# SabaPivot/ProjectionTrainer

Measured on AMD Instinct MI355X. Metric: Stage-1 images/sec/node (SigLIP-L-384 + Gemma3-1B, 576+128 tok), higher is better.
Workload: dtype bf16; 1 GPU; cfg2: SigLIP-ViT-L/16-384 frozen fwd + MLP projector fwd/bwd + Gemma3-1B frozen fwd/bwd, 575 vis + 128 text tokens; global_batch=32, per_gpu_batch=32, seq_len=703, parallelism=dp1

## Files before the change

include/ptk.h:

```cpp
#ifndef PTK_H
#define PTK_H

#include <stddef.h>
#include <stdint.h>

#ifdef __cplusplus
extern "C" {
#endif

#define PTK_ABI_VERSION 8

int ptk_abi_version(void);
const char* ptk_last_error(void);


typedef struct {
  int g;
  int skip;
  int64_t gs;
  int64_t off;
} ptk_rowmap;

enum { PTK_ACT_NONE = 0, PTK_ACT_GELU_TANH = 1, PTK_ACT_GELU_ERF = 2, PTK_ACT_GEGLU = 3,
       PTK_ACT_GELU_ERF_BWD = 4, PTK_ACT_GEGLU_BWD = 5 };
enum { PTK_OUT_BF16 = 0, PTK_OUT_F32 = 1, PTK_OUT_F32_BF16ROUND = 2 };

typedef struct {
  const void* A;
  const void* B;
  void* C;
  int M, N, K;
  int64_t lda, ldb, ldc;
  int batch;
  int batch_inner;
  int64_t sA0, sA1, sB0, sB1, sC0, sC1;
  float alpha;
  int act;
  int out;
  const float* bias;
  const float* rowadd;
  int rowadd_period;
  int64_t ld_rowadd;
  const float* resid;
  int64_t ld_resid;
  void* aux;
  void* aux2;
  int64_t ld_aux;
  const void* aux_in;
  const void* aux_in2;
  int64_t ld_aux_in;
  ptk_rowmap amap;
  ptk_rowmap cmap;
  const void* resid16;
  int64_t ld_resid16;
  int bf16_linear;
  void* tail_ws;
  const void* B_kt;
  int A_kt, C_kt, aux_kt, aux_in_kt;
} ptk_gemm_desc;
int ptk_gemm_ktiled_counts(int64_t* out2, int reset);
int ptk_gemm_ktiled_pair(const ptk_gemm_desc* producer, const ptk_gemm_desc* consumer, int ncu, int64_t part_floats,
                         int train);
int ptk_a_ktiled_reload(void);
int ptk_gemm(const ptk_gemm_desc* d, void* stream);
int64_t ptk_kstep_tile_offset(int64_t row, int64_t k, int64_t K);
int ptk_pack_kstep_tiles_bf16(const void* src, void* dst, int N, int K, void* stream);
#define PTK_GEMM_TAIL_COUNTER_BYTES 16384
size_t ptk_gemm_tail_scratch_bytes(void);
int ptk_gemm_tail_split(const ptk_gemm_desc* d);
int ptk_gemm_plan(const ptk_gemm_desc* d, int ncu, int* path, int* tile_rows, int* tail_split);
int ptk_gemm_split_plan(const ptk_gemm_desc* d, int ncu, int64_t part_floats, int* slices, int* kc, int* rem,
                        int* tail_ws);

int ptk_layernorm(const float* x, const float* w, const float* b, void* y, int rows, int cols, float eps,
                  void* stream);
int ptk_rmsnorm(const float* x, const float* w, void* y, float* rstd, int rows, int cols, float eps,
                void* stream);
int ptk_rmsnorm_bwd(const float* x, const float* w, const float* rstd, const float* dn, const float* dacc,
                    float* dx, int rows, int cols, void* stream);
int ptk_qknorm_rope_fwd(const void* qkv, const float* q_norm_w, const float* k_norm_w, const float* cos_t,
                        const float* sin_t, int batch, int seq, int heads, int kv_heads, int head_dim, float eps,
                        void* Q, void* K, void* V, float* rstd_q, float* rstd_k, void* stream);
int ptk_qknorm_rope_bwd(const void* qkv, const float* q_norm_w, const float* k_norm_w, const float* cos_t,
                        const float* sin_t, int batch, int seq, int heads, int kv_heads, int head_dim,
                        const float* rstd_q, const float* rstd_k, const void* dQ, const void* dK, const void* dV,
                        void* dqkv, void* stream);
int ptk_softmax(const float* S, void* P, int nz, int rows, int cols, int64_t ld, int rows_per_batch, int qdiv,
                int zdiv, int causal, int window, const int32_t* key_valid, int key_len, void* stream);
int ptk_cross_entropy(void* logits, int64_t ld, int rows, int vocab, const int64_t* targets, float* row_loss,
                      const float* gscale, void* stream);
int ptk_transpose_bf16(const void* in, int64_t ld_in, void* out, int64_t ld_out, int nz, int64_t s_in,
                       int64_t s_out, int rows, int cols, int rows_pad, void* stream);
int ptk_transpose_rows_bf16(const void* in, int64_t ld_in, int map_g, int64_t map_gs, int64_t map_off, int rows,
                            int cols, void* out, int64_t ld_out, int rows_pad, void* stream);
int ptk_weight_grad_bf16(const void* dy, int64_t lddy, int y_map_g, int64_t y_map_gs, int64_t y_map_off, int Ny,
                         const void* x, int64_t ldx, int x_map_g, int64_t x_map_gs, int64_t x_map_off, int Nx, int rows,
                         void* grad, void* ta, void* tb, float* part, int64_t part_floats, int mode, void* stream);
int ptk_cast_f32_bf16(const float* in, void* out, int64_t n, void* stream);
int ptk_fill_normal_bf16(void* out, int64_t n, uint64_t seed, float std, float mean, void* stream);
int ptk_gemm_timer_enable(int on);
int ptk_gemm_force_small_tiles(int mode);
int ptk_gemm_timer_read(int act_class, double* total_ms, int* count);
#define PTK_GEMM_NPATHS 9
int ptk_gemm_path_counts(int64_t* counts, int reset);

int ptk_stage_timers_enable(int on);
int ptk_stage_begin(const char* name, void* stream);
int ptk_stage_end(void* stream);
int64_t ptk_stage_timers_read(char* buf, size_t cap, int reset);

typedef struct {
  const void* Q; const void* K; const void* V; void* O; float* lse;
  int rows, nkeys, head_dim;
  int64_t ldq, ldk, ldo;
  int batch, batch_inner, zdiv;
  int64_t sQ0, sQ1, sK0, sK1, sO0, sO1;
  ptk_rowmap qmap, omap;
  int qdiv, causal, window;
  const int32_t* key_valid;
  float scale;
} ptk_flash_desc;
int ptk_flash_attn_fwd(const ptk_flash_desc* d, void* stream);

typedef struct {
  const void* Q; const void* K; const void* V; const void* O; const void* dO;
  const float* lse; float* delta;
  void* dQ; void* dK; void* dV;
  int rows, nkeys, head_dim;
  int batch, batch_inner, zdiv;
  int64_t ldo, sO0, sO1;
  ptk_rowmap omap;
  int qdiv, causal, window;
  const int32_t* key_valid;
  float scale;
  void* workspace;
  int64_t workspace_bytes;
} ptk_flash_bwd_desc;
size_t ptk_flash_bwd_workspace_bytes(const ptk_flash_bwd_desc* d);
int ptk_flash_attn_bwd(const ptk_flash_bwd_desc* d, void* stream);

typedef struct {
  int image_size, patch_size, channels, hidden, heads, intermediate, layers;
  float eps;
} ptk_siglip_config;

typedef struct {
  const void* wqkv;  const float* bqkv;
  const void* wo;    const float* bo;
  const void* w1;    const float* b1;
  const void* w2;    const float* b2;
  const float* ln1_w; const float* ln1_b;
  const float* ln2_w; const float* ln2_b;
  const void* wqkv_kt; const void* wo_kt; const void* w1_kt; const void* w2_kt;
} ptk_siglip_layer;

typedef struct {
  const void* patch_w;
  const float* patch_b;
  const float* pos;
  const float* post_w; const float* post_b;
  const ptk_siglip_layer* layers;
} ptk_siglip_weights;

size_t ptk_siglip_workspace_bytes(const ptk_siglip_config* c, int batch);
int ptk_siglip_fwd(const ptk_siglip_config* c, const ptk_siglip_weights* w, int batch, const void* pixels,
                   void* out, void* ws, size_t ws_bytes, void* stream);

typedef struct {
  int vision_dim, inter_dim, llm_dim;
  const void* w1;   const float* b1;
  const void* w2;   const float* b2;
  const void* w2t;
  void* tail_ws;
} ptk_projector;

int ptk_projector_fwd(const ptk_projector* p, int rows, const void* x, void* a, void* h, float* out,
                      ptk_rowmap out_map, int64_t ld_out, int round_bf16, void* stream);
size_t ptk_projector_workspace_bytes(const ptk_projector* p, int rows);
int ptk_projector_bwd(const ptk_projector* p, int rows, const void* x, const void* a, const void* h,
                      const void* dy, float* dw1, float* db1, float* dw2, float* db2, void* ws, size_t ws_bytes,
                      void* stream);
int ptk_gather_vision_grad(const float* dx_llm, int batch, int num_patches, int seq_pad, int llm_dim, void* dy,
                           void* stream);

typedef struct {
  int vocab, hidden, inter, layers, heads, kv_heads, head_dim;
  int sliding_window, sliding_pattern;
  int pad_token_id;
  float query_pre_attn_scalar, eps;
} ptk_gemma3_config;

typedef struct {
  const void* wqkv;  const void* wqkv_t;
  const void* wo;    const void* wo_t;
  const void* wgu;   const void* wgu_t;
  const void* wd;    const void* wd_t;
  const float* ln_in; const float* ln_post_attn; const float* ln_pre_ff; const float* ln_post_ff;
  const float* q_norm; const float* k_norm;
  const void* wqkv_kt; const void* wqkv_t_kt;
  const void* wo_kt;   const void* wo_t_kt;
  const void* wgu_kt;  const void* wgu_t_kt;
  const void* wd_kt;   const void* wd_t_kt;
} ptk_gemma3_layer;

typedef struct {
  const void* embed;
  const void* embed_t;
  const float* final_norm;
  const float* rope_cos_local; const float* rope_sin_local;
  const float* rope_cos_global; const float* rope_sin_global;
  int rope_max_pos;
  const ptk_gemma3_layer* layers;
} ptk_gemma3_weights;

typedef struct {
  int batch, text_len, num_vision, seq_pad;
  const int64_t* token_ids;
  const int64_t* labels;
  float* x;
// ... 136 lines not shown
```

projectiontrainer_amd/_lib.py:

```python
from __future__ import annotations

import ctypes as C
import os

_HERE = os.path.dirname(os.path.abspath(__file__))
LIB_PATH = os.path.join(_HERE, "libptk.so")
if os.environ.get("PTK_LIB"):
    LIB_PATH = os.path.join(os.path.dirname(_HERE), os.environ["PTK_LIB"])

c_void_p, c_int, c_int64, c_float, c_size_t, c_uint64 = C.c_void_p, C.c_int, C.c_int64, C.c_float, C.c_size_t, C.c_uint64
c_float_p = C.POINTER(C.c_float)

ACT_NONE, ACT_GELU_TANH, ACT_GELU_ERF, ACT_GEGLU, ACT_GELU_ERF_BWD, ACT_GEGLU_BWD = range(6)
OUT_BF16, OUT_F32, OUT_F32_BF16ROUND = range(3)


class RowMap(C.Structure):
    _fields_ = [("g", c_int), ("skip", c_int), ("gs", c_int64), ("off", c_int64)]


class GemmDesc(C.Structure):
    _fields_ = [("A", c_void_p), ("B", c_void_p), ("C", c_void_p),
                ("M", c_int), ("N", c_int), ("K", c_int),
                ("lda", c_int64), ("ldb", c_int64), ("ldc", c_int64),
                ("batch", c_int), ("batch_inner", c_int),
                ("sA0", c_int64), ("sA1", c_int64), ("sB0", c_int64), ("sB1", c_int64),
                ("sC0", c_int64), ("sC1", c_int64),
                ("alpha", c_float), ("act", c_int), ("out", c_int),
                ("bias", c_void_p), ("rowadd", c_void_p), ("rowadd_period", c_int),
                ("ld_rowadd", c_int64), ("resid", c_void_p), ("ld_resid", c_int64),
                ("aux", c_void_p), ("aux2", c_void_p), ("ld_aux", c_int64),
                ("aux_in", c_void_p), ("aux_in2", c_void_p), ("ld_aux_in", c_int64),
                ("amap", RowMap), ("cmap", RowMap), ("resid16", c_void_p), ("ld_resid16", c_int64),
                ("bf16_linear", c_int), ("tail_ws", c_void_p), ("B_kt", c_void_p),
                ("A_kt", c_int), ("C_kt", c_int), ("aux_kt", c_int), ("aux_in_kt", c_int)]


class FlashDesc(C.Structure):
    _fields_ = [("Q", c_void_p), ("K", c_void_p), ("V", c_void_p), ("O", c_void_p), ("lse", c_void_p),
                ("rows", c_int), ("nkeys", c_int), ("head_dim", c_int),
                ("ldq", c_int64), ("ldk", c_int64), ("ldo", c_int64),
                ("batch", c_int), ("batch_inner", c_int), ("zdiv", c_int),
                ("sQ0", c_int64), ("sQ1", c_int64), ("sK0", c_int64), ("sK1", c_int64),
                ("sO0", c_int64), ("sO1", c_int64), ("qmap", RowMap), ("omap", RowMap),
                ("qdiv", c_int), ("causal", c_int), ("window", c_int), ("key_valid", c_void_p),
                ("scale", c_float)]


class FlashBwdDesc(C.Structure):
    _fields_ = [("Q", c_void_p), ("K", c_void_p), ("V", c_void_p), ("O", c_void_p), ("dO", c_void_p),
                ("lse", c_void_p), ("delta", c_void_p), ("dQ", c_void_p), ("dK", c_void_p), ("dV", c_void_p),
                ("rows", c_int), ("nkeys", c_int), ("head_dim", c_int),
                ("batch", c_int), ("batch_inner", c_int), ("zdiv", c_int),
                ("ldo", c_int64), ("sO0", c_int64), ("sO1", c_int64), ("omap", RowMap),
                ("qdiv", c_int), ("causal", c_int), ("window", c_int), ("key_valid", c_void_p),
                ("scale", c_float), ("workspace", c_void_p), ("workspace_bytes", c_int64)]


class SiglipConfigC(C.Structure):
    _fields_ = [("image_size", c_int), ("patch_size", c_int), ("channels", c_int), ("hidden", c_int),
                ("heads", c_int), ("intermediate", c_int), ("layers", c_int), ("eps", c_float)]


class SiglipLayerC(C.Structure):
    _fields_ = [("wqkv", c_void_p), ("bqkv", c_void_p), ("wo", c_void_p), ("bo", c_void_p),
                ("w1", c_void_p), ("b1", c_void_p), ("w2", c_void_p), ("b2", c_void_p),
                ("ln1_w", c_void_p), ("ln1_b", c_void_p), ("ln2_w", c_void_p), ("ln2_b", c_void_p),
                ("wqkv_kt", c_void_p), ("wo_kt", c_void_p), ("w1_kt", c_void_p), ("w2_kt", c_void_p)]


class SiglipWeightsC(C.Structure):
    _fields_ = [("patch_w", c_void_p), ("patch_b", c_void_p), ("pos", c_void_p),
                ("post_w", c_void_p), ("post_b", c_void_p), ("layers", C.POINTER(SiglipLayerC))]


class ProjectorC(C.Structure):
    _fields_ = [("vision_dim", c_int), ("inter_dim", c_int), ("llm_dim", c_int),
                ("w1", c_void_p), ("b1", c_void_p), ("w2", c_void_p), ("b2", c_void_p), ("w2t", c_void_p),
                ("tail_ws", c_void_p)]


class Gemma3ConfigC(C.Structure):
    _fields_ = [("vocab", c_int), ("hidden", c_int), ("inter", c_int), ("layers", c_int), ("heads", c_int),
                ("kv_heads", c_int), ("head_dim", c_int), ("sliding_window", c_int),
                ("sliding_pattern", c_int), ("pad_token_id", c_int),
                ("query_pre_attn_scalar", c_float), ("eps", c_float)]


class Gemma3LayerC(C.Structure):
    _fields_ = [("wqkv", c_void_p), ("wqkv_t", c_void_p), ("wo", c_void_p), ("wo_t", c_void_p),
                ("wgu", c_void_p), ("wgu_t", c_void_p), ("wd", c_void_p), ("wd_t", c_void_p),
                ("ln_in", c_void_p), ("ln_post_attn", c_void_p), ("ln_pre_ff", c_void_p),
                ("ln_post_ff", c_void_p), ("q_norm", c_void_p), ("k_norm", c_void_p),
                ("wqkv_kt", c_void_p), ("wqkv_t_kt", c_void_p), ("wo_kt", c_void_p), ("wo_t_kt", c_void_p),
                ("wgu_kt", c_void_p), ("wgu_t_kt", c_void_p), ("wd_kt", c_void_p), ("wd_t_kt", c_void_p)]


class Gemma3WeightsC(C.Structure):
    _fields_ = [("embed", c_void_p), ("embed_t", c_void_p), ("final_norm", c_void_p),
                ("rope_cos_local", c_void_p), ("rope_sin_local", c_void_p),
                ("rope_cos_global", c_void_p), ("rope_sin_global", c_void_p),
                ("rope_max_pos", c_int), ("layers", C.POINTER(Gemma3LayerC))]


class Gemma3BatchC(C.Structure):
    _fields_ = [("batch", c_int), ("text_len", c_int), ("num_vision", c_int), ("seq_pad", c_int),
                ("token_ids", c_void_p), ("labels", c_void_p), ("x", c_void_p), ("dx", c_void_p),
                ("loss_scale", c_float), ("loss", c_void_p), ("label_offset", c_int)]


class Gemma3GenerateC(C.Structure):
    _fields_ = [("batch", c_int), ("prompt_len", c_int), ("max_new_tokens", c_int), ("do_sample", c_int),
                ("top_k", c_int), ("temperature", c_float), ("seed", C.c_uint64), ("eos_token_id", c_int64),
                ("pad_token_id", c_int64), ("prompt_batch_stride", c_int64), ("top_p", c_float)]


class Gemma3DecodeC(C.Structure):
    _fields_ = [("rows", c_int), ("prompt_len", c_int), ("max_new_tokens", c_int), ("prompt_repeat", c_int),
                ("prompt_batch_stride", c_int64)]


class Gemma3LayerGradsC(C.Structure):
    _fields_ = [(n, c_void_p) for n in ("wqkv", "wo", "wgu", "wd", "ln_in", "ln_post_attn", "ln_pre_ff",
                                        "ln_post_ff", "q_norm", "k_norm")]


class Gemma3GradsC(C.Structure):
    _fields_ = [("embed", c_void_p), ("final_norm", c_void_p), ("layers", C.POINTER(Gemma3LayerGradsC))]


class ImageDesc(C.Structure):
    _fields_ = [("src_off", c_int64), ("h", C.c_int32), ("w", C.c_int32), ("c", C.c_int32),
                ("kh", C.c_int32), ("kv", C.c_int32), ("pad_", C.c_int32),
                ("coef_off", c_int64), ("tmp_off", c_int64)]


ABI_VERSION = 8

SIGNATURES = {
    "ptk_abi_version": (c_int, []),
    "ptk_last_error": (C.c_char_p, []),
    "ptk_gemm": (c_int, [C.POINTER(GemmDesc), c_void_p]),
    "ptk_gemm_tail_scratch_bytes": (c_size_t, []),
    "ptk_gemm_tail_split": (c_int, [C.POINTER(GemmDesc)]),
    "ptk_gemm_plan": (c_int, [C.POINTER(GemmDesc), c_int] + [C.POINTER(c_int)] * 3),
    "ptk_gemm_split_plan": (c_int, [C.POINTER(GemmDesc), c_int, c_int64] + [C.POINTER(c_int)] * 4),
    "ptk_layernorm": (c_int, [c_void_p, c_void_p, c_void_p, c_void_p, c_int, c_int, c_float, c_void_p]),
    "ptk_rmsnorm": (c_int, [c_void_p, c_void_p, c_void_p, c_void_p, c_int, c_int, c_float, c_void_p]),
    "ptk_rmsnorm_bwd": (c_int, [c_void_p] * 6 + [c_int, c_int, c_void_p]),
    "ptk_qknorm_rope_fwd": (c_int, [c_void_p] * 5 + [c_int] * 5 + [c_float] + [c_void_p] * 6),
    "ptk_qknorm_rope_bwd": (c_int, [c_void_p] * 5 + [c_int] * 5 + [c_void_p] * 7),
    "ptk_softmax": (c_int, [c_void_p, c_void_p, c_int, c_int, c_int, c_int64, c_int, c_int, c_int, c_int,
                            c_int, c_void_p, c_int, c_void_p]),
    "ptk_cross_entropy": (c_int, [c_void_p, c_int64, c_int, c_int, c_void_p, c_void_p, c_void_p, c_void_p]),
    "ptk_transpose_bf16": (c_int, [c_void_p, c_int64, c_void_p, c_int64, c_int, c_int64, c_int64, c_int,
                                   c_int, c_int, c_void_p]),
    "ptk_transpose_rows_bf16": (c_int, [c_void_p, c_int64, c_int, c_int64, c_int64, c_int, c_int, c_void_p, c_int64,
                                        c_int, c_void_p]),
    "ptk_weight_grad_bf16": (c_int, [c_void_p, c_int64, c_int, c_int64, c_int64, c_int,
                                     c_void_p, c_int64, c_int, c_int64, c_int64, c_int, c_int,
                                     c_void_p, c_void_p, c_void_p, c_void_p, c_int64, c_int, c_void_p]),
    "ptk_cast_f32_bf16": (c_int, [c_void_p, c_void_p, c_int64, c_void_p]),
    "ptk_kstep_tile_offset": (c_int64, [c_int64, c_int64, c_int64]),
    "ptk_pack_kstep_tiles_bf16": (c_int, [c_void_p, c_void_p, c_int, c_int, c_void_p]),
    "ptk_fill_normal_bf16": (c_int, [c_void_p, c_int64, c_uint64, c_float, c_float, c_void_p]),
    "ptk_gemm_timer_enable": (c_int, [c_int]),
    "ptk_gemm_force_small_tiles": (c_int, [c_int]),
    "ptk_gemm_timer_read": (c_int, [c_int, C.POINTER(C.c_double), C.POINTER(c_int)]),
    "ptk_gemm_path_counts": (c_int, [c_void_p, c_int]),
    "ptk_gemm_ktiled_counts": (c_int, [c_void_p, c_int]),
    "ptk_gemm_ktiled_pair": (c_int, [C.POINTER(GemmDesc), C.POINTER(GemmDesc), c_int, c_int64, c_int]),
    "ptk_a_ktiled_reload": (c_int, []),
    "ptk_stage_timers_enable": (c_int, [c_int]),
    "ptk_stage_begin": (c_int, [C.c_char_p, c_void_p]),
    "ptk_stage_end": (c_int, [c_void_p]),
    "ptk_stage_timers_read": (c_int64, [C.c_char_p, c_size_t, c_int]),
    "ptk_flash_attn_fwd": (c_int, [C.POINTER(FlashDesc), c_void_p]),
    "ptk_flash_attn_bwd": (c_int, [C.POINTER(FlashBwdDesc), c_void_p]),
    "ptk_flash_bwd_workspace_bytes": (c_size_t, [C.POINTER(FlashBwdDesc)]),
    "ptk_siglip_workspace_bytes": (c_size_t, [C.POINTER(SiglipConfigC), c_int]),
    "ptk_siglip_fwd": (c_int, [C.POINTER(SiglipConfigC), C.POINTER(SiglipWeightsC), c_int, c_void_p, c_void_p,
                               c_void_p, c_size_t, c_void_p]),
    "ptk_projector_fwd": (c_int, [C.POINTER(ProjectorC), c_int, c_void_p, c_void_p, c_void_p, c_void_p, RowMap,
                                  c_int64, c_int, c_void_p]),
    "ptk_projector_workspace_bytes": (c_size_t, [C.POINTER(ProjectorC), c_int]),
    "ptk_projector_bwd": (c_int, [C.POINTER(ProjectorC), c_int] + [c_void_p] * 8 + [c_void_p, c_size_t, c_void_p]),
    "ptk_gather_vision_grad": (c_int, [c_void_p, c_int, c_int, c_int, c_int, c_void_p, c_void_p]),
    "ptk_gemma3_workspace_bytes": (c_size_t, [C.POINTER(Gemma3ConfigC), c_int, c_int, c_int]),
    "ptk_gemma3_loss_fwd_bwd": (c_int, [C.POINTER(Gemma3ConfigC), C.POINTER(Gemma3WeightsC),
                                        C.POINTER(Gemma3BatchC), c_void_p, c_size_t, c_void_p]),
    "ptk_gemma3_loss_fwd": (c_int, [C.POINTER(Gemma3ConfigC), C.POINTER(Gemma3WeightsC),
                                    C.POINTER(Gemma3BatchC), c_void_p, c_size_t, c_void_p]),
    "ptk_gemma3_train_workspace_bytes": (c_size_t, [C.POINTER(Gemma3ConfigC), c_int, c_int, c_int]),
    "ptk_gemma3_train_fwd_bwd": (c_int, [C.POINTER(Gemma3ConfigC), C.POINTER(Gemma3WeightsC),
                                         C.POINTER(Gemma3BatchC), C.POINTER(Gemma3GradsC), c_void_p, c_size_t,
                                         c_void_p]),
    "ptk_gemma3_generate_workspace_bytes": (c_size_t, [C.POINTER(Gemma3ConfigC), c_int, c_int, c_int]),
    "ptk_gemma3_generate": (c_int, [C.POINTER(Gemma3ConfigC), C.POINTER(Gemma3WeightsC), C.POINTER(Gemma3GenerateC),
                                    c_void_p, c_void_p, c_void_p, c_void_p, c_void_p, c_size_t, c_void_p]),
    "ptk_gemma3_decode_workspace_bytes": (c_size_t, [C.POINTER(Gemma3ConfigC), C.POINTER(Gemma3DecodeC)]),
    "ptk_gemma3_decode_prefill": (c_int, [C.POINTER(Gemma3ConfigC), C.POINTER(Gemma3WeightsC),
                                          C.POINTER(Gemma3DecodeC), c_void_p, c_void_p, c_int64, c_void_p, c_void_p,
                                          c_size_t, c_void_p]),
    "ptk_gemma3_decode_step": (c_int, [C.POINTER(Gemma3ConfigC), C.POINTER(Gemma3WeightsC), C.POINTER(Gemma3DecodeC),
                                       c_int, c_void_p, c_void_p, c_void_p, c_void_p, c_size_t, c_void_p]),
    "ptk_beam_candidates_workspace_bytes": (c_size_t, [c_int, c_int, c_int]),
    "ptk_beam_candidates": (c_int, [c_void_p, c_int64, c_void_p, c_int, c_int, c_int, c_int, c_int, c_float, c_float,
                                    c_int, c_uint64, c_int, c_int, c_void_p, c_void_p, c_void_p, c_void_p, c_size_t,
                                    c_void_p]),
    "ptk_sample_next_token_workspace_bytes": (c_size_t, [c_int]),
    "ptk_sample_next_token": (c_int, [c_void_p, c_int64, c_int, c_int, c_int, c_int, c_float, c_float, c_uint64, c_int,
                                      c_int64, c_int64, c_void_p, c_void_p, c_int64, c_int, c_float, c_void_p,
                                      c_void_p, c_size_t, c_void_p]),
    "ptk_beam_candidates_penalized_workspace_bytes": (c_size_t, [c_int, c_int, c_int]),
    "ptk_beam_candidates_penalized": (c_int, [c_void_p, c_int64, c_void_p, c_int, c_int, c_int, c_int, c_int, c_float,
                                              c_float, c_int, c_uint64, c_int, c_int, c_void_p, c_int64, c_int,
                                              c_float, c_void_p, c_void_p, c_void_p, c_void_p, c_size_t, c_void_p]),
    "ptk_gemma3_generate_penalized_workspace_bytes": (c_size_t, [C.POINTER(Gemma3ConfigC), c_int, c_int, c_int]),
    "ptk_gemma3_generate_penalized": (c_int, [C.POINTER(Gemma3ConfigC), C.POINTER(Gemma3WeightsC),
                                              C.POINTER(Gemma3GenerateC), c_void_p, c_void_p, c_void_p, c_void_p,
                                              c_float, c_void_p, c_size_t, c_void_p]),
    "ptk_gemm_skinny_part_bytes": (c_size_t, [c_int, c_int, c_int]),
    "ptk_gemm_skinny": (c_int, [c_void_p, c_int64, c_void_p, c_int64, c_void_p, c_int64, c_int, c_int, c_int, c_int,
                                c_void_p, c_size_t, c_void_p]),
    "ptk_embed_grad_workspace_bytes": (c_size_t, [c_int, c_int]),
    "ptk_embed_grad": (c_int, [c_void_p, c_int, c_int, c_int, c_int, c_int, c_float, c_void_p, c_void_p, c_void_p,
                               c_size_t, c_void_p]),
    "ptk_bf16_sumsq_partial_floats": (c_int, []),
    "ptk_bf16_grad_scale_sumsq": (c_int, [c_void_p, c_int64, c_float, c_void_p, c_void_p, c_void_p]),
    "ptk_adamw_bf16": (c_int, [c_void_p] * 4 + [c_int64, c_void_p, c_float] + [C.c_double] * 5 +
                       [c_int, c_void_p, c_void_p]),
    "ptk_resize_ksize": (c_int, [c_int, c_int]),
    "ptk_resize_coeffs": (c_int, [c_int, c_int, c_void_p, c_void_p]),
    "ptk_image_preprocess": (c_int, [c_void_p, c_void_p, c_void_p, c_int, c_int, c_int, c_int, c_void_p, c_int,
                                     c_void_p, c_void_p, c_void_p]),
    "ptk_comm_unique_id_bytes": (c_int, []),
    "ptk_comm_get_unique_id": (c_int, [c_void_p]),
    "ptk_comm_init": (c_int, [C.POINTER(c_void_p), c_void_p, c_int, c_int]),
    "ptk_comm_destroy": (c_int, [c_void_p]),
    "ptk_comm_world": (c_int, [c_void_p]),
    "ptk_comm_allreduce_sum": (c_int, [c_void_p, c_void_p, c_int64, c_void_p]),
    "ptk_comm_allreduce_avg": (c_int, [c_void_p, c_void_p, c_int64, c_void_p]),
    "ptk_projector_bwd_allreduce": (c_int, [C.POINTER(ProjectorC), c_int] + [c_void_p] * 5 +
                                    [c_void_p, c_size_t, c_void_p, c_void_p, c_void_p]),
    "ptk_clip_adamw": (c_int, [c_void_p, c_void_p, c_void_p, c_void_p, c_int64, c_float, c_float, c_float,
                               c_float, c_float, c_float, c_float, c_int, c_void_p, c_void_p, c_void_p]),
}

_lib = None


class PtkError(RuntimeError):
    pass


def lib():
    global _lib
    if _lib is None:
        if not os.path.exists(LIB_PATH):
            raise PtkError(f"libptk.so not found at {LIB_PATH}: run `python -c 'import __graft_entry__ as g; g.build()'`")
        L = C.CDLL(LIB_PATH)
        for name, (res, args) in SIGNATURES.items():
            if os.environ.get("PTK_LIB") and not hasattr(L, name):
                continue
            f = getattr(L, name)
            f.restype, f.argtypes = res, args
        if L.ptk_abi_version() != ABI_VERSION:
            raise PtkError("libptk ABI version mismatch")
        _lib = L
    return _lib


def check(rc: int, what: str = ""):
    if rc != 0:
        raise PtkError(f"{what}: {lib().ptk_last_error().decode()}")


def ptr(t) -> int | None:
    return None if t is None else t.data_ptr()


GEMM_PATHS = ("nt128", "big", "big2", "w4", "nt128b", "p8sk", "p8", "tn", "unused8")


def gemm_path_counts(reset=False):
    buf = (C.c_int64 * (8 * len(GEMM_PATHS)))()
    check(lib().ptk_gemm_path_counts(buf, int(reset)), "gemm_path_counts")
    return {(GEMM_PATHS[i // 8], i % 8): int(v) for i, v in enumerate(buf) if v}


def gemm_ktiled_counts(reset=False):
    buf = (C.c_int64 * 2)()
    check(lib().ptk_gemm_ktiled_counts(buf, int(reset)), "gemm_ktiled_counts")
    return int(buf[0]), int(buf[1])


_stages_on = os.environ.get("PTK_STAGE_TIMERS", "0") not in ("", "0")


def stage_timers_enable(on=True):
    global _stages_on
    _stages_on = bool(on)
    check(lib().ptk_stage_timers_enable(int(bool(on))), "stage_timers_enable")


class stage:

    def __init__(self, name, device=None):
        self.name, self.device, self.on = name, device, False

    def __enter__(self):
        self.on = _stages_on
        if self.on:
            self.st = stream_ptr(self.device)
            check(lib().ptk_stage_begin(self.name.encode(), self.st), "stage_begin")
        return self

    def __exit__(self, *exc):
        if self.on:
            check(lib().ptk_stage_end(self.st), "stage_end")
        return False


def stage_timers_read(reset=False):
    n = lib().ptk_stage_timers_read(None, 0, 0)
    if n < 0:
        check(-1, "stage_timers_read")
    buf = C.create_string_buffer(int(n) + 64)
    n = lib().ptk_stage_timers_read(buf, len(buf), int(reset))
    if n < 0:
        check(-1, "stage_timers_read")
    out = {}
    for line in buf.value.decode().splitlines():
        name, ms, cnt = line.split("\t")
        out[name] = (float(ms), int(cnt))
    return out


def stream_ptr(device=None) -> int:
    import torch
    return torch.cuda.current_stream(device).cuda_stream
```

projectiontrainer_amd/csrc/attn.hip:

```cpp
#include "common.h"
#include "ptk_internal.h"

namespace ptk {

constexpr int QKR_HB = 4;

template <int EPL>
__global__ void __launch_bounds__(256) qknorm_rope_fwd_kernel(const bf16_t* __restrict__ qkv,
                                                              const float* __restrict__ qw,
                                                              const float* __restrict__ kw,
                                                              const float* __restrict__ cos_t,
                                                              const float* __restrict__ sin_t, AttnShape sh,
                                                              float eps, bf16_t* __restrict__ Q,
                                                              bf16_t* __restrict__ K, bf16_t* __restrict__ V,
                                                              float* __restrict__ rstd_q, float* __restrict__ rstd_k) {
  constexpr int D = EPL * 64;
  const int lane = threadIdx.x & 63;
  const int nh = sh.Hq + 2 * sh.Hkv;
  const long m = (long)blockIdx.x * 4 + (threadIdx.x >> 6);
  if (m >= (long)sh.B * sh.S) return;
  const int b = (int)(m / sh.S), s = (int)(m - (long)b * sh.S);
  const int G = sh.Hq / sh.Hkv;
  const int fi = (lane & 31) * EPL;
  const long ps = sh.pos ? (long)sh.pos[m] : (long)s;
// ... 45 lines not shown
      } else {
        const int kvh = h - sh.Hq;
        dst = K + (((long)b * sh.Hkv + kvh) * sh.S + s) * D + lane * EPL;
        if (lane == 0) rstd_k[m * sh.Hkv + kvh] = rs;
      }
#pragma unroll
      for (int e = 0; e < EPL; ++e) dst[e] = f2bf(xn[e] * cs[e] + sgn * part[e] * sn[e]);
    }
  }
}

template <int EPL>
__global__ void __launch_bounds__(256) qknorm_rope_bwd_kernel(
    const bf16_t* __restrict__ qkv, const float* __restrict__ qw, const float* __restrict__ kw,
    const float* __restrict__ cos_t, const float* __restrict__ sin_t, AttnShape sh, const float* __restrict__ rstd_q,
    const float* __restrict__ rstd_k, const bf16_t* __restrict__ dQ, const bf16_t* __restrict__ dK,
    const bf16_t* __restrict__ dV, bf16_t* __restrict__ dqkv, FlashBwdArgs fb) {
  constexpr int D = EPL * 64;
  const int lane = threadIdx.x & 63;
  const int nh = sh.Hq + 2 * sh.Hkv;
  const long m = (long)blockIdx.x * 4 + (threadIdx.x >> 6);
  if (m >= (long)sh.B * sh.S) return;
  const int b = (int)(m / sh.S), s = (int)(m - (long)b * sh.S);
  const int G = sh.Hq / sh.Hkv;
  const float* dkv_src = nullptr;
  int dkv_np = 0;
  if (D == 256 && fb.dkv_deferred) {
    const int slab = s / DKV_KEYS;
    const int P = dkv_pieces(fb, slab);
    if (P > 1) {
      dkv_np = P;
      dkv_src = fb.dkv_part + (long)dkv_part_base(fb, slab) * fb.nz * (2L * DKV_KEYS * D) +
                (long)(s - slab * DKV_KEYS) * D + lane * EPL;
    }
  }
  const int fi = (lane & 31) * EPL;
  float cs[EPL], sn[EPL], wq[EPL], wk[EPL];
#pragma unroll
  for (int e = 0; e < EPL; ++e) {
    cs[e] = cos_t[(long)s * (D / 2) + fi + e];
    sn[e] = sin_t[(long)s * (D / 2) + fi + e];
    wq[e] = 1.f + qw[lane * EPL + e];
    wk[e] = 1.f + kw[lane * EPL + e];
  }
  const float sgn = lane < 32 ? 1.f : -1.f;
  const bf16_t* xrow = qkv + m * (long)nh * D + lane * EPL;
  bf16_t* orow = dqkv + m * (long)nh * D + lane * EPL;
  for (int h0 = 0; h0 < nh; h0 += QKR_HB) {
    bf16_t gy[QKR_HB][EPL], xr[QKR_HB][EPL];
    float rsv[QKR_HB];
#pragma unroll
    for (int i = 0; i < QKR_HB; ++i) {
      const int h = h0 + i;
      if (h >= nh) break;
      const bf16_t* dy;
      if (h < sh.Hq) {
        const int kvh = h / G, j = h - kvh * G;
        dy = dQ + ((((long)b * sh.Hkv + kvh) * sh.S + s) * G + j) * D + lane * EPL;
        rsv[i] = rstd_q[m * sh.Hq + h];
      } else if (h < sh.Hq + sh.Hkv) {
        const int kvh = h - sh.Hq;
        dy = dK + (((long)b * sh.Hkv + kvh) * sh.S + s) * D + lane * EPL;
        rsv[i] = rstd_k[m * sh.Hkv + kvh];
      } else {
        dy = dV + (((long)b * sh.Hkv + (h - sh.Hq - sh.Hkv)) * sh.S + s) * D + lane * EPL;
        rsv[i] = 0.f;
      }
      if (dkv_np > 0 && h >= sh.Hq) {
        const int which = h < sh.Hq + sh.Hkv ? 0 : 1;
        const int kvh = which == 0 ? h - sh.Hq : h - sh.Hq - sh.Hkv;
        const long z = (long)b * sh.Hkv + kvh;
        const float* src = dkv_src + z * (2L * DKV_KEYS * D) + (long)which * DKV_KEYS * D;
        const long pstride = (long)fb.nz * (2L * DKV_KEYS * D);
        float acc[EPL];
#pragma unroll
        for (int e = 0; e < EPL; ++e) acc[e] = 0.f;
        for (int pc = 0; pc < dkv_np; ++pc) {
#pragma unroll
          for (int e = 0; e < EPL; ++e) acc[e] += src[pc * pstride + e];
        }
        const float mul = which == 0 ? fb.scale : 1.f;
#pragma unroll
        for (int e = 0; e < EPL; ++e) gy[i][e] = f2bf(acc[e] * mul);
      } else {
#pragma unroll
        for (int e = 0; e < EPL; ++e) gy[i][e] = dy[e];
      }
      if (h < sh.Hq + sh.Hkv)
#pragma unroll
        for (int e = 0; e < EPL; ++e) xr[i][e] = xrow[(long)h * D + e];
    }
#pragma unroll
    for (int i = 0; i < QKR_HB; ++i) {
      const int h = h0 + i;
      if (h >= nh) break;
      bf16_t* out = orow + (long)h * D;
      if (h >= sh.Hq + sh.Hkv) {
#pragma unroll
        for (int e = 0; e < EPL; ++e) out[e] = gy[i][e];
        continue;
      }
      const bool isq = h < sh.Hq;
      const float rs = rsv[i];
      float ds[EPL], dc[EPL], part[EPL];
#pragma unroll
      for (int e = 0; e < EPL; ++e) {
        const float g = bf2f(gy[i][e]);
        dc[e] = g * cs[e];
        ds[e] = g * sn[e];
      }
#pragma unroll
      for (int e = 0; e < EPL; ++e) part[e] = xor32_get(ds[e]);
      float x[EPL], dxn[EPL];
      float sdot = 0.f;
#pragma unroll
      for (int e = 0; e < EPL; ++e) {
        x[e] = bf2f(xr[i][e]);
        dxn[e] = bfround(dc[e] + sgn * part[e]) * (isq ? wq[e] : wk[e]);
        sdot += dxn[e] * x[e];
      }
      sdot = warp_sum(sdot);
      const float c3 = rs * rs * rs * sdot / D;
#pragma unroll
      for (int e = 0; e < EPL; ++e) out[e] = f2bf(rs * dxn[e] - c3 * x[e]);
    }
  }
}

constexpr int SMAXV = 8;

__global__ void __launch_bounds__(256) softmax_fwd_kernel(const float* __restrict__ S, bf16_t* __restrict__ P,
                                                          long nrows, int rows, int cols, long ld, MaskSpec mk) {
  const int lane = threadIdx.x & 63;
  const long gr = (long)blockIdx.x * 4 + (threadIdx.x >> 6);
  if (gr >= nrows) return;
  const long z = gr / rows;
  const int r = (int)(gr - z * rows);
  const int q = (r % mk.rows_per_batch) / mk.qdiv;
  const long b = z / mk.zdiv;
  const float* srow = S + gr * ld;
  bf16_t* prow = P + gr * ld;
  float4 v[SMAXV];
  float mx = -INFINITY;
#pragma unroll
  for (int i = 0; i < SMAXV; ++i) {
    const int c0 = lane * 4 + i * 256;
    if (c0 >= cols) break;
    float4 t = *reinterpret_cast<const float4*>(srow + c0);
    float tv[4] = {t.x, t.y, t.z, t.w};
#pragma unroll
    for (int e = 0; e < 4; ++e) {
      const int k = c0 + e;
      bool ok = mk.key_valid ? (mk.key_valid[b * cols + k] != 0) : (k < mk.key_len);
      if (mk.causal) ok = ok && (k <= q);
      if (mk.window) ok = ok && (k > q - mk.window);
      tv[e] = ok ? tv[e] : -INFINITY;
      mx = fmaxf(mx, tv[e]);
    }
    v[i] = make_float4(tv[0], tv[1], tv[2], tv[3]);
  }
  mx = warp_max(mx);
  float sum = 0.f;
#pragma unroll
  for (int i = 0; i < SMAXV; ++i) {
    const int c0 = lane * 4 + i * 256;
    if (c0 >= cols) break;
    float4 t = v[i];
    t.x = t.x == -INFINITY ? 0.f : __expf(t.x - mx);
    t.y = t.y == -INFINITY ? 0.f : __expf(t.y - mx);
    t.z = t.z == -INFINITY ? 0.f : __expf(t.z - mx);
    t.w = t.w == -INFINITY ? 0.f : __expf(t.w - mx);
    v[i] = t;
    sum += t.x + t.y + t.z + t.w;
  }
  sum = warp_sum(sum);
  const float inv = sum > 0.f ? 1.f / sum : 0.f;
#pragma unroll
  for (int i = 0; i < SMAXV; ++i) {
    const int c0 = lane * 4 + i * 256;
    if (c0 >= cols) break;
    u16x4_t o;
    o[0] = f2bf(v[i].x * inv); o[1] = f2bf(v[i].y * inv); o[2] = f2bf(v[i].z * inv); o[3] = f2bf(v[i].w * inv);
    *reinterpret_cast<u16x4_t*>(prow + c0) = o;
  }
}

__global__ void __launch_bounds__(256) softmax_bwd_kernel(const bf16_t* __restrict__ P, const float* __restrict__ dP,
                                                          bf16_t* __restrict__ dS, long nrows, int cols, long ld,
                                                          float scale) {
  const int lane = threadIdx.x & 63;
  const long gr = (long)blockIdx.x * 4 + (threadIdx.x >> 6);
  if (gr >= nrows) return;
  float4 pv[SMAXV], gv[SMAXV];
  float dot = 0.f;
#pragma unroll
  for (int i = 0; i < SMAXV; ++i) {
    const int c0 = lane * 4 + i * 256;
    if (c0 >= cols) break;
    u16x4_t u = *reinterpret_cast<const u16x4_t*>(P + gr * ld + c0);
    pv[i] = make_float4(bf2f(u[0]), bf2f(u[1]), bf2f(u[2]), bf2f(u[3]));
    gv[i] = *reinterpret_cast<const float4*>(dP + gr * ld + c0);
    dot += pv[i].x * gv[i].x + pv[i].y * gv[i].y + pv[i].z * gv[i].z + pv[i].w * gv[i].w;
  }
  dot = warp_sum(dot);
#pragma unroll
  for (int i = 0; i < SMAXV; ++i) {
    const int c0 = lane * 4 + i * 256;
    if (c0 >= cols) break;
    u16x4_t o;
    o[0] = f2bf(pv[i].x * (gv[i].x - dot) * scale);
    o[1] = f2bf(pv[i].y * (gv[i].y - dot) * scale);
    o[2] = f2bf(pv[i].z * (gv[i].z - dot) * scale);
    o[3] = f2bf(pv[i].w * (gv[i].w - dot) * scale);
    *reinterpret_cast<u16x4_t*>(dS + gr * ld + c0) = o;
  }
}

#define QKR_DISPATCH(KERNEL, ...)                                                                     \
  switch (s.D) {                                                                                      \
    case 64: hipLaunchKernelGGL(KERNEL<1>, grid, dim3(256), 0, st, __VA_ARGS__); break;              \
    case 128: hipLaunchKernelGGL(KERNEL<2>, grid, dim3(256), 0, st, __VA_ARGS__); break;             \
    case 256: hipLaunchKernelGGL(KERNEL<4>, grid, dim3(256), 0, st, __VA_ARGS__); break;             \
    default: return set_error("qknorm_rope: head_dim %d unsupported", s.D);                          \
  }

int launch_qknorm_rope_fwd(const bf16_t* qkv, const float* qw, const float* kw, const float* cos_t,
                           const float* sin_t, AttnShape s, float eps, bf16_t* Q, bf16_t* K, bf16_t* V,
                           float* rstd_q, float* rstd_k, hipStream_t st) {
  if (s.Hq % s.Hkv) return set_error("qknorm_rope: Hq %% Hkv != 0");
  const long waves = (long)s.B * s.S;
  dim3 grid((unsigned)((waves + 3) / 4));
  QKR_DISPATCH(qknorm_rope_fwd_kernel, qkv, qw, kw, cos_t, sin_t, s, eps, Q, K, V, rstd_q, rstd_k)
  return hipGetLastError() == hipSuccess ? 0 : set_error("qknorm_rope_fwd launch failed");
}
int launch_qknorm_rope_bwd(const bf16_t* qkv, const float* qw, const float* kw, const float* cos_t,
                           const float* sin_t, AttnShape s, const float* rstd_q, const float* rstd_k,
                           const bf16_t* dQ, const bf16_t* dK, const bf16_t* dV, bf16_t* dqkv, hipStream_t st,
                           const FlashBwdArgs* dkv) {
  if (s.Hq % s.Hkv) return set_error("qknorm_rope: Hq %% Hkv != 0");
  FlashBwdArgs fb;
  fb.dkv_deferred = 0;
  if (dkv && dkv->dkv_deferred) {
    if (s.D != 256 || dkv->D != 256 || dkv->nkeys != s.S || dkv->nz != s.B * s.Hkv || !dkv->dkv_part)
      return set_error("qknorm_rope_bwd: deferred dK/dV plan does not match the shape");
    fb = *dkv;
  }
  const long waves = (long)s.B * s.S;
  dim3 grid((unsigned)((waves + 3) / 4));
  QKR_DISPATCH(qknorm_rope_bwd_kernel, qkv, qw, kw, cos_t, sin_t, s, rstd_q, rstd_k, dQ, dK, dV, dqkv, fb)
  return hipGetLastError() == hipSuccess ? 0 : set_error("qknorm_rope_bwd launch failed");
}
int launch_softmax_fwd(const float* S, bf16_t* P, int nz, int rows, int cols, long ld, MaskSpec m, hipStream_t st) {
  if (cols % 4 || cols > SMAXV * 256 || ld % 4) return set_error("softmax: cols=%d unsupported", cols);
  const long nrows = (long)nz * rows;
  if (nrows <= 0) return 0;
  hipLaunchKernelGGL(softmax_fwd_kernel, dim3((unsigned)((nrows + 3) / 4)), dim3(256), 0, st, S, P, nrows, rows,
                     cols, ld, m);
  return hipGetLastError() == hipSuccess ? 0 : set_error("softmax_fwd launch failed");
}
int launch_softmax_bwd(const bf16_t* P, const float* dP, bf16_t* dS, int nrows, int cols, long ld, float scale,
                       hipStream_t st) {
  if (cols % 4 || cols > SMAXV * 256 || ld % 4) return set_error("softmax_bwd: cols=%d unsupported", cols);
  if (nrows <= 0) return 0;
  hipLaunchKernelGGL(softmax_bwd_kernel, dim3((unsigned)((nrows + 3) / 4)), dim3(256), 0, st, P, dP, dS,
                     (long)nrows, cols, ld, scale);
  return hipGetLastError() == hipSuccess ? 0 : set_error("softmax_bwd launch failed");
}

}
```

projectiontrainer_amd/csrc/capi.cpp:

```cpp
#include <stdarg.h>
#include <stdio.h>

#include "../../include/ptk.h"
#include "ptk_internal.h"

namespace ptk {

static thread_local char g_err[512] = "";

int set_error(const char* fmt, ...) {
  va_list ap;
  va_start(ap, fmt);
  vsnprintf(g_err, sizeof(g_err), fmt, ap);
  va_end(ap);
  return -1;
}

RowMap to_map(ptk_rowmap m) { return RowMap{m.g, m.skip, (long)m.gs, (long)m.off}; }

GemmArgs to_args(const ptk_gemm_desc* d) {
  GemmArgs a;
  a.A = (const bf16_t*)d->A; a.B = (const bf16_t*)d->B; a.C = d->C;
  a.M = d->M; a.N = d->N; a.K = d->K;
  a.lda = d->lda; a.ldb = d->ldb; a.ldc = d->ldc;
// ... 96 lines not shown
int ptk_qknorm_rope_fwd(const void* qkv, const float* q_norm_w, const float* k_norm_w, const float* cos_t,
                        const float* sin_t, int batch, int seq, int heads, int kv_heads, int head_dim, float eps,
                        void* Q, void* K, void* V, float* rstd_q, float* rstd_k, void* stream) {
  const AttnShape sh{batch, seq, heads, kv_heads, head_dim};
  return launch_qknorm_rope_fwd((const bf16_t*)qkv, q_norm_w, k_norm_w, cos_t, sin_t, sh, eps, (bf16_t*)Q,
                                (bf16_t*)K, (bf16_t*)V, rstd_q, rstd_k, ST);
}
int ptk_qknorm_rope_bwd(const void* qkv, const float* q_norm_w, const float* k_norm_w, const float* cos_t,
                        const float* sin_t, int batch, int seq, int heads, int kv_heads, int head_dim,
                        const float* rstd_q, const float* rstd_k, const void* dQ, const void* dK, const void* dV,
                        void* dqkv, void* stream) {
  const AttnShape sh{batch, seq, heads, kv_heads, head_dim};
  return launch_qknorm_rope_bwd((const bf16_t*)qkv, q_norm_w, k_norm_w, cos_t, sin_t, sh, rstd_q, rstd_k,
                                (const bf16_t*)dQ, (const bf16_t*)dK, (const bf16_t*)dV, (bf16_t*)dqkv, ST);
}
int ptk_softmax(const float* S, void* P, int nz, int rows, int cols, int64_t ld, int rows_per_batch, int qdiv,
                int zdiv, int causal, int window, const int32_t* key_valid, int key_len, void* stream) {
  MaskSpec m{rows_per_batch > 0 ? rows_per_batch : rows, qdiv > 0 ? qdiv : 1, zdiv > 0 ? zdiv : 1, causal, window,
             key_valid, key_len};
  return launch_softmax_fwd(S, (bf16_t*)P, nz, rows, cols, ld, m, ST);
}

int ptk_cross_entropy(void* logits, int64_t ld, int rows, int vocab, const int64_t* targets, float* row_loss,
                      const float* gscale, void* stream) {
  return launch_ce_fwd_bwd((bf16_t*)logits, ld, rows, vocab, targets, row_loss, gscale, ST);
}

int ptk_transpose_bf16(const void* in, int64_t ld_in, void* out, int64_t ld_out, int nz, int64_t s_in, int64_t s_out,
                       int rows, int cols, int rows_pad, void* stream) {
  return launch_transpose((const bf16_t*)in, ld_in, s_in, 0, 1, (bf16_t*)out, ld_out, s_out, 0, nz, rows, cols,
                          rows_pad, ST);
}

int ptk_transpose_rows_bf16(const void* in, int64_t ld_in, int map_g, int64_t map_gs, int64_t map_off, int rows,
                            int cols, void* out, int64_t ld_out, int rows_pad, void* stream) {
  const RowMap m{map_g, 0, map_gs, map_off};
  return launch_transpose_rows((const bf16_t*)in, ld_in, m, rows, cols, (bf16_t*)out, ld_out, rows_pad, ST);
}

int64_t ptk_kstep_tile_offset(int64_t row, int64_t k, int64_t K) { return kstep_tile_offset(row, k, K); }
int ptk_pack_kstep_tiles_bf16(const void* src, void* dst, int N, int K, void* stream) {
  return launch_pack_kstep_tiles((const bf16_t*)src, (bf16_t*)dst, N, K, ST);
}
int ptk_cast_f32_bf16(const float* in, void* out, int64_t n, void* stream) {
  return launch_cast_f32_bf16(in, (bf16_t*)out, n, ST);
}

int ptk_gemm_force_small_tiles(int mode) {
  if (mode != 0 && mode != 1 && mode != 2 && mode != 4 && mode != 8 && mode != 32 && mode != 512 && mode != 1024 &&
      mode != 4096)
    return set_error("gemm tile mode %d not in {0, 1, 2, 4, 8, 32, 512, 1024, 4096}", mode);
  force_small_tiles(mode);
  return 0;
}
int ptk_gemm_timer_enable(int on) {
  timer_enable(on);
  return 0;
}
int ptk_gemm_timer_read(int act_class, double* total_ms, int* count) { return timer_read(act_class, total_ms, count); }
int ptk_gemm_path_counts(int64_t* counts, int reset) { return path_counts(counts, reset); }
int ptk_gemm_ktiled_counts(int64_t* out2, int reset) { return ktiled_counts(out2, reset); }
int ptk_gemm_ktiled_pair(const ptk_gemm_desc* producer, const ptk_gemm_desc* consumer, int ncu, int64_t part_floats,
                         int train) {
  if (!producer || !consumer || ncu <= 0 || producer->batch > 1 || consumer->batch > 1) return 0;
  return !train && gemm_ktiled_pair(to_args(producer), producer->act, to_args(consumer), (long)part_floats,
                                    test_plan_env(ncu), a_ktiled_mode() != 0, true) ? 1 : 0;
}

int ptk_fill_normal_bf16(void* out, int64_t n, uint64_t seed, float std, float mean, void* stream) {
  return launch_fill_normal_bf16((bf16_t*)out, n, seed, std, mean, ST);
}

int ptk_flash_attn_fwd(const ptk_flash_desc* d, void* stream) {
  if (!d) return set_error("flash: null desc");
  FlashArgs a;
  a.Q = (const bf16_t*)d->Q; a.K = (const bf16_t*)d->K; a.V = (const bf16_t*)d->V; a.O = (bf16_t*)d->O;
  a.lse = d->lse; a.rows = d->rows; a.nkeys = d->nkeys; a.D = d->head_dim;
  a.ldq = d->ldq; a.ldk = d->ldk; a.ldo = d->ldo;
  a.zin = d->batch_inner > 0 ? d->batch_inner : 1; a.zdiv = d->zdiv > 0 ? d->zdiv : 1;
  a.sQ0 = d->sQ0; a.sQ1 = d->sQ1; a.sK0 = d->sK0; a.sK1 = d->sK1; a.sO0 = d->sO0; a.sO1 = d->sO1;
  a.qmap = to_map(d->qmap); a.omap = to_map(d->omap);
  a.qdiv = d->qdiv > 0 ? d->qdiv : 1; a.causal = d->causal; a.window = d->window;
  a.key_valid = d->key_valid; a.scale = d->scale;
  return launch_attn_fwd(a, d->batch > 0 ? d->batch : 1, ST);
}

static FlashBwdArgs to_bwd_args(const ptk_flash_bwd_desc* d) {
  FlashBwdArgs a;
  a.Q = (const bf16_t*)d->Q; a.K = (const bf16_t*)d->K; a.V = (const bf16_t*)d->V; a.O = (const bf16_t*)d->O;
  a.dO = (const bf16_t*)d->dO; a.lse = d->lse; a.delta = d->delta;
  a.dQ = (bf16_t*)d->dQ; a.dK = (bf16_t*)d->dK; a.dV = (bf16_t*)d->dV;
  a.rows = d->rows; a.nkeys = d->nkeys; a.D = d->head_dim;
  a.zin = d->batch_inner > 0 ? d->batch_inner : 1; a.zdiv = d->zdiv > 0 ? d->zdiv : 1;
  a.ldo = d->ldo; a.sO0 = d->sO0; a.sO1 = d->sO1; a.omap = to_map(d->omap);
  a.qdiv = d->qdiv > 0 ? d->qdiv : 1; a.causal = d->causal; a.window = d->window;
  a.key_valid = d->key_valid; a.scale = d->scale;
  a.dkv_part = (float*)d->workspace;
  a.dkv_part_bytes = d->workspace && d->workspace_bytes > 0 ? (size_t)d->workspace_bytes : 0;
  return a;
}

size_t ptk_flash_bwd_workspace_bytes(const ptk_flash_bwd_desc* d) {
  if (!d) return 0;
  return attn_bwd_workspace_bytes(to_bwd_args(d), d->batch > 0 ? d->batch : 1);
}

int ptk_flash_attn_bwd(const ptk_flash_bwd_desc* d, void* stream) {
  if (!d) return set_error("flash_bwd: null desc");
  return launch_attn_bwd(to_bwd_args(d), d->batch > 0 ? d->batch : 1, ST);
}

int ptk_projector_fwd(const ptk_projector* p, int rows, const void* x, void* a, void* h, float* out,
                      ptk_rowmap out_map, int64_t ld_out, int round_bf16, void* stream) {
  const int Dv = p->vision_dim, I = p->inter_dim, Dl = p->llm_dim;
  TailScratchScope tail(p->tail_ws, ST);
  if (tail.status) return -1;
  StageScope stage("projector.fwd", ST);
  GemmArgs g1;
  g1.A = (const bf16_t*)x; g1.B = (const bf16_t*)p->w1; g1.C = h;
  g1.M = rows; g1.N = I; g1.K = Dv; g1.lda = Dv; g1.ldb = Dv; g1.ldc = I;
  g1.bias = p->b1; g1.aux = (bf16_t*)a; g1.ld_aux = I;
  if (launch_gemm(g1, ACT_GELU_ERF, OUT_BF16, 1, ST)) return -1;
  GemmArgs g2;
  g2.A = (const bf16_t*)h; g2.B = (const bf16_t*)p->w2; g2.C = out;
  g2.M = rows; g2.N = Dl; g2.K = I; g2.lda = I; g2.ldb = I; g2.ldc = ld_out;
  g2.bias = p->b2; g2.cmap = to_map(out_map);
  return launch_gemm(g2, ACT_NONE, round_bf16 ? OUT_F32_BFR : OUT_F32, 1, ST);
}

}
static size_t align256(size_t v) { return (v + 255) & ~(size_t)255; }
extern "C" {

size_t ptk_projector_workspace_bytes(const ptk_projector* p, int rows) {
  const size_t Dv = p->vision_dim, I = p->inter_dim, Dl = p->llm_dim, R = ((size_t)rows + 63) / 64 * 64;
  size_t s = 0;
  s += align256(Dl * R * 2);
  s += align256(I * R * 2);
  s += align256(R * I * 2);
  s += align256(Dv * R * 2);
  s += align256(64 * (I > Dl ? I : Dl) * 4);
  return s;
}

}

namespace ptk {
int projector_bwd_stage(const ptk_projector* p, int rows, const void* x, const void* a, const void* h, const void* dy,
                        float* dw1, float* db1, float* dw2, float* db2, void* ws, size_t ws_bytes, int stage,
                        hipStream_t st) {
  const int Dv = p->vision_dim, I = p->inter_dim, Dl = p->llm_dim, R = rows, Rp = (rows + 63) / 64 * 64;
  if (ws_bytes < ptk_projector_workspace_bytes(p, rows)) return set_error("projector_bwd: workspace too small");
  char* w = (char*)ws;
  bf16_t* dyT = (bf16_t*)w; w += align256((size_t)Dl * Rp * 2);
  bf16_t* T = (bf16_t*)w; w += align256((size_t)I * Rp * 2);
  bf16_t* dA = (bf16_t*)w; w += align256((size_t)Rp * I * 2);
  bf16_t* xT = (bf16_t*)w; w += align256((size_t)Dv * Rp * 2);
  float* part = (float*)w;
  const long part_floats = 64L * (I > Dl ? I : Dl);
  auto tn_wgrad = [&](const void* A, int lda, const void* B, int ldb, float* C, int M, int N) -> int {
    if (!wgrad_tn_enabled()) return 1;
    GemmArgs g;
    g.A = (const bf16_t*)A; g.B = (const bf16_t*)B; g.C = C; g.M = M; g.N = N; g.K = Rp;
    g.lda = lda; g.ldb = ldb; g.ldc = N;
    if (!tn_supported(g, OUT_F32, 1, lean_epilogue_enabled())) return 1;
    return gemm_tn(g, OUT_F32, 1, nullptr, st, R) ? -1 : 0;
  };
  if (stage == 0) {
    if (launch_colsum_bf16((const bf16_t*)dy, R, Dl, db2, part, part_floats, st)) return -1;
    const int tn = tn_wgrad(dy, Dl, h, I, dw2, Dl, I);
    if (tn <= 0) return tn;
    if (launch_transpose((const bf16_t*)dy, Dl, 0, 0, 1, dyT, Rp, 0, 0, 1, R, Dl, Rp, st)) return -1;
    if (launch_transpose((const bf16_t*)h, I, 0, 0, 1, T, Rp, 0, 0, 1, R, I, Rp, st)) return -1;
    GemmArgs g;
    g.A = dyT; g.B = T; g.C = dw2; g.M = Dl; g.N = I; g.K = Rp; g.lda = Rp; g.ldb = Rp; g.ldc = I;
    return launch_gemm(g, ACT_NONE, OUT_F32, 1, st);
  }
  GemmArgs g2;
  g2.A = (const bf16_t*)dy; g2.B = (const bf16_t*)p->w2t; g2.C = dA; g2.M = R; g2.N = I; g2.K = Dl;
  g2.lda = Dl; g2.ldb = Dl; g2.ldc = I; g2.aux_in = (const bf16_t*)a; g2.ld_aux_in = I;
  if (launch_gemm(g2, ACT_GELU_ERF_BWD, OUT_BF16, 1, st)) return -1;
// ... 40 lines not shown
```

projectiontrainer_amd/csrc/flash.hip:

```cpp
#include <algorithm>
#include <cstdlib>
#include <functional>
#include <queue>
#include <type_traits>
#include <vector>
#include "common.h"
#include "ptk_internal.h"

namespace ptk {

typedef __attribute__((ext_vector_type(4))) short s16x4_t;
typedef const __attribute__((address_space(1))) void* fa_gptr_t;
typedef __attribute__((address_space(3))) void* fa_lptr_t;

PTK_DEV void fa_glds16(const void* src, void* lds) {
  const uint32_t m0 = __builtin_amdgcn_readfirstlane((uint32_t)(uintptr_t)(fa_lptr_t)lds);
  asm volatile("s_nop 0\n\tglobal_load_lds_dwordx4 %0, off" ::"v"(src), "{m0}"(m0) : "memory");
}

template <int D>
PTK_DEV int swz_k(int r) { return D == 256 ? (r & 15) : ((r >> 1) & 7); }
template <int D>
PTK_DEV int swz_v(int r) { return D == 256 ? 2 * (r & 7) : 2 * ((r >> 1) & 3); }
PTK_DEV int swz_rt(int r) { return (r & 7) << 1; }
// ... 2027 lines not shown
        for (int j = 0; j < 4; ++j) {
          uv[j] = f2bf(dv[ds][kg][j]);
          uk[j] = f2bf(dk[ds][kg][j] * a.scale);
        }
        *reinterpret_cast<u16x4_t*>(dvp + 16 * ds) = uv;
        *reinterpret_cast<u16x4_t*>(dkp + 16 * ds) = uk;
      }
    }
  } else {
    float* part = a.dkv_part + ((long)(base + piece) * nz + z) * (2L * DKV_KEYS * D);
#pragma unroll
    for (int kg = 0; kg < KG; ++kg) {
      const int kl = wave * KPW + 16 * kg + c16;
      float* pk = part + (long)kl * D + 4 * g;
      float* pv = pk + (long)DKV_KEYS * D;
#pragma unroll
      for (int ds = 0; ds < DS; ++ds) {
        *reinterpret_cast<float4*>(pk + 16 * ds) = make_float4(dk[ds][kg][0], dk[ds][kg][1], dk[ds][kg][2], dk[ds][kg][3]);
        *reinterpret_cast<float4*>(pv + 16 * ds) = make_float4(dv[ds][kg][0], dv[ds][kg][1], dv[ds][kg][2], dv[ds][kg][3]);
      }
    }
  }
  FA_STAMPS_WRITE(2, c1 - c0);
}

__global__ void __launch_bounds__(256) attn_dkv_reduce_kernel(FlashBwdArgs a) {
  constexpr int D = 256;
  const int s = blockIdx.y;
  const int P = dkv_pieces(a, s);
  if (P == 1) return;
  int base = 0;
  for (int t = 0; t < s; ++t) {
    const int pt = dkv_pieces(a, t);
    if (pt > 1) base += pt;
  }
  const long i = (long)blockIdx.x * 256 + threadIdx.x;
  const long per_z = 2L * DKV_KEYS * D / 4;
  if (i >= (long)a.nz * per_z) return;
  const long z = i / per_z;
  const long r = i - z * per_z;
  const int which = (int)(r / (DKV_KEYS * D / 4));
  const int kl = (int)((r / (D / 4)) % DKV_KEYS);
  const int d4 = (int)(r % (D / 4));
  const int key = s * DKV_KEYS + kl;
  if (key >= a.nkeys) return;
  float4 acc = make_float4(0.f, 0.f, 0.f, 0.f);
  for (int pc = 0; pc < P; ++pc) {
    const float4 v = reinterpret_cast<const float4*>(a.dkv_part + ((long)(base + pc) * a.nz + z) * (2L * DKV_KEYS * D))[r];
    acc.x += v.x; acc.y += v.y; acc.z += v.z; acc.w += v.w;
  }
  const float m = which == 0 ? a.scale : 1.f;
  u16x4_t u;
  u[0] = f2bf(acc.x * m); u[1] = f2bf(acc.y * m); u[2] = f2bf(acc.z * m); u[3] = f2bf(acc.w * m);
  bf16_t* out = (which == 0 ? a.dK : a.dV) + (z * a.nkeys + key) * (long)D + 4 * d4;
  *reinterpret_cast<u16x4_t*>(out) = u;
}

static double dkv_makespan(FlashBwdArgs& a, int nz, int nslab, int target, int ncu) {
  a.dkv_target = target;
  std::vector<double> cost;
  for (int s = 0; s < nslab; ++s) {
    int lo, hi;
    dkv_slab_chunks(a, s, lo, hi);
    const int n = hi - lo, P = dkv_pieces(a, s);
    for (int p = 0; p < P; ++p) {
      const int c = (int)((long)(p + 1) * n / P - (long)p * n / P);
      cost.push_back(c + 1.5 + (P > 1 ? 1.0 : 0.0));
    }
  }
  std::sort(cost.begin(), cost.end(), std::greater<double>());
  std::priority_queue<double, std::vector<double>, std::greater<double>> cu;
  for (int i = 0; i < ncu; ++i) cu.push(0.0);
  double span = 0.0;
  for (double c : cost)
    for (int z = 0; z < nz; ++z) {
      const double t = cu.top() + c;
      cu.pop();
      cu.push(t);
      span = std::max(span, t);
    }
  return span;
}

static void dkv_plan(FlashBwdArgs& a, int nz, int& nslab, long& npieces, long& nsplit) {
  a.nz = nz;
  nslab = (a.nkeys + DKV_KEYS - 1) / DKV_KEYS;
  long total = 0;
  for (int s = 0; s < nslab; ++s) {
    int lo, hi;
    a.dkv_target = 0;
    dkv_slab_chunks(a, s, lo, hi);
    total += hi - lo;
  }
  const int ncu = device_cus();
  auto items_for = [&](int t) {
    long items = 0;
    a.dkv_target = t;
    for (int s = 0; s < nslab; ++s) items += dkv_pieces(a, s);
    return items;
  };
  int base = (int)std::max(4L, (total * nz + ncu - 1) / ncu);
  while (items_for(base) > 128 && base <= total) base += std::max(1, base / 8);
  int best = base;
  double best_span = dkv_makespan(a, nz, nslab, base, ncu);
  for (int k = 9; k >= 3; --k) {
    const int t = std::max(4, base * k / 12);
    if (items_for(t) > 128) break;
    const double sp = dkv_makespan(a, nz, nslab, t, ncu);
    if (sp < best_span - 1e-9) { best_span = sp; best = t; }
  }
  a.dkv_target = best;
  std::vector<std::pair<int, int>> it;
  npieces = 0;
  nsplit = 0;
  for (int s = 0; s < nslab; ++s) {
    int lo, hi;
    dkv_slab_chunks(a, s, lo, hi);
    const int n = hi - lo, P = dkv_pieces(a, s);
    npieces += P;
    if (P > 1) nsplit += P;
    for (int p = 0; p < P; ++p)
      it.push_back({-(int)((long)(p + 1) * n / P - (long)p * n / P), s * 256 + p});
  }
  std::stable_sort(it.begin(), it.end(), [](const std::pair<int, int>& x, const std::pair<int, int>& y) {
    return x.first < y.first;
  });
  a.dkv_items = (int)it.size();
  for (size_t i = 0; i < it.size() && i < 128; ++i) {
    a.dkv_item_slab[i] = (unsigned char)(it[i].second >> 8);
    a.dkv_item_piece[i] = (unsigned char)(it[i].second & 255);
  }
}

size_t attn_bwd_workspace_bytes(const FlashBwdArgs& a0, int nz) {
  if (a0.D != 256 || a0.rows <= 0 || nz <= 0) return 0;
  FlashBwdArgs a = a0;
  int nslab;
  long np, ns;
  dkv_plan(a, nz, nslab, np, ns);
  return (size_t)ns * nz * 2 * DKV_KEYS * 256 * sizeof(float);
}

int launch_attn_bwd(const FlashBwdArgs& a, int nz, hipStream_t st, FlashBwdArgs* defer) {
  if (defer) {
    *defer = a;
    defer->dkv_deferred = 0;
  }
  if (a.rows <= 0 || nz <= 0) return 0;
  if (a.rows % 64 || a.nkeys % 64) return set_error("attn_bwd: rows (%d) and keys (%d) must be multiples of 64",
                                                   a.rows, a.nkeys);
  if (a.ldo & 7) return set_error("attn_bwd: O stride must be a multiple of 8");
  const dim3 gd((unsigned)(((long)nz * a.rows + 15) / 16)), gq((unsigned)((long)((a.rows + 127) / 128) * nz)),
      gk((unsigned)(a.nkeys / 64), (unsigned)nz);
  switch (a.D) {
    case 64:
      hipLaunchKernelGGL(attn_delta_kernel<64>, gd, dim3(256), 0, st, a, nz);
      hipLaunchKernelGGL(attn_bwd_dkv_kernel<64>, gk, dim3(256), 0, st, a);
      hipLaunchKernelGGL(attn_bwd_dq_kernel<64>, gq, dim3(512), 0, st, a);
      break;
    case 256: {
      FlashBwdArgs b = a;
      int nslab;
      long np, ns;
      dkv_plan(b, nz, nslab, np, ns);
      if (ns > 0 && (!b.dkv_part || b.dkv_part_bytes < (size_t)ns * nz * 2 * DKV_KEYS * 256 * sizeof(float))) {
        b.dkv_target = 0;
        np = nslab;
        ns = 0;
        b.dkv_items = nslab;
        for (int s = 0; s < nslab && s < 128; ++s) { b.dkv_item_slab[s] = (unsigned char)s; b.dkv_item_piece[s] = 0; }
      }
      if (b.dkv_items > 128 || nslab > 128) return set_error("attn_bwd: %d dK/dV work items over %d key slabs (max 128)", b.dkv_items, nslab);
      const bool dq_new = (a.nkeys + 31) / 32 <= FA_MAXT;
      if (dq_new) {
        const bool persist = PTK_AB("PTK_ATTN_PERSIST", 1) != 0;
        const long nblk = (long)gq.x;
        const long g = persist ? std::min<long>(nblk, device_cus()) : nblk;
        hipLaunchKernelGGL(attn_bwd_dq256w_kernel, dim3((unsigned)g), dim3(256), 0, st, b, nz, (int)nblk);
      }
      else hipLaunchKernelGGL(attn_delta_kernel<256>, gd, dim3(256), 0, st, b, nz);
      if ((b.qdiv & (b.qdiv - 1)) || (long)b.rows * 256 * 2 > 0x7fffffffL)
        hipLaunchKernelGGL(attn_bwd_dkv256_kernel<32>, dim3((unsigned)(np * nz)), dim3(256), 0, st, b);
      else
        hipLaunchKernelGGL(attn_bwd_dkv256b_kernel, dim3((unsigned)(np * nz)), dim3(256), 0, st, b);
      if (ns > 0 && defer) {
        *defer = b;
        defer->dkv_deferred = 1;
      } else if (ns > 0)
        hipLaunchKernelGGL(attn_dkv_reduce_kernel, dim3((unsigned)((nz * 2L * DKV_KEYS * 64 + 255) / 256), (unsigned)nslab),
                           dim3(256), 0, st, b);
      if (!dq_new) hipLaunchKernelGGL(attn_bwd_dq_kernel<256>, gq, dim3(512), 0, st, b);
      break;
    }
    default: return set_error("attn_bwd: head_dim %d unsupported (64, 256)", a.D);
  }
  return hipGetLastError() == hipSuccess ? 0 : set_error("attn_bwd launch failed");
}

int launch_attn_fwd(const FlashArgs& a, int nz, hipStream_t st) {
  if (a.rows <= 0 || nz <= 0) return 0;
  if (a.nkeys < 4) return set_error("attn_fwd: nkeys must be >= 4");
  if ((a.ldq | a.ldk | a.ldo) & 7) return set_error("attn_fwd: row strides must be multiples of 8");
  if (a.key_valid && (a.nkeys & 3)) return set_error("attn_fwd: key_valid rows must be a multiple of 4");
  const long nblk = (long)((a.rows + 127) / 128) * nz;
  if (nblk > 0x7fffffffL) return set_error("attn_fwd: too many blocks");
  dim3 grid((unsigned)nblk);
  switch (a.D) {
    case 64: {
      if ((a.nkeys + 31) / 32 > FA_MAXT || (long)a.nkeys * a.ldk * 2 > 0x7fffffffL)
        hipLaunchKernelGGL((attn_fwd_kernel<64, 1>), grid, dim3(512), 0, st, a);
      else {
        FlashArgs b = a;
        b.variant = PTK_AB("PTK_FA64_XCD", 1) ? 0 : 1;
        hipLaunchKernelGGL(attn_fwd64_kernel, grid, dim3(512), 0, st, b);
      }
      break;
    }
    case 256: {
      if ((a.nkeys + 31) / 32 > FA_MAXT || (long)a.nkeys * a.ldk * 2 > 0x7fffffffL)
        hipLaunchKernelGGL((attn_fwd_kernel<256, 1>), grid, dim3(512), 0, st, a);
      else {
        const bool persist = PTK_AB("PTK_ATTN_PERSIST", 1) != 0;
        const long g = persist ? std::min<long>(nblk, device_cus()) : nblk;
        hipLaunchKernelGGL(attn_fwd256w_kernel, dim3((unsigned)g), dim3(256), 0, st, a, nz, (int)nblk);
      }
      break;
    }
    default: return set_error("attn_fwd: head_dim %d unsupported (64, 256)", a.D);
  }
  return hipGetLastError() == hipSuccess ? 0 : set_error("attn_fwd launch failed");
}

}

#ifdef PTK_FA_STAMPS
extern "C" int ptk_debug_fa_stamps_read(void* host, size_t bytes) {
  return hipMemcpyFromSymbol(host, HIP_SYMBOL(ptk::g_fa_stamps), bytes, 0, hipMemcpyDeviceToHost) == hipSuccess ? 0 : -1;
}
#endif
```

projectiontrainer_amd/csrc/models.cpp:

```cpp
#include <cstdlib>
#include <algorithm>
#include <math.h>
#include <string.h>

#include <vector>

#include "../../include/ptk.h"
#include "ptk_internal.h"

using namespace ptk;

namespace {

struct Bump {
  char* base;
  size_t off = 0;
  explicit Bump(void* b) : base((char*)b) {}
  template <class T>
  T* take(size_t n) {
    off = (off + 255) & ~(size_t)255;
    T* p = base ? reinterpret_cast<T*>(base + off) : nullptr;
    off += n * sizeof(T);
    return p;
  }
};

float bfround_host(float f) {
  uint32_t u;
  memcpy(&u, &f, 4);
  u += 0x7fffu + ((u >> 16) & 1u);
  u &= 0xffff0000u;
  memcpy(&f, &u, 4);
  return f;
}

constexpr int LM_SPLITK = 8;
constexpr int LM_KSLICES = 16;

#define CK(x) \
  do {        \
    if ((x)) return -1; \
  } while (0)
#define CKH(x)                                                                       \
  do {                                                                               \
    hipError_t e_ = (x);                                                             \
    if (e_ != hipSuccess) return set_error("%s: %s", #x, hipGetErrorString(e_));    \
  } while (0)

static bool geglu_split() {
  const int v = PTK_AB("PTK_GEGLU_SPLIT", 0) == 1;
  return v != 0;
}
static bool norm_wg_fused() { return PTK_AB("PTK_NORM_WG", 1) != 0; }

static int residual_norm_bwd_grads(const float* x2, const float* w_pre, const float* rstd_pre, const bf16_t* dn,
                                   float* dR, const bf16_t* t, const float* w_post, const float* rstd_t, bf16_t* dt,
                                   int M, int H, bf16_t* g_pre, bf16_t* g_post, float* wpart, hipStream_t st) {
  const RowMap ident{0, 0, 0, 0};
  if (g_pre && norm_wg_fused()) {
    const int nb = residual_norm_bwd_wg_blocks(M);
    float* pq = wpart + rms_wgrad_finish_floats(nb, H);
    CK(launch_residual_norm_bwd_wg(x2, w_pre, rstd_pre, dn, dR, t, w_post, rstd_t, dt, M, H, wpart, pq, st));
    CK(launch_rms_wgrad_finish(wpart, nb, H, g_pre, st));
    return launch_rms_wgrad_finish(pq, nb, H, g_post, st);
  }
  if (g_pre) CK(launch_rms_wgrad_bdy(x2, H, ident, rstd_pre, dn, H, M, H, g_pre, wpart, st));
  CK(launch_residual_norm_bwd_bdn(x2, w_pre, rstd_pre, dn, dR, t, w_post, rstd_t, dt, M, H, st));
  if (g_pre) CK(launch_rms_wgrad_bx(t, H, ident, rstd_t, dR, H, 1, M, H, g_post, wpart, st));
  return 0;
}
static bool dkv_reduce_split() {
  static const int v = [] { const char* e = getenv("PTK_DKV_REDUCE_SPLIT"); return e && e[0] == '1' ? 1 : 0; }();
  return v != 0;
}

static bool lm_stats_only() {
#ifdef PTK_DIAG
  static const int v = [] { const char* e = getenv("PTK_LM_STATS_ONLY"); return e && e[0] == '1' ? 1 : 0; }();
  return v != 0;
#else
  return false;
#endif
}

static bool ce_two_pass() {
  static const int v = [] { const char* e = getenv("PTK_CE_TWO_PASS"); return e && e[0] == '1' ? 1 : 0; }();
  return v != 0;
}

static int g_a_ktiled = -1;
}
namespace ptk {
int a_ktiled_mode() {
  if (g_a_ktiled < 0) {
    const char* e = getenv("PTK_A_KTILED");
    g_a_ktiled = e && e[0] == '0' ? 0 : (e && e[0] == '2' ? 2 : 1);
  }
  return g_a_ktiled;
}
}
extern "C" int ptk_a_ktiled_reload(void) {
  g_a_ktiled = -1;
  return a_ktiled_mode();
}
namespace {

GemmArgs gemm(const void* A, long lda, const void* B, long ldb, void* C, long ldc, int M, int N, int K,
              const void* B_kt = nullptr) {
  GemmArgs g;
  g.B_kt = (const bf16_t*)B_kt;
  g.A = (const bf16_t*)A; g.B = (const bf16_t*)B; g.C = C;
  g.lda = lda; g.ldb = ldb; g.ldc = ldc;
  g.M = M; g.N = N; g.K = K;
  return g;
}

struct SiglipWs {
  bf16_t *patches, *h, *a, *qkv, *o, *mlp;
  void* tail;
};

SiglipWs siglip_layout(Bump& bp, const ptk_siglip_config* c, int B) {
  const long D = c->hidden, I = c->intermediate, P = c->patch_size, Nn = (c->image_size / P) * (c->image_size / P);
  const long Np = (Nn + 63) / 64 * 64, M = B * Nn, H = c->heads, hd = D / H, Kp = (long)c->channels * P * P;
  SiglipWs w;
  w.patches = bp.take<bf16_t>(M * Kp);
  w.h = bp.take<bf16_t>(M * D);
  w.a = bp.take<bf16_t>(M * D);
  w.qkv = bp.take<bf16_t>(M * 3 * D);
  w.o = bp.take<bf16_t>(M * D);
  w.mlp = bp.take<bf16_t>(M * I);
  w.tail = bp.take<char>(p8_tail_scratch_bytes_models());
  return w;
}

struct GemmaLayerSave {
  float *x2, *rstd_in, *rstd_ao, *rstd_pre, *rstd_dn, *rstd_q, *rstd_k;
  bf16_t *qkv, *Q, *K, *V, *O, *ao, *glu_a, *glu_b, *dn;
  float* lse;
  bf16_t *xn_in = nullptr, *xn_ff = nullptr, *h = nullptr;
};
struct GemmaWs {
  std::vector<float*> x;
  std::vector<GemmaLayerSave> L;
  bf16_t *P, *xn, *O, *h, *Vt, *Kt, *Qt, *dqkv, *dgu, *dao, *dO, *dS, *dST, *PT, *dOT, *dQ, *dK, *dV, *xf, *logits;
  bf16_t* dtmp;
  float *S, *rstd_f, *row_loss, *dxf, *dxf_part, *count, *gscale, *delta;
  float* ce_stats = nullptr;
  float* dkv_part;
  size_t dkv_part_bytes;
  int32_t* key_valid;
  bf16_t *TA = nullptr, *TB = nullptr, *TL = nullptr, *TX = nullptr;
  float* wpart = nullptr;
  void* eg_keys = nullptr;
  float* skpart = nullptr;
  long sk_floats = 0;
  void* tail = nullptr;
};

GemmaWs gemma_layout(Bump& bp, const ptk_gemma3_config* c, int B, int T, int Sp, bool train = false) {
  const long H = c->hidden, I = c->inter, D = c->head_dim, Hq = c->heads, Hkv = c->kv_heads, G = Hq / Hkv;
  const long M = (long)B * Sp, Dq = Hq * D, Dqkv = (Hq + 2 * Hkv) * D, R = (long)B * T, V = c->vocab;
  const long Z = (long)B * Hkv, SG = (long)Sp * G;
  GemmaWs w;
  w.key_valid = bp.take<int32_t>(M);
  w.x.push_back(nullptr);
  for (int l = 1; l <= c->layers; ++l) w.x.push_back(bp.take<float>(M * H));
  for (int l = 0; l < c->layers; ++l) {
    GemmaLayerSave s;
    s.x2 = bp.take<float>(M * H);
    s.rstd_in = bp.take<float>(M);
    s.rstd_ao = bp.take<float>(M);
    s.rstd_pre = bp.take<float>(M);
    s.rstd_dn = bp.take<float>(M);
    s.rstd_q = bp.take<float>(M * Hq);
    s.rstd_k = bp.take<float>(M * Hkv);
    s.qkv = bp.take<bf16_t>(M * Dqkv);
    s.Q = bp.take<bf16_t>(Z * SG * D);
    s.K = bp.take<bf16_t>(Z * Sp * D);
    s.V = bp.take<bf16_t>(Z * Sp * D);
    s.lse = bp.take<float>(Z * SG);
    s.O = bp.take<bf16_t>(M * Dq);
    s.ao = bp.take<bf16_t>(M * H);
    s.glu_a = bp.take<bf16_t>(M * I);
    s.glu_b = bp.take<bf16_t>(M * I);
    s.dn = bp.take<bf16_t>(M * H);
    if (train) {
      s.xn_in = bp.take<bf16_t>(M * H);
      s.xn_ff = bp.take<bf16_t>(M * H);
      s.h = bp.take<bf16_t>(M * I);
    }
    w.L.push_back(s);
  }
  w.P = nullptr;
  w.xn = bp.take<bf16_t>(M * H);
  w.O = nullptr;
  w.h = bp.take<bf16_t>(M * I);
  w.Vt = nullptr;
  w.Kt = nullptr;
  w.Qt = nullptr;
  w.S = nullptr;
  w.delta = bp.take<float>(Z * SG);
  {
    FlashBwdArgs fa;
    fa.rows = (int)SG; fa.nkeys = Sp; fa.D = (int)D; fa.qdiv = (int)G; fa.causal = 1;
    size_t nb = attn_bwd_workspace_bytes(fa, (int)Z);
    fa.window = c->sliding_window;
    if (c->sliding_window > 0) nb = std::max(nb, attn_bwd_workspace_bytes(fa, (int)Z));
    w.dkv_part_bytes = nb;
    w.dkv_part = nb ? bp.take<float>((long)(nb / sizeof(float))) : nullptr;
  }
  w.dqkv = bp.take<bf16_t>(M * Dqkv);
  w.dgu = bp.take<bf16_t>(M * 2 * I);
  w.dtmp = bp.take<bf16_t>(M * H);
  w.dao = bp.take<bf16_t>(M * H);
  w.dO = bp.take<bf16_t>(Z * SG * D);
  w.dS = nullptr;
  w.dST = nullptr;
  w.PT = nullptr;
  w.dOT = nullptr;
  w.dQ = bp.take<bf16_t>(Z * SG * D);
  w.dK = bp.take<bf16_t>(Z * Sp * D);
  w.dV = bp.take<bf16_t>(Z * Sp * D);
  w.xf = bp.take<bf16_t>(R * H);
  w.rstd_f = bp.take<float>(R);
  w.logits = bp.take<bf16_t>(R * V);
  if (V % 64 == 0) w.ce_stats = bp.take<float>(R * (V / 64) * 2);
  w.row_loss = bp.take<float>(R);
  w.dxf = bp.take<float>(R * H);
  w.dxf_part = bp.take<float>((long)std::max(LM_SPLITK + 1, LM_KSLICES) * R * H);
  w.count = bp.take<float>(4);
  w.gscale = bp.take<float>(4);
  if (train) {
    const long Rp = (R + 63) / 64 * 64;
    w.TA = bp.take<bf16_t>(std::max(std::max(2 * I, Dqkv), H) * M);
    w.TB = bp.take<bf16_t>(std::max(std::max(H, Dq), I) * M);
    w.TL = bp.take<bf16_t>(V * Rp);
    w.TX = bp.take<bf16_t>(H * Rp);
    w.eg_keys = bp.take<char>((long)embed_grad_ws_bytes(B, T));
    w.wpart = bp.take<float>(std::max(std::max((long)rms_wgrad_partial_floats((int)M, (int)H),
                                               2L * rms_wgrad_finish_floats(residual_norm_bwd_wg_blocks((int)M), (int)H)),
                                      (long)qknorm_wgrad_partial_floats(M, (int)D)));
  }
  w.sk_floats = std::max(std::max(2 * M * H, 2 * 2 * I * H), 4 * std::max(Dqkv, H) * H);
  if (train) w.sk_floats = std::max(w.sk_floats, V * H);
  w.sk_floats = std::max(w.sk_floats, (long)(p8_tail_scratch_bytes() / sizeof(float)) + 64);
  if (train) w.sk_floats = std::max(w.sk_floats, (long)(tn_slab_bytes() / sizeof(float)));
  w.skpart = bp.take<float>(w.sk_floats);
  w.tail = bp.take<char>(p8_tail_scratch_bytes_models());
  return w;
}

int gemm_split(const GemmArgs& a, int out, float* part, long part_floats, hipStream_t st) {
  const GemmPlanEnv env = gemm_plan_env();
  const GemmSplitPlan sp = gemm_split_plan(a, out, part ? part_floats : 0, env);
  if (sp.kc != 0 && a.a_kt) return set_error("gemm_split: a K split cannot read a k-step-tiled A");
  if (sp.kc == 0) {
    GemmArgs b = a;
    GemmPlan plan = sp.direct;
    if (sp.tail_ws) {
      b.tail_ws = part;
      plan.tail.slab = reinterpret_cast<float*>(reinterpret_cast<char*>(part) + P8_CNT_BYTES);
    }
    return launch_gemm(b, ACT_NONE, out, 1, st, env.force_tiles == 0 ? &plan : nullptr);
  }
  const int kc = sp.kc, nfull = sp.slices, rem = sp.rem;
  GemmArgs b = a;
  b.B_kt = nullptr;
  b.C = part; b.ldc = a.N; b.K = kc;
  b.sA0 = kc; b.sB0 = kc; b.sC0 = (long)a.M * a.N;
  b.bf16_linear = 0; b.resid16 = nullptr; b.ld_resid16 = 0;
  CK(launch_gemm(b, ACT_NONE, OUT_F32, nfull, st));
  if (rem) {
    GemmArgs r = b;
    r.A = a.A + (long)nfull * kc; r.B = a.B + (long)nfull * kc; r.K = rem;
    r.C = part + (long)nfull * a.M * a.N;
    CK(launch_gemm(r, ACT_NONE, OUT_F32, 1, st));
  }
  const bool bf = out == OUT_BF16;
  return launch_splitk_reduce(part, nfull + (rem ? 1 : 0), a.M, a.N, a.C, a.ldc, bf ? 1 : 0,
                              bf ? a.resid16 : nullptr, a.ld_resid16, st);
}

static int wgrad_tn_mode() { return PTK_AB("PTK_WGRAD_TN", 1); }
}
namespace ptk {
int wgrad_tn_enabled() { return wgrad_tn_mode() != 0; }
}
namespace {
int weight_grad(const bf16_t* dy, long lddy, RowMap ymap, int Ny, const bf16_t* x, long ldx, RowMap xmap, int Nx,
                int rows, bf16_t* TA, bf16_t* TB, void* grad, float* skpart, long sk_floats, hipStream_t st,
                int tn = -1) {
  if (!grad) return 0;
  if (tn < 0) tn = wgrad_tn_mode();
  if (tn && ymap.g == 0 && ymap.off == 0 && xmap.g == 0 && xmap.off == 0 && rows > 0) {
    const int Kp = (rows + 63) / 64 * 64;
    GemmArgs g = gemm(dy, lddy, x, ldx, grad, Nx, Ny, Nx, Kp);
    g.bf16_linear = 1;
    g.resid16 = (const bf16_t*)grad;
    g.ld_resid16 = Nx;
    const GemmPlanEnv env = gemm_plan_env();
    if (skpart && (size_t)sk_floats * sizeof(float) >= tn_slab_bytes() && tn_supported(g, OUT_BF16, 1, env.lean_epi))
      return gemm_tn(g, OUT_BF16, 1, skpart, st, rows);
    const int S = skpart ? tn_slices(g, sk_floats, env) : (tn_supported(g, OUT_BF16, 1, env.lean_epi) ? 1 : 0);
    if (S == 1) return gemm_tn(g, OUT_BF16, 1, nullptr, st, rows);
    if (S > 1) {
      GemmArgs b = g;
      b.C = skpart;
      b.ldc = Nx;
      b.bf16_linear = 0;
      b.resid16 = nullptr;
      b.ld_resid16 = 0;
      CK(gemm_tn(b, OUT_F32, S, nullptr, st, rows));
      return launch_splitk_reduce(skpart, S, Ny, Nx, grad, Nx, 1, (const bf16_t*)grad, Nx, st);
    }
  }
  if (tn == 2) return set_error("weight_grad: the TN path does not take Ny %d Nx %d rows %d", Ny, Nx, rows);
  if (!TA || !TB)
    return set_error("weight_grad: Ny %d Nx %d rows %d take the transpose path, which needs ta / tb scratch", Ny, Nx,
                     rows);
  const int Kp = (rows + 63) / 64 * 64;
  CK(launch_transpose_rows(dy, lddy, ymap, rows, Ny, TA, Kp, Kp, st));
  CK(launch_transpose_rows(x, ldx, xmap, rows, Nx, TB, Kp, Kp, st));
  GemmArgs g = gemm(TA, Kp, TB, Kp, grad, Nx, Ny, Nx, Kp);
  g.bf16_linear = 1;
  g.resid16 = (const bf16_t*)grad;
  g.ld_resid16 = Nx;
  return gemm_split(g, OUT_BF16, skpart, sk_floats, st);
}

}

extern "C" {

int ptk_weight_grad_bf16(const void* dy, int64_t lddy, int y_map_g, int64_t y_map_gs, int64_t y_map_off, int Ny,
                         const void* x, int64_t ldx, int x_map_g, int64_t x_map_gs, int64_t x_map_off, int Nx, int rows,
                         void* grad, void* ta, void* tb, float* part, int64_t part_floats, int mode, void* stream) {
  if (mode < 0 || mode > 2) return set_error("weight_grad: mode %d (0 auto, 1 transposes, 2 TN)", mode);
// ... 53 lines not shown
      fa.zin = Hh; fa.zdiv = Hh;
      fa.sQ0 = fa.sK0 = (long)Nn * 3 * D; fa.sQ1 = fa.sK1 = hd;
      fa.sO0 = (long)Nn * D; fa.sO1 = hd;
      fa.scale = 1.0f / sqrtf((float)hd);
      StageScope sf("siglip.flash", st);
      CK(launch_attn_fwd(fa, B * Hh, st));
    }
    {
      GemmArgs g = gemm(w.o, D, L.wo, D, w.h, D, M, D, D, L.wo_kt);
      g.bias = L.bo; g.bf16_linear = 1; g.resid16 = w.h; g.ld_resid16 = D;
      CK(launch_gemm(g, ACT_NONE, OUT_BF16, 1, st));
    }
    sq.next("siglip.mlp");
    CK(launch_layernorm_bf16(w.h, L.ln2_w, L.ln2_b, w.a, M, D, c->eps, st));
    {
      GemmArgs g = gemm(w.a, D, L.w1, D, w.mlp, I, M, I, D, L.w1_kt);
      g.bias = L.b1;
      CK(launch_gemm(g, ACT_GELU_TANH, OUT_BF16, 1, st));
    }
    {
      GemmArgs g = gemm(w.mlp, I, L.w2, I, w.h, D, M, D, I, L.w2_kt);
      g.bias = L.b2; g.bf16_linear = 1; g.resid16 = w.h; g.ld_resid16 = D;
      CK(launch_gemm(g, ACT_NONE, OUT_BF16, 1, st));
    }
  }
  sq.next("siglip.post_norm");
  CK(launch_layernorm_bf16(w.h, wt->post_w, wt->post_b, (bf16_t*)out, M, D, c->eps, st));
  return 0;
}

size_t ptk_gemma3_workspace_bytes(const ptk_gemma3_config* c, int batch, int text_len, int seq_pad) {
  Bump bp(nullptr);
  gemma_layout(bp, c, batch, text_len, seq_pad);
  return bp.off + 256;
}

size_t ptk_gemma3_train_workspace_bytes(const ptk_gemma3_config* c, int batch, int text_len, int seq_pad) {
  Bump bp(nullptr);
  gemma_layout(bp, c, batch, text_len, seq_pad, true);
  return bp.off + 256;
}

}

namespace {

int gemma_run(const ptk_gemma3_config* c, const ptk_gemma3_weights* wt, const ptk_gemma3_batch* bt,
              const ptk_gemma3_grads* gr, void* ws, size_t ws_bytes, hipStream_t st, bool fwd_only = false) {
  const bool train = gr != nullptr;
  const int B = bt->batch, T = bt->text_len, Nv = bt->num_vision, Sp = bt->seq_pad, S = Nv + T;
  const int lo = bt->label_offset;
  if (Sp % 64 || S > Sp) return set_error("gemma3: seq_pad %d must be a multiple of 64 and >= %d", Sp, S);
  if (Sp > wt->rope_max_pos) return set_error("gemma3: seq_pad %d exceeds rope table (%d)", Sp, wt->rope_max_pos);
  if (c->heads % c->kv_heads) return set_error("gemma3: heads %% kv_heads");
  if (Nv < 1) return set_error("gemma3: num_vision must be >= 1");
  if (lo < 0 || lo >= T) return set_error("gemma3: label_offset %d outside [0, text_len %d)", lo, T);
  const size_t need = train ? ptk_gemma3_train_workspace_bytes(c, B, T, Sp) : ptk_gemma3_workspace_bytes(c, B, T, Sp);
  if (ws_bytes < need) return set_error("gemma3: workspace too small");
  if (c->vocab % 64 || c->vocab < 64 * LM_SPLITK) return set_error("gemma3: vocab must be a multiple of 64 and >= %d", 64 * LM_SPLITK);
  if (train && (!gr->layers || !gr->embed || !gr->final_norm)) return set_error("gemma3 train: grads missing");
  const int H = c->hidden, I = c->inter, D = c->head_dim, Hq = c->heads, Hkv = c->kv_heads, G = Hq / Hkv;
  const int M = B * Sp, Dq = Hq * D, Dqkv = (Hq + 2 * Hkv) * D, Tl = T - lo, R = B * Tl, V = c->vocab;
  const int Z = B * Hkv, SG = Sp * G, nl = c->layers;
  const float eps = c->eps, scale = 1.0f / sqrtf(c->query_pre_attn_scalar);
  Bump bp(ws);
  GemmaWs w = gemma_layout(bp, c, B, T, Sp, train);
  TailScratchScope tail(w.tail, st);
  CK(tail.status);
  AttnShape ash{B, Sp, Hq, Hkv, D};
  const RowMap ident{0, 0, 0, 0};
  const int Rp = (R + 63) / 64 * 64;
  StageSeq sq(st);
  sq.next("gemma.embed");

  const float escale = bfround_host(sqrtf((float)H));
  CK(launch_build_llm_inputs((const bf16_t*)wt->embed, bt->token_ids, B, T, Nv, S, Sp, H, escale, c->pad_token_id,
                             bt->x, w.key_valid, st));
  w.x[0] = bt->x;
  CK(launch_rmsnorm_fwd(w.x[0], H, ident, wt->layers[0].ln_in, train ? w.L[0].xn_in : w.xn, w.L[0].rstd_in, M, H,
                        eps, st));

  const RowMap lossmap{Tl, 0, Sp, Nv - 1 + lo};

  auto mlp_fwd = [&](int l, GemmArgs& g, GemmArgs& d) {
    const ptk_gemma3_layer& L = wt->layers[l];
    g = gemm(train ? w.L[l].xn_ff : w.xn, H, L.wgu, H, train ? w.L[l].h : w.h, I, M, 2 * I, H, L.wgu_kt);
    g.aux = w.L[l].glu_a; g.aux2 = w.L[l].glu_b; g.ld_aux = I;
    d = gemm(g.C, I, L.wd, I, w.L[l].dn, H, M, H, I, L.wd_kt);
  };
  auto mlp_bwd = [&](int l, GemmArgs& g, GemmArgs& d) {
    const ptk_gemma3_layer& L = wt->layers[l];
    g = gemm(w.dao, H, L.wd_t, H, w.dgu, 2 * I, M, I, H, L.wd_t_kt);
    g.aux_in = w.L[l].glu_a; g.aux_in2 = w.L[l].glu_b; g.ld_aux_in = I;
    d = gemm(w.dgu, 2 * I, L.wgu_t, 2 * I, w.dtmp, H, M, H, 2 * I, L.wgu_t_kt);
  };
  bool h_kt = false, dgu_kt = false, fac_kt = false;
  if (!train && nl > 1 && !geglu_split() && a_ktiled_mode()) {
    const GemmPlanEnv env = gemm_plan_env();
    h_kt = true;
    dgu_kt = !fwd_only;
    fac_kt = dgu_kt && a_ktiled_mode() != 2;
    for (int l = 0; l + 1 < nl; ++l) {
      GemmArgs gf, df, gb, db;
      mlp_fwd(l, gf, df);
      mlp_bwd(l, gb, db);
      h_kt = h_kt && gemm_ktiled_pair(gf, ACT_GEGLU, df, w.sk_floats, env, true, false);
      dgu_kt = dgu_kt && gemm_ktiled_pair(gb, ACT_GEGLU_BWD, db, w.sk_floats, env, true, false);
      fac_kt = fac_kt && gemm_ktiled_pair(gf, ACT_GEGLU, df, w.sk_floats, env, true, true) &&
               gemm_ktiled_pair(gb, ACT_GEGLU_BWD, db, w.sk_floats, env, true, true);
    }
  }

  for (int l = 0; l < nl; ++l) {
    const ptk_gemma3_layer& L = wt->layers[l];
    GemmaLayerSave& sv = w.L[l];
    const bool sliding = (l + 1) % c->sliding_pattern != 0;
    const float* cs = sliding ? wt->rope_cos_local : wt->rope_cos_global;
    const float* sn = sliding ? wt->rope_sin_local : wt->rope_sin_global;
    bf16_t* xin = train ? sv.xn_in : w.xn;
    bf16_t* xff = train ? sv.xn_ff : w.xn;
    bf16_t* hh = train ? sv.h : w.h;
    sq.next("gemma.fwd.attn");
    CK(gemm_split(gemm(xin, H, L.wqkv, H, sv.qkv, Dqkv, M, Dqkv, H, L.wqkv_kt), OUT_BF16, w.skpart, w.sk_floats, st));
    CK(launch_qknorm_rope_fwd(sv.qkv, L.q_norm, L.k_norm, cs, sn, ash, eps, sv.Q, sv.K, sv.V, sv.rstd_q, sv.rstd_k,
                              st));
    {
      FlashArgs fa;
      fa.Q = sv.Q; fa.K = sv.K; fa.V = sv.V; fa.O = sv.O; fa.lse = sv.lse;
      fa.rows = SG; fa.nkeys = Sp; fa.D = D;
      fa.ldq = D; fa.ldk = D; fa.ldo = D;
      fa.zin = Hkv; fa.zdiv = Hkv;
      fa.sQ0 = (long)Hkv * SG * D; fa.sQ1 = (long)SG * D;
      fa.sK0 = (long)Hkv * Sp * D; fa.sK1 = (long)Sp * D;
      fa.sO0 = (long)Sp * Hq * D; fa.sO1 = (long)G * D;
      fa.omap = RowMap{G, 0, Hq, 0};
      fa.qdiv = G; fa.causal = 1; fa.window = sliding ? c->sliding_window : 0;
      fa.key_valid = w.key_valid;
      fa.scale = scale;
      StageScope sf("gemma.fwd.flash", st);
      CK(launch_attn_fwd(fa, Z, st));
    }
    CK(gemm_split(gemm(sv.O, Dq, L.wo, Dq, sv.ao, H, M, H, Dq, L.wo_kt), OUT_BF16, w.skpart, w.sk_floats, st));
    CK(launch_residual_norm_fwd(sv.ao, w.x[l], L.ln_post_attn, L.ln_pre_ff, sv.x2, xff, sv.rstd_ao, sv.rstd_pre, M,
                                H, eps, st));
    sq.next("gemma.fwd.mlp");
    if (l + 1 < nl) {
      GemmArgs g, d;
      mlp_fwd(l, g, d);
      g.c_kt = d.a_kt = h_kt;
      g.aux_kt = fac_kt;
      CK(launch_gemm(g, ACT_GEGLU, OUT_BF16, 1, st));
      CK(gemm_split(d, OUT_BF16, w.skpart, w.sk_floats, st));
    } else {
      GemmArgs g = gemm(xff, H, L.wgu, H, hh, I, R, 2 * I, H, L.wgu_kt);
      g.amap = lossmap;
      g.aux = sv.glu_a; g.aux2 = sv.glu_b; g.ld_aux = I;
      CK(launch_gemm(g, ACT_GEGLU, OUT_BF16, 1, st));
      CK(launch_zero(sv.dn, (size_t)M * H * sizeof(bf16_t), st));
      GemmArgs g2 = gemm(hh, I, L.wd, I, sv.dn, H, R, H, I, L.wd_kt);
      g2.cmap = lossmap;
      CK(launch_gemm(g2, ACT_NONE, OUT_BF16, 1, st));
    }
    const float* wnext = (l + 1 < nl) ? wt->layers[l + 1].ln_in : nullptr;
    float* rnext = (l + 1 < nl) ? w.L[l + 1].rstd_in : nullptr;
    bf16_t* xnext = (train && l + 1 < nl) ? w.L[l + 1].xn_in : w.xn;
    CK(launch_residual_norm_fwd(sv.dn, sv.x2, L.ln_post_ff, wnext, w.x[l + 1], xnext, sv.rstd_dn, rnext, M, H, eps,
                                st));
  }

  sq.next("gemma.lm_head_ce");
  CK(launch_rmsnorm_fwd(w.x[nl], H, lossmap, wt->final_norm, w.xf, w.rstd_f, R, H, eps, st));
  {
    GemmArgs g = gemm(w.xf, H, wt->embed, H, w.logits, V, R, V, H);
    if (w.ce_stats && !ce_two_pass()) {
      g.row_stats = w.ce_stats;
      g.ld_stats = (V / 64) * 2;
      g.stats_only = lm_stats_only() ? 1 : 0;
    }
    CK(launch_gemm(g, ACT_NONE, OUT_BF16, 1, st));
    CK(launch_count_valid(bt->labels, R, bt->loss_scale, w.gscale, w.count, st));
    if (g.row_stats)
      CK(launch_ce_stats_fwd_bwd(w.logits, V, R, V, w.ce_stats, g.ld_stats, bt->labels, w.row_loss, w.gscale, st));
    else
      CK(launch_ce_fwd_bwd(w.logits, V, R, V, bt->labels, w.row_loss, w.gscale, st));
  }
  CK(launch_loss_reduce(w.row_loss, R, w.count, bt->loss, st));
  if (fwd_only) return 0;
  sq.next("gemma.lm_head_bwd");
  if (train) CK(weight_grad(w.logits, V, ident, V, w.xf, H, ident, H, R, w.TL, w.TX, gr->embed, w.skpart, w.sk_floats, st));
  const bool ks_fits = (double)R * V * 2 + (double)LM_KSLICES * (V / LM_KSLICES) * 2 < 4293918720.0;
  if (R % 256 == 0 && V % (64 * LM_KSLICES) == 0 && ks_fits) {
    GemmArgs g = gemm(w.logits, V, wt->embed_t, V, w.dxf_part, H, R, H, V / LM_KSLICES);
    CK(gemm_p8_kslices(g, LM_KSLICES, st));
    CK(launch_sum_partials(w.dxf_part, LM_KSLICES, (long)R * H, w.dxf, st));
  } else {
    const int kc = V / (64 * LM_SPLITK) * 64, rem = V - LM_SPLITK * kc;
    GemmArgs g = gemm(w.logits, V, wt->embed_t, V, w.dxf_part, H, R, H, kc);
    g.sA0 = kc; g.sB0 = kc; g.sC0 = (long)R * H;
    CK(launch_gemm(g, ACT_NONE, OUT_F32, LM_SPLITK, st));
    if (rem) {
      const long o = (long)LM_SPLITK * kc;
      CK(launch_gemm(gemm(w.logits + o, V, (const bf16_t*)wt->embed_t + o, V, w.dxf_part + (long)LM_SPLITK * R * H, H, R, H, rem),
                     ACT_NONE, OUT_F32, 1, st));
    }
    CK(launch_sum_partials(w.dxf_part, LM_SPLITK + (rem ? 1 : 0), (long)R * H, w.dxf, st));
  }
  float* dR = bt->dx;
  CK(launch_zero(dR, (size_t)M * H * 4, st));
  CK(launch_rmsnorm_bwd_scatter(w.x[nl], lossmap, wt->final_norm, w.rstd_f, w.dxf, dR, R, H, st));
  if (train)
    CK(launch_rms_wgrad(w.x[nl], H, lossmap, w.rstd_f, w.dxf, H, 1, R, H, (bf16_t*)gr->final_norm, w.wpart, st));

  for (int l = nl - 1; l >= 0; --l) {
    const ptk_gemma3_layer& L = wt->layers[l];
    const ptk_gemma3_layer_grads* GL = train ? &gr->layers[l] : nullptr;
    GemmaLayerSave& sv = w.L[l];
    const bool sliding = (l + 1) % c->sliding_pattern != 0;
    const float* cs = sliding ? wt->rope_cos_local : wt->rope_cos_global;
    const float* sn = sliding ? wt->rope_sin_local : wt->rope_sin_global;
    const bool last = l == nl - 1;
    sq.next("gemma.bwd.mlp");
    if (last) {
      CK(launch_post_norm_bwd(dR, sv.dn, L.ln_post_ff, sv.rstd_dn, w.dao, M, H, st));
      if (train)
        CK(launch_rms_wgrad_bx(sv.dn, H, ident, sv.rstd_dn, dR, H, 1, M, H, (bf16_t*)GL->ln_post_ff, w.wpart, st));
    }
    if (train)
      CK(last ? weight_grad(w.dao, H, lossmap, H, sv.h, I, ident, I, R, w.TA, w.TB, GL->wd, w.skpart, w.sk_floats, st)
              : weight_grad(w.dao, H, ident, H, sv.h, I, ident, I, M, w.TA, w.TB, GL->wd, w.skpart, w.sk_floats, st));
    if (!last) {
      if (geglu_split()) {
        CK(launch_gemm(gemm(w.dao, H, L.wd_t, H, w.h, I, M, I, H, L.wd_t_kt), ACT_NONE, OUT_BF16, 1, st));
        CK(launch_geglu_bwd(w.h, sv.glu_a, sv.glu_b, w.dgu, M, I, st));
      } else {
        GemmArgs g, d;
        mlp_bwd(l, g, d);
        g.c_kt = dgu_kt;
        g.aux_in_kt = fac_kt;
        CK(launch_gemm(g, ACT_GEGLU_BWD, OUT_BF16, 1, st));
      }
      if (train) CK(weight_grad(w.dgu, 2 * I, ident, 2 * I, sv.xn_ff, H, ident, H, M, w.TA, w.TB, GL->wgu, w.skpart, w.sk_floats, st));
      {
        GemmArgs g, d;
        mlp_bwd(l, g, d);
        d.a_kt = dgu_kt;
        CK(gemm_split(d, OUT_BF16, w.skpart, w.sk_floats, st));
      }
    } else {
      GemmArgs g = gemm(w.dao, H, L.wd_t, H, w.h, I, R, I, H, L.wd_t_kt);
      g.amap = lossmap;
      CK(launch_gemm(g, ACT_NONE, OUT_BF16, 1, st));
      CK(launch_geglu_bwd(w.h, sv.glu_a, sv.glu_b, w.dgu, R, I, st));
      if (train) CK(weight_grad(w.dgu, 2 * I, ident, 2 * I, sv.xn_ff, H, lossmap, H, R, w.TA, w.TB, GL->wgu, w.skpart, w.sk_floats, st));
      CK(launch_zero(w.dtmp, (size_t)M * H * sizeof(bf16_t), st));
      GemmArgs g2 = gemm(w.dgu, 2 * I, L.wgu_t, 2 * I, w.dtmp, H, R, H, 2 * I, L.wgu_t_kt);
      g2.cmap = lossmap;
      CK(launch_gemm(g2, ACT_NONE, OUT_BF16, 1, st));
    }
    sq.next("gemma.bwd.attn");
    CK(residual_norm_bwd_grads(sv.x2, L.ln_pre_ff, sv.rstd_pre, w.dtmp, dR, sv.ao, L.ln_post_attn, sv.rstd_ao, w.dao,
                               M, H, train ? (bf16_t*)GL->ln_pre_ff : nullptr,
                               train ? (bf16_t*)GL->ln_post_attn : nullptr, w.wpart, st));
    if (train)
      CK(weight_grad(w.dao, H, ident, H, sv.O, Dq, ident, Dq, M, w.TA, w.TB, GL->wo, w.skpart, w.sk_floats, st));
    {
      GemmArgs g = gemm(w.dao, H, L.wo_t, H, w.dO, (long)G * D, M, G * D, H, L.wo_t_kt);
      g.sB0 = (long)G * D * H; g.sC0 = (long)Sp * G * D;
      g.cmap = RowMap{Sp, 0, (long)Hkv * Sp, 0};
      CK(launch_gemm(g, ACT_NONE, OUT_BF16, Hkv, st));
    }
    FlashBwdArgs dkv_plan;
    dkv_plan.dkv_deferred = 0;
    {
      FlashBwdArgs fb;
      fb.Q = sv.Q; fb.K = sv.K; fb.V = sv.V; fb.O = sv.O; fb.dO = w.dO; fb.lse = sv.lse; fb.delta = w.delta;
      fb.dQ = w.dQ; fb.dK = w.dK; fb.dV = w.dV;
      fb.rows = SG; fb.nkeys = Sp; fb.D = D;
      fb.zin = Hkv; fb.zdiv = Hkv;
      fb.ldo = D; fb.sO0 = (long)Sp * Hq * D; fb.sO1 = (long)G * D;
      fb.omap = RowMap{G, 0, Hq, 0};
      fb.qdiv = G; fb.causal = 1; fb.window = sliding ? c->sliding_window : 0;
      fb.key_valid = w.key_valid;
      fb.scale = scale;
      fb.dkv_part = w.dkv_part; fb.dkv_part_bytes = w.dkv_part_bytes;
      StageScope sf("gemma.bwd.flash", st);
      CK(launch_attn_bwd(fb, Z, st, (dkv_reduce_split() || train) ? nullptr : &dkv_plan));
    }
    CK(launch_qknorm_rope_bwd(sv.qkv, L.q_norm, L.k_norm, cs, sn, ash, sv.rstd_q, sv.rstd_k, w.dQ, w.dK, w.dV, w.dqkv,
                              st, &dkv_plan));
    if (train) {
      CK(launch_qknorm_wgrad(sv.qkv, cs, sn, ash, sv.rstd_q, sv.rstd_k, w.dQ, w.dK, (bf16_t*)GL->q_norm,
                             (bf16_t*)GL->k_norm, w.wpart, st));
      CK(weight_grad(w.dqkv, Dqkv, ident, Dqkv, sv.xn_in, H, ident, H, M, w.TA, w.TB, GL->wqkv, w.skpart, w.sk_floats, st));
    }
    CK(gemm_split(gemm(w.dqkv, Dqkv, L.wqkv_t, Dqkv, w.dtmp, H, M, H, Dqkv, L.wqkv_t_kt), OUT_BF16, w.skpart, w.sk_floats, st));
    if (l > 0) {
      const ptk_gemma3_layer& Lp = wt->layers[l - 1];
      const GemmaLayerSave& sp = w.L[l - 1];
      CK(residual_norm_bwd_grads(w.x[l], L.ln_in, sv.rstd_in, w.dtmp, dR, sp.dn, Lp.ln_post_ff, sp.rstd_dn, w.dao,
                                 M, H, train ? (bf16_t*)GL->ln_in : nullptr,
                                 train ? (bf16_t*)gr->layers[l - 1].ln_post_ff : nullptr, w.wpart, st));
    } else {
      if (train)
        CK(launch_rms_wgrad_bdy(w.x[l], H, ident, sv.rstd_in, w.dtmp, H, M, H, (bf16_t*)GL->ln_in, w.wpart, st));
      CK(launch_rmsnorm_bwd_bdn(w.x[l], L.ln_in, sv.rstd_in, w.dtmp, dR, dR, M, H, st));
    }
  }
  if (train) sq.next("gemma.embed_grad");
  if (train) CK(launch_embed_grad(bt->token_ids, B, T, Nv, Sp, H, escale, dR, (bf16_t*)gr->embed, w.eg_keys, st));
  return 0;
}

}

namespace {

struct GenPass {
  float *xa, *xb, *x2, *rs1, *rs2, *rq, *rk;
  bf16_t *xn, *qkv, *Q, *K, *V, *O, *ao, *h, *dn;
  int32_t* kv;
  float* skp = nullptr;
  size_t skp_bytes = 0;
};
size_t gen_skinny_bytes(const ptk_gemma3_config* c, long rows) {
  if (rows > 256) return 0;
  rows = std::min<long>(rows, 64);
  const int H = c->hidden, I = c->inter, D = c->head_dim, Dq = c->heads * D, Dqkv = (c->heads + 2 * c->kv_heads) * D;
  const int M = (int)rows;
  const int shapes[5][2] = {{Dqkv, H}, {H, Dq}, {2 * I, H}, {H, I}, {c->vocab, H}};
  size_t b = 0;
  for (const auto& nk : shapes) b = std::max(b, skinny_part_bytes(M, nk[0], nk[1]));
  return b;
}
int gen_gemm(const GenPass& g, const bf16_t* A, long lda, const void* B, long ldb, bf16_t* C, long ldc, int M, int N,
             int K, int act, hipStream_t st) {
  if (g.skp_bytes > 0 && skinny_supported(std::min(M, 64), N, K, lda, ldb, ldc, act)) {
    for (int r0 = 0; r0 < M; r0 += 64)
      CK(launch_gemm_skinny(A + (long)r0 * lda, lda, (const bf16_t*)B, ldb, C + (long)r0 * ldc, ldc, std::min(64, M - r0),
                            N, K, act, g.skp, g.skp_bytes, st));
    return 0;
  }
  return launch_gemm(gemm(A, lda, B, ldb, C, ldc, M, N, K), act, OUT_BF16, 1, st);
}
struct GenWs {
  GenPass pre, dec;
  std::vector<bf16_t*> kc, vc;
  bf16_t *xf, *logits;
  float* rstd_f;
  int32_t* finished;
  int64_t *next, *feed;
  void* tail;
};
GenPass gen_pass(Bump& bp, const ptk_gemma3_config* c, long M) {
  const long H = c->hidden, I = c->inter, D = c->head_dim, Hq = c->heads, Hkv = c->kv_heads;
  const long Dq = Hq * D, Dqkv = (Hq + 2 * Hkv) * D;
  GenPass g;
  g.xa = bp.take<float>(M * H);
  g.xb = bp.take<float>(M * H);
  g.x2 = bp.take<float>(M * H);
  g.rs1 = bp.take<float>(M);
  g.rs2 = bp.take<float>(M);
  g.rq = bp.take<float>(M * Hq);
  g.rk = bp.take<float>(M * Hkv);
  g.xn = bp.take<bf16_t>(M * H);
  g.qkv = bp.take<bf16_t>(M * Dqkv);
  g.Q = bp.take<bf16_t>(M * Dq);
  g.K = bp.take<bf16_t>(M * Hkv * D);
// ... 482 lines not shown
```

projectiontrainer_amd/csrc/norm.hip:

```cpp
#include "common.h"
#include "ptk_internal.h"

namespace ptk {

constexpr int MAXV = 12;

PTK_DEV float4 ld4(const float* p) { return *reinterpret_cast<const float4*>(p); }
PTK_DEV void st4(float* p, float4 v) { *reinterpret_cast<float4*>(p) = v; }
PTK_DEV float4 ld4bf(const bf16_t* p) {
  u16x4_t u = *reinterpret_cast<const u16x4_t*>(p);
  return make_float4(bf2f(u[0]), bf2f(u[1]), bf2f(u[2]), bf2f(u[3]));
}
PTK_DEV void st4bf(bf16_t* p, float4 v) {
  u16x4_t u;
  u[0] = f2bf(v.x); u[1] = f2bf(v.y); u[2] = f2bf(v.z); u[3] = f2bf(v.w);
  *reinterpret_cast<u16x4_t*>(p) = u;
}
PTK_DEV float dot4(float4 a, float4 b) { return a.x * b.x + a.y * b.y + a.z * b.z + a.w * b.w; }
PTK_DEV float4 bfr4(float4 v) { return make_float4(bfround(v.x), bfround(v.y), bfround(v.z), bfround(v.w)); }
PTK_DEV float4 onep(float4 w) { return make_float4(1.f + w.x, 1.f + w.y, 1.f + w.z, 1.f + w.w); }
PTK_DEV float4 mul4(float4 a, float4 b) { return make_float4(a.x * b.x, a.y * b.y, a.z * b.z, a.w * b.w); }
PTK_DEV float4 add4(float4 a, float4 b) { return make_float4(a.x + b.x, a.y + b.y, a.z + b.z, a.w + b.w); }
PTK_DEV float4 scl4(float4 a, float s) { return make_float4(a.x * s, a.y * s, a.z * s, a.w * s); }

#define ROW_SETUP                                          \
  const int lane = threadIdx.x & 63;                       \
  const long row = (long)blockIdx.x * 4 + (threadIdx.x >> 6); \
  if (row >= rows) return;

#define FOR_V for (int v = 0; v < NV; ++v) if (v < NV - 1 || lane * 4 + v * 256 < cols)
#define COL (lane * 4 + v * 256)

PTK_DEV float4 ldx4(const float* p) { return ld4(p); }
PTK_DEV float4 ldx4(const bf16_t* p) { return ld4bf(p); }

template <typename T, int NV>
PTK_DEV void layernorm_body(const T* __restrict__ x, const float* __restrict__ w, const float* __restrict__ b,
                            bf16_t* __restrict__ y, long rows, int cols, float eps) {
  ROW_SETUP
  float4 r[NV];
  float s = 0.f;
#pragma unroll
  FOR_V { r[v] = ldx4(x + row * cols + COL); s += r[v].x + r[v].y + r[v].z + r[v].w; }
  const float mean = warp_sum(s) / cols;
  float q = 0.f;
#pragma unroll
  FOR_V {
    float4 d = make_float4(r[v].x - mean, r[v].y - mean, r[v].z - mean, r[v].w - mean);
    r[v] = d;
    q += dot4(d, d);
  }
  const float rstd = rsqrtf(warp_sum(q) / cols + eps);
#pragma unroll
  FOR_V { st4bf(y + row * cols + COL, add4(mul4(scl4(r[v], rstd), ld4(w + COL)), ld4(b + COL))); }
}

template <int NV>
__global__ void __launch_bounds__(256) layernorm_f32(const float* __restrict__ x, const float* __restrict__ w,
                                                     const float* __restrict__ b, bf16_t* __restrict__ y, long rows,
                                                     int cols, float eps) {
  layernorm_body<float, NV>(x, w, b, y, rows, cols, eps);
}
template <int NV>
__global__ void __launch_bounds__(256) layernorm_b16(const bf16_t* __restrict__ x, const float* __restrict__ w,
                                                     const float* __restrict__ b, bf16_t* __restrict__ y, long rows,
                                                     int cols, float eps) {
  layernorm_body<bf16_t, NV>(x, w, b, y, rows, cols, eps);
}

template <int NV>
__global__ void __launch_bounds__(256) rmsnorm_fwd_kernel(const float* __restrict__ x, long ldx, RowMap xmap,
                                                          const float* __restrict__ w, bf16_t* __restrict__ y,
                                                          float* __restrict__ rstd_out, long rows, int cols,
                                                          float eps) {
  ROW_SETUP
  const float* xr = x + map_row(xmap, row) * ldx;
  float4 r[NV];
  float q = 0.f;
#pragma unroll
  FOR_V { r[v] = ld4(xr + COL); q += dot4(r[v], r[v]); }
  const float rs = rsqrtf(warp_sum(q) / cols + eps);
  if (lane == 0 && rstd_out) rstd_out[row] = rs;
#pragma unroll
  FOR_V { st4bf(y + row * cols + COL, mul4(scl4(r[v], rs), onep(ld4(w + COL)))); }
}

template <int NV>
__global__ void __launch_bounds__(256) residual_norm_fwd_kernel(
    const bf16_t* __restrict__ t, const float* __restrict__ xi, const float* __restrict__ w_post,
    const float* __restrict__ w_next, float* __restrict__ xo, bf16_t* __restrict__ n,
    float* __restrict__ rstd_t, float* __restrict__ rstd_x, long rows, int cols, float eps) {
  ROW_SETUP
  float4 r[NV];
  float q = 0.f;
#pragma unroll
  FOR_V { r[v] = ld4bf(t + row * cols + COL); q += dot4(r[v], r[v]); }
  const float rs = rsqrtf(warp_sum(q) / cols + eps);
  if (lane == 0) rstd_t[row] = rs;
  float q2 = 0.f;
#pragma unroll
  FOR_V {
    float4 yv = bfr4(mul4(scl4(r[v], rs), onep(ld4(w_post + COL))));
    float4 xv = add4(ld4(xi + row * cols + COL), yv);
    st4(xo + row * cols + COL, xv);
    r[v] = xv;
    q2 += dot4(xv, xv);
  }
  if (!w_next) return;
  const float rs2 = rsqrtf(warp_sum(q2) / cols + eps);
  if (lane == 0) rstd_x[row] = rs2;
#pragma unroll
  FOR_V { st4bf(n + row * cols + COL, mul4(scl4(r[v], rs2), onep(ld4(w_next + COL)))); }
}

#define RMS_BWD_BODY(XV, DNV, RS, OUTEXPR)                                   \
  {                                                                           \
    float sdot = 0.f;                                                         \
    _Pragma("unroll") FOR_V { sdot += dot4(mul4(DNV[v], onep(ld4(w + COL))), XV[v]); } \
    sdot = warp_sum(sdot);                                                    \
    const float c3 = RS * RS * RS * sdot / cols;                              \
    _Pragma("unroll") FOR_V {                                                 \
      float4 dxv = add4(scl4(mul4(DNV[v], onep(ld4(w + COL))), RS), scl4(XV[v], -c3)); \
      OUTEXPR;                                                                \
    }                                                                         \
  }

template <typename TD, int NV>
PTK_DEV void rmsnorm_bwd_body(const float* __restrict__ x, const float* __restrict__ w, const float* __restrict__ rstd,
                              const TD* __restrict__ dn, const float* dacc, float* dx, long rows, int cols) {
  ROW_SETUP
  float4 xv[NV], dv[NV];
#pragma unroll
  FOR_V { xv[v] = ld4(x + row * cols + COL); dv[v] = ldx4(dn + row * cols + COL); }
  const float rs = rstd[row];
  RMS_BWD_BODY(xv, dv, rs, {
    float4 o = dacc ? add4(ld4(dacc + row * cols + COL), dxv) : dxv;
    st4(dx + row * cols + COL, o);
  })
}
template <int NV>
__global__ void __launch_bounds__(256) rmsnorm_bwd_f32_kernel(const float* __restrict__ x, const float* __restrict__ w,
                                                              const float* __restrict__ rstd, const float* __restrict__ dn,
                                                              const float* dacc, float* dx, long rows, int cols) {
  rmsnorm_bwd_body<float, NV>(x, w, rstd, dn, dacc, dx, rows, cols);
}
template <int NV>
__global__ void __launch_bounds__(256) rmsnorm_bwd_bdn_kernel(const float* __restrict__ x, const float* __restrict__ w,
                                                              const float* __restrict__ rstd, const bf16_t* __restrict__ dn,
                                                              const float* dacc, float* dx, long rows, int cols) {
  rmsnorm_bwd_body<bf16_t, NV>(x, w, rstd, dn, dacc, dx, rows, cols);
}

template <int NV>
__global__ void __launch_bounds__(256) rmsnorm_bwd_scatter_kernel(const float* __restrict__ x, RowMap xmap,
                                                                  const float* __restrict__ w,
                                                                  const float* __restrict__ rstd,
                                                                  const float* __restrict__ dn, float* dR,
                                                                  long rows, int cols) {
  ROW_SETUP
  const long xr = map_row(xmap, row);
  float4 xv[NV], dv[NV];
#pragma unroll
  FOR_V { xv[v] = ld4(x + xr * cols + COL); dv[v] = ld4(dn + row * cols + COL); }
  const float rs = rstd[row];
  RMS_BWD_BODY(xv, dv, rs, { st4(dR + xr * cols + COL, add4(ld4(dR + xr * cols + COL), dxv)); })
}

template <int NV>
PTK_DEV void post_norm_bwd_row(const float* dR, const bf16_t* t, const float* w, float rs, bf16_t* dt, int lane,
                               int cols) {
  float4 xv[NV], dv[NV];
#pragma unroll
  FOR_V { xv[v] = ld4bf(t + COL); dv[v] = bfr4(ld4(dR + COL)); }
  RMS_BWD_BODY(xv, dv, rs, { st4bf(dt + COL, dxv); })
}

template <typename TD, int NV>
PTK_DEV void residual_norm_bwd_body(
    const float* __restrict__ x2, const float* __restrict__ w_pre, const float* __restrict__ rstd_pre,
    const TD* __restrict__ dn, float* __restrict__ dR, const bf16_t* __restrict__ t,
    const float* __restrict__ w_post, const float* __restrict__ rstd_t, bf16_t* __restrict__ dt, long rows,
    int cols) {
  ROW_SETUP
  float4 nd[NV];
  {
    const float* w = w_pre;
    float4 xv[NV], dv[NV];
#pragma unroll
    FOR_V { xv[v] = ld4(x2 + row * cols + COL); dv[v] = ldx4(dn + row * cols + COL); }
    const float rs = rstd_pre[row];
    RMS_BWD_BODY(xv, dv, rs, {
      nd[v] = add4(ld4(dR + row * cols + COL), dxv);
      st4(dR + row * cols + COL, nd[v]);
    })
  }
  {
    const float* w = w_post;
    const float rs = rstd_t[row];
    float4 xv[NV], dv[NV];
#pragma unroll
    FOR_V { xv[v] = ld4bf(t + row * cols + COL); dv[v] = bfr4(nd[v]); }
    RMS_BWD_BODY(xv, dv, rs, { st4bf(dt + row * cols + COL, dxv); })
  }
}
template <int NV>
__global__ void __launch_bounds__(256) residual_norm_bwd_kernel(
    const float* __restrict__ x2, const float* __restrict__ w_pre, const float* __restrict__ rstd_pre,
    const float* __restrict__ dn, float* __restrict__ dR, const bf16_t* __restrict__ t,
    const float* __restrict__ w_post, const float* __restrict__ rstd_t, bf16_t* __restrict__ dt, long rows,
    int cols) {
  residual_norm_bwd_body<float, NV>(x2, w_pre, rstd_pre, dn, dR, t, w_post, rstd_t, dt, rows, cols);
}
template <int NV>
__global__ void __launch_bounds__(256) residual_norm_bwd_bdn_kernel(
    const float* __restrict__ x2, const float* __restrict__ w_pre, const float* __restrict__ rstd_pre,
    const bf16_t* __restrict__ dn, float* __restrict__ dR, const bf16_t* __restrict__ t,
    const float* __restrict__ w_post, const float* __restrict__ rstd_t, bf16_t* __restrict__ dt, long rows,
    int cols) {
  residual_norm_bwd_body<bf16_t, NV>(x2, w_pre, rstd_pre, dn, dR, t, w_post, rstd_t, dt, rows, cols);
}

#ifndef PTK_NWG_WAVES
#define PTK_NWG_WAVES 4
#endif
constexpr int NWG = PTK_NWG_WAVES;
template <int NV>
__global__ void __launch_bounds__(64 * NWG) residual_norm_bwd_wg_kernel(
    const float* __restrict__ x2, const float* __restrict__ w_pre, const float* __restrict__ rstd_pre,
    const bf16_t* __restrict__ dn, float* __restrict__ dR, const bf16_t* __restrict__ t,
    const float* __restrict__ w_post, const float* __restrict__ rstd_t, bf16_t* __restrict__ dt, long rows,
    int cols, float* __restrict__ part_pre, float* __restrict__ part_post) {
  __shared__ float4 red[NWG][NV][64];
  const int lane = threadIdx.x & 63, wv = threadIdx.x >> 6;
  const long row = (long)blockIdx.x * NWG + wv;
  const bool ok = row < rows;
#define NWG_SUM(PART)                                                                    \
  __syncthreads();                                                                       \
  if (wv == 0) {                                                                         \
    float* part = PART + (long)blockIdx.x * cols;                                        \
    _Pragma("unroll") FOR_V {                                                            \
      float4 a = red[0][v][lane];                                                        \
      _Pragma("unroll") for (int g = 1; g < NWG; ++g) a = add4(a, red[g][v][lane]);      \
      st4(part + COL, a);                                                                \
    }                                                                                    \
  }                                                                                      \
  __syncthreads();
  float4 nd[NV];
  if (ok) {
    const float* w = w_pre;
    float4 xv[NV], dv[NV];
#pragma unroll
    FOR_V { xv[v] = ld4(x2 + row * cols + COL); dv[v] = ld4bf(dn + row * cols + COL); }
    const float rs = rstd_pre[row];
#pragma unroll
    FOR_V { red[wv][v][lane] = scl4(mul4(dv[v], xv[v]), rs); }
    RMS_BWD_BODY(xv, dv, rs, {
      nd[v] = add4(ld4(dR + row * cols + COL), dxv);
      st4(dR + row * cols + COL, nd[v]);
    })
  } else {
#pragma unroll
    for (int v = 0; v < NV; ++v) red[wv][v][lane] = make_float4(0.f, 0.f, 0.f, 0.f);
  }
  NWG_SUM(part_pre)
  if (ok) {
    const float* w = w_post;
    const float rs = rstd_t[row];
    float4 xv[NV], dv[NV];
#pragma unroll
    FOR_V { xv[v] = ld4bf(t + row * cols + COL); dv[v] = bfr4(nd[v]); }
#pragma unroll
    FOR_V { red[wv][v][lane] = scl4(mul4(dv[v], xv[v]), rs); }
    RMS_BWD_BODY(xv, dv, rs, { st4bf(dt + row * cols + COL, dxv); })
  } else {
#pragma unroll
    for (int v = 0; v < NV; ++v) red[wv][v][lane] = make_float4(0.f, 0.f, 0.f, 0.f);
  }
  NWG_SUM(part_post)
#undef NWG_SUM
}

template <int NV>
__global__ void __launch_bounds__(256) post_norm_bwd_kernel(const float* __restrict__ dR, const bf16_t* __restrict__ t,
                                                            const float* __restrict__ w, const float* __restrict__ rstd_t,
                                                            bf16_t* __restrict__ dt, long rows, int cols) {
  ROW_SETUP
  post_norm_bwd_row<NV>(dR + row * cols, t + row * cols, w, rstd_t[row], dt + row * cols, lane, cols);
}

#define NORM_DISPATCH(KERNEL, ...)                                                                  \
  do {                                                                                              \
    switch ((cols + 255) / 256) {                                                                   \
      case 1: hipLaunchKernelGGL(KERNEL<1>, NORM_GRID, __VA_ARGS__); break;                         \
      case 2: hipLaunchKernelGGL(KERNEL<2>, NORM_GRID, __VA_ARGS__); break;                         \
      case 3: hipLaunchKernelGGL(KERNEL<3>, NORM_GRID, __VA_ARGS__); break;                         \
      case 4: hipLaunchKernelGGL(KERNEL<4>, NORM_GRID, __VA_ARGS__); break;                         \
      case 5: hipLaunchKernelGGL(KERNEL<5>, NORM_GRID, __VA_ARGS__); break;                         \
      case 6: hipLaunchKernelGGL(KERNEL<6>, NORM_GRID, __VA_ARGS__); break;                         \
      case 7: hipLaunchKernelGGL(KERNEL<7>, NORM_GRID, __VA_ARGS__); break;                         \
      case 8: hipLaunchKernelGGL(KERNEL<8>, NORM_GRID, __VA_ARGS__); break;                         \
      case 9: hipLaunchKernelGGL(KERNEL<9>, NORM_GRID, __VA_ARGS__); break;                         \
      case 10: hipLaunchKernelGGL(KERNEL<10>, NORM_GRID, __VA_ARGS__); break;                       \
      case 11: hipLaunchKernelGGL(KERNEL<11>, NORM_GRID, __VA_ARGS__); break;                       \
      default: hipLaunchKernelGGL(KERNEL<MAXV>, NORM_GRID, __VA_ARGS__); break;                     \
    }                                                                                               \
  } while (0)

static int check_cols(int cols) {
  if (cols <= 0 || cols % 4 || cols > 256 * MAXV) return set_error("norm: cols=%d unsupported", cols);
  return 0;
}
#define NORM_GRID dim3((unsigned)((rows + 3) / 4)), dim3(256), 0, st
#define RET_LAUNCH(name) return hipGetLastError() == hipSuccess ? 0 : set_error(name " launch failed")

int launch_layernorm(const float* x, const float* w, const float* b, bf16_t* y, int rows, int cols, float eps,
                     hipStream_t st) {
  if (check_cols(cols)) return -1;
  if (rows <= 0) return 0;
  NORM_DISPATCH(layernorm_f32, x, w, b, y, (long)rows, cols, eps);
  RET_LAUNCH("layernorm");
}
int launch_layernorm_bf16(const bf16_t* x, const float* w, const float* b, bf16_t* y, int rows, int cols, float eps,
                          hipStream_t st) {
  if (check_cols(cols)) return -1;
  if (rows <= 0) return 0;
  NORM_DISPATCH(layernorm_b16, x, w, b, y, (long)rows, cols, eps);
  RET_LAUNCH("layernorm_bf16");
}
int launch_rmsnorm_fwd(const float* x, long ldx, RowMap xmap, const float* w, bf16_t* y, float* rstd, int rows,
                       int cols, float eps, hipStream_t st) {
  if (check_cols(cols)) return -1;
  if (rows <= 0) return 0;
  NORM_DISPATCH(rmsnorm_fwd_kernel, x, ldx, xmap, w, y, rstd, (long)rows, cols, eps);
  RET_LAUNCH("rmsnorm_fwd");
}
int launch_residual_norm_fwd(const bf16_t* t, const float* xi, const float* w_post, const float* w_next, float* xo,
                             bf16_t* n, float* rstd_t, float* rstd_x, int rows, int cols, float eps,
                             hipStream_t st) {
  if (check_cols(cols)) return -1;
  if (rows <= 0) return 0;
  NORM_DISPATCH(residual_norm_fwd_kernel, t, xi, w_post, w_next, xo, n, rstd_t, rstd_x,
                     (long)rows, cols, eps);
  RET_LAUNCH("residual_norm_fwd");
}
int launch_rmsnorm_bwd_f32(const float* x, const float* w, const float* rstd, const float* dn, const float* dacc,
                           float* dx, int rows, int cols, hipStream_t st) {
  if (check_cols(cols)) return -1;
  if (rows <= 0) return 0;
  NORM_DISPATCH(rmsnorm_bwd_f32_kernel, x, w, rstd, dn, dacc, dx, (long)rows, cols);
  RET_LAUNCH("rmsnorm_bwd");
}
int launch_rmsnorm_bwd_bdn(const float* x, const float* w, const float* rstd, const bf16_t* dn, const float* dacc,
                           float* dx, int rows, int cols, hipStream_t st) {
  if (check_cols(cols)) return -1;
  if (rows <= 0) return 0;
  NORM_DISPATCH(rmsnorm_bwd_bdn_kernel, x, w, rstd, dn, dacc, dx, (long)rows, cols);
  RET_LAUNCH("rmsnorm_bwd_bdn");
}
int launch_residual_norm_bwd_bdn(const float* x2, const float* w_pre, const float* rstd_pre, const bf16_t* dn,
                                 float* dR, const bf16_t* t, const float* w_post, const float* rstd_t, bf16_t* dt,
                                 int rows, int cols, hipStream_t st) {
  if (check_cols(cols)) return -1;
  if (rows <= 0) return 0;
  NORM_DISPATCH(residual_norm_bwd_bdn_kernel, x2, w_pre, rstd_pre, dn, dR, t, w_post, rstd_t, dt, (long)rows, cols);
  RET_LAUNCH("residual_norm_bwd_bdn");
}
int residual_norm_bwd_wg_blocks(int rows) { return (rows + NWG - 1) / NWG; }
int launch_residual_norm_bwd_wg(const float* x2, const float* w_pre, const float* rstd_pre, const bf16_t* dn,
                                float* dR, const bf16_t* t, const float* w_post, const float* rstd_t, bf16_t* dt,
                                int rows, int cols, float* part_pre, float* part_post, hipStream_t st) {
  if (check_cols(cols)) return -1;
  if (rows <= 0) return 0;
#undef NORM_GRID
#define NORM_GRID dim3((unsigned)residual_norm_bwd_wg_blocks(rows)), dim3(64 * NWG), 0, st
  NORM_DISPATCH(residual_norm_bwd_wg_kernel, x2, w_pre, rstd_pre, dn, dR, t, w_post, rstd_t, dt, (long)rows, cols,
                part_pre, part_post);
#undef NORM_GRID
#define NORM_GRID dim3((unsigned)((rows + 3) / 4)), dim3(256), 0, st
  RET_LAUNCH("residual_norm_bwd_wg");
}
int launch_rmsnorm_bwd_scatter(const float* x, RowMap xmap, const float* w, const float* rstd, const float* dn,
                               float* dR, int rows, int cols, hipStream_t st) {
  if (check_cols(cols)) return -1;
  if (rows <= 0) return 0;
  NORM_DISPATCH(rmsnorm_bwd_scatter_kernel, x, xmap, w, rstd, dn, dR, (long)rows, cols);
  RET_LAUNCH("rmsnorm_bwd_scatter");
}
int launch_residual_norm_bwd(const float* x2, const float* w_pre, const float* rstd_pre, const float* dn, float* dR,
                             const bf16_t* t, const float* w_post, const float* rstd_t, bf16_t* dt, int rows,
                             int cols, hipStream_t st) {
  if (check_cols(cols)) return -1;
  if (rows <= 0) return 0;
  NORM_DISPATCH(residual_norm_bwd_kernel, x2, w_pre, rstd_pre, dn, dR, t, w_post, rstd_t, dt,
                     (long)rows, cols);
  RET_LAUNCH("residual_norm_bwd");
}
int launch_post_norm_bwd(const float* dR, const bf16_t* t, const float* w, const float* rstd_t, bf16_t* dt,
                         int rows, int cols, hipStream_t st) {
  if (check_cols(cols)) return -1;
  if (rows <= 0) return 0;
  NORM_DISPATCH(post_norm_bwd_kernel, dR, t, w, rstd_t, dt, (long)rows, cols);
  RET_LAUNCH("post_norm_bwd");
}

}
```

projectiontrainer_amd/csrc/ptk_internal.h:

```cpp
#pragma once
#include <hip/hip_runtime.h>
#include <stddef.h>
#include <stdint.h>

#include <type_traits>

#include "common.h"

namespace ptk {

int set_error(const char* fmt, ...);

#ifdef PTK_AB_ENV
}
#include <cstdlib>
namespace ptk {
inline int ab_env(const char* name, int dflt) { const char* e = getenv(name); return e && *e ? atoi(e) : dflt; }
#define PTK_AB(NAME, DFLT) ([] { static const int v_ = ::ptk::ab_env(NAME, DFLT); return v_; }())
#else
#define PTK_AB(NAME, DFLT) (DFLT)
#endif

enum Act { ACT_NONE = 0, ACT_GELU_TANH = 1, ACT_GELU_ERF = 2, ACT_GEGLU = 3,
           ACT_GELU_ERF_BWD = 4, ACT_GEGLU_BWD = 5 };
enum Out { OUT_BF16 = 0, OUT_F32 = 1, OUT_F32_BFR = 2 };

struct GemmArgs {
  const bf16_t* A = nullptr;
  const bf16_t* B = nullptr;
  void* C = nullptr;
  int M = 0, N = 0, K = 0;
  long lda = 0, ldb = 0, ldc = 0;
  int zin = 1;
  long sA0 = 0, sA1 = 0, sB0 = 0, sB1 = 0, sC0 = 0, sC1 = 0;
  float alpha = 1.f;
  const float* bias = nullptr;
  const float* rowadd = nullptr;
  int rowadd_period = 1;
  long ld_rowadd = 0;
  const float* resid = nullptr;
  long ld_resid = 0;
  const bf16_t* resid16 = nullptr;
  long ld_resid16 = 0;
  int bf16_linear = 0;
  bf16_t* aux = nullptr;
  bf16_t* aux2 = nullptr;
  long ld_aux = 0;
  const bf16_t* aux_in = nullptr;
  const bf16_t* aux_in2 = nullptr;
  long ld_aux_in = 0;
  RowMap amap{0, 0, 0, 0};
  RowMap cmap{0, 0, 0, 0};
  float* row_stats = nullptr;
  long ld_stats = 0;
  int stats_only = 0;
  void* tail_ws = nullptr;
  const bf16_t* B_kt = nullptr;
  int a_kt = 0, c_kt = 0, aux_kt = 0, aux_in_kt = 0;
};

enum GemmPath { GEMM_PATH_NT = 0, GEMM_PATH_BIG = 1, GEMM_PATH_BIG2 = 2, GEMM_PATH_W4 = 3, GEMM_PATH_NTB = 4,
                GEMM_PATH_P8SK = 5, GEMM_PATH_P8 = 6, GEMM_PATH_TN = 7, GEMM_NPATH = 9 };
int path_counts(int64_t* out, int reset);
int ktiled_counts(int64_t* out2, int reset);
int device_cus();

template <class F>
inline bool gemm_act_out(int act, int out, F&& f) {
#define PTK_ACT_OUT(ACT_, OUT_)                                                          \
  if (act == ACT_ && out == OUT_) {                                                      \
    f(std::integral_constant<int, ACT_>{}, std::integral_constant<int, OUT_>{});         \
    return true;                                                                         \
  }
  PTK_ACT_OUT(ACT_NONE, OUT_BF16)
  PTK_ACT_OUT(ACT_NONE, OUT_F32)
  PTK_ACT_OUT(ACT_NONE, OUT_F32_BFR)
  PTK_ACT_OUT(ACT_GELU_TANH, OUT_BF16)
  PTK_ACT_OUT(ACT_GELU_ERF, OUT_BF16)
  PTK_ACT_OUT(ACT_GEGLU, OUT_BF16)
  PTK_ACT_OUT(ACT_GELU_ERF_BWD, OUT_BF16)
  PTK_ACT_OUT(ACT_GEGLU_BWD, OUT_BF16)
#undef PTK_ACT_OUT
  return false;
}

constexpr int W4 = 256;
constexpr int W4_KT = 64;
// ... 22 lines not shown
  P8Tail tail;
  bool single_round = false;
};
GemmPlan gemm_plan(const GemmArgs& a, int act, int out, int batch, const GemmPlanEnv& env);
constexpr bool bkt_act(int act) { return act != ACT_GELU_ERF && act != ACT_GELU_ERF_BWD; }
long kstep_tile_offset(long row, long k, long K);
bool b_ktiled_ok(const GemmArgs& a, const GemmPlan& plan, int act, int batch);
bool a_ktiled_ok(const GemmArgs& a, const GemmPlan& plan, int act, int out, int batch, bool lean_epi);
bool c_ktiled_ok(const GemmArgs& a, const GemmPlan& plan, int act, int out, int batch, bool lean_epi);
bool gemm_ktiled_pair(const GemmArgs& prod, int pact, const GemmArgs& cons, long part_floats, const GemmPlanEnv& env,
                      bool enabled, bool factors);
int a_ktiled_mode();
int launch_gemm(const GemmArgs& a, int act, int out, int batch, hipStream_t st, const GemmPlan* planned = nullptr);
struct GemmSplitPlan {
  int slices = 1, kc = 0, rem = 0;
  bool tail_ws = false;
  GemmPlan direct;
};
GemmSplitPlan gemm_split_plan(const GemmArgs& a, int out, long part_floats, const GemmPlanEnv& env);
bool w4_supported(const GemmArgs& a, int act, int out);
int launch_gemm_w4(const GemmArgs& a, int act, int out, hipStream_t st, int max_grid);
double w4_round_fill(long M, long N, int ncu);
bool p8_supported(const GemmArgs& a, int act, int out);
int launch_gemm_p8(const GemmArgs& a, int act, int out, hipStream_t st, const P8Tail& tail, int tm = 256);
int p8_tile_height(const GemmArgs& a, int act, int out, int ncu);
int launch_gemm_p8_kslices(const GemmArgs& a, int slices, hipStream_t st);
int gemm_p8_kslices(const GemmArgs& a, int slices, hipStream_t st);
bool lean_epilogue_candidate(const GemmArgs& a, bool lean_epi);
bool lean_epilogue_ok(const GemmArgs& a, int act, int out, uint32_t& c_bytes, bool lean_epi);
bool lean_epilogue_enabled();
bool tn_supported(const GemmArgs& a, int out, int slices, bool lean_epi);
int tn_slices(const GemmArgs& a, long part_floats, const GemmPlanEnv& env);
P8Tail tn_tail_plan(const GemmArgs& a, void* slab, int ncu);
size_t tn_slab_bytes();
int launch_gemm_tn(const GemmArgs& a, int out, int slices, void* slab, hipStream_t st, long k_rows = -1);
int gemm_tn(const GemmArgs& a, int out, int slices, void* slab, hipStream_t st, long k_rows = -1);
int wgrad_tn_enabled();
size_t p8_tail_scratch_bytes();
size_t p8_tail_scratch_bytes_models();
size_t p8_slab_bytes(long G);
bool streamk_enabled();
P8Tail p8_tail_plan_ws(const GemmArgs& a, long ntile, long G, void* slab, long max_t0, long max_t1);
P8Tail p8_tail_plan(const GemmArgs& a, int act, int out, const GemmPlanEnv& env);
void* tail_scope();
struct TailScratchScope {
  void* prev;
  int status = 0;
  TailScratchScope(void* ws, hipStream_t st);
  ~TailScratchScope();
};
bool stage_timers_on();
void stage_begin(const char* name, hipStream_t st);
int stage_end(hipStream_t st);
struct StageScope {
  hipStream_t st;
  bool on;
  StageScope(const char* name, hipStream_t s) : st(s), on(stage_timers_on()) { if (on) stage_begin(name, s); }
  ~StageScope() { if (on) (void)stage_end(st); }
};
struct StageSeq {
  hipStream_t st;
  bool on, open = false;
  explicit StageSeq(hipStream_t s) : st(s), on(stage_timers_on()) {}
  void next(const char* name) {
    if (!on) return;
    if (open) (void)stage_end(st);
    stage_begin(name, st);
    open = true;
  }
  ~StageSeq() { if (on && open) (void)stage_end(st); }
};
void timer_enable(int on);
void force_small_tiles(int mode);
int timer_read(int cls, double* total_ms, int* count);

int launch_layernorm(const float* x, const float* w, const float* b, bf16_t* y, int rows, int cols,
                     float eps, hipStream_t st);
int launch_layernorm_bf16(const bf16_t* x, const float* w, const float* b, bf16_t* y, int rows, int cols,
                          float eps, hipStream_t st);
int launch_rmsnorm_fwd(const float* x, long ldx, RowMap xmap, const float* w, bf16_t* y, float* rstd,
                       int rows, int cols, float eps, hipStream_t st);
int launch_residual_norm_fwd(const bf16_t* t, const float* xi, const float* w_post, const float* w_next,
                             float* xo, bf16_t* n, float* rstd_t, float* rstd_x, int rows, int cols,
                             float eps, hipStream_t st);
int launch_rmsnorm_bwd_f32(const float* x, const float* w, const float* rstd, const float* dn,
                           const float* dacc, float* dx, int rows, int cols, hipStream_t st);
int launch_residual_norm_bwd(const float* x2, const float* w_pre, const float* rstd_pre, const float* dn,
                             float* dR, const bf16_t* t, const float* w_post, const float* rstd_t,
                             bf16_t* dt, int rows, int cols, hipStream_t st);
int launch_post_norm_bwd(const float* dR, const bf16_t* t, const float* w, const float* rstd_t, bf16_t* dt,
                         int rows, int cols, hipStream_t st);
int launch_rmsnorm_bwd_bdn(const float* x, const float* w, const float* rstd, const bf16_t* dn, const float* dacc,
                           float* dx, int rows, int cols, hipStream_t st);
int launch_residual_norm_bwd_bdn(const float* x2, const float* w_pre, const float* rstd_pre, const bf16_t* dn,
                                 float* dR, const bf16_t* t, const float* w_post, const float* rstd_t, bf16_t* dt,
                                 int rows, int cols, hipStream_t st);
int residual_norm_bwd_wg_blocks(int rows);
int launch_residual_norm_bwd_wg(const float* x2, const float* w_pre, const float* rstd_pre, const bf16_t* dn,
                                float* dR, const bf16_t* t, const float* w_post, const float* rstd_t, bf16_t* dt,
                                int rows, int cols, float* part_pre, float* part_post, hipStream_t st);
int launch_rmsnorm_bwd_scatter(const float* x, RowMap xmap, const float* w, const float* rstd,
                               const float* dn, float* dR, int rows, int cols, hipStream_t st);

struct AttnShape {
  int B, S, Hq, Hkv, D;
  const int32_t* pos = nullptr;
};
int launch_qknorm_rope_fwd(const bf16_t* qkv, const float* qw, const float* kw, const float* cos_t,
                           const float* sin_t, AttnShape s, float eps, bf16_t* Q, bf16_t* K, bf16_t* V,
                           float* rstd_q, float* rstd_k, hipStream_t st);
int launch_qknorm_rope_bwd(const bf16_t* qkv, const float* qw, const float* kw, const float* cos_t,
                           const float* sin_t, AttnShape s, const float* rstd_q, const float* rstd_k,
                           const bf16_t* dQ, const bf16_t* dK, const bf16_t* dV, bf16_t* dqkv,
                           hipStream_t st, const struct FlashBwdArgs* dkv = nullptr);
struct MaskSpec {
  int rows_per_batch;
  int qdiv;
  int zdiv;
  int causal;
  int window;
  const int32_t* key_valid;
  int key_len;
};
int launch_softmax_fwd(const float* S, bf16_t* P, int nz, int rows, int cols, long ld, MaskSpec m,
                       hipStream_t st);
int launch_softmax_bwd(const bf16_t* P, const float* dP, bf16_t* dS, int nrows, int cols, long ld,
                       float scale, hipStream_t st);

struct FlashArgs {
  const bf16_t* Q = nullptr;
  const bf16_t* K = nullptr;
  const bf16_t* V = nullptr;
  bf16_t* O = nullptr;
  float* lse = nullptr;
  int rows = 0, nkeys = 0, D = 0;
  long ldq = 0, ldk = 0, ldo = 0;
  int zin = 1, zdiv = 1;
  long sQ0 = 0, sQ1 = 0, sK0 = 0, sK1 = 0, sO0 = 0, sO1 = 0;
  RowMap qmap{0, 0, 0, 0}, omap{0, 0, 0, 0};
  int qdiv = 1, causal = 0, window = 0;
  const int32_t* key_valid = nullptr;
  float scale = 1.f;
  int variant = 0;
};
int launch_attn_fwd(const FlashArgs& a, int nz, hipStream_t st);
struct FlashBwdArgs {
  const bf16_t* Q = nullptr;
  const bf16_t* K = nullptr;
  const bf16_t* V = nullptr;
  const bf16_t* O = nullptr;
  const bf16_t* dO = nullptr;
  const float* lse = nullptr;
  float* delta = nullptr;
  bf16_t* dQ = nullptr;
  bf16_t* dK = nullptr;
  bf16_t* dV = nullptr;
  int rows = 0, nkeys = 0, D = 0;
  int zin = 1, zdiv = 1;
  long ldo = 0, sO0 = 0, sO1 = 0;
  RowMap omap{0, 0, 0, 0};
  int qdiv = 1, causal = 0, window = 0;
  const int32_t* key_valid = nullptr;
  float scale = 1.f;
  float* dkv_part = nullptr;
  size_t dkv_part_bytes = 0;
  int dkv_target = 0, nz = 1;
  int dkv_items = 0;
  unsigned char dkv_item_slab[128], dkv_item_piece[128];
  int dkv_deferred = 0;
};

constexpr int DKV_KEYS = 128, DKV_CH = 32;
__host__ __device__ inline void dkv_slab_chunks(const FlashBwdArgs& a, int s, int& c_lo, int& c_hi) {
  int r_lo = 0, r_hi = a.rows;
  if (a.causal) {
    r_lo = min(a.rows, s * DKV_KEYS * a.qdiv);
    if (a.window > 0) r_hi = min(a.rows, (s * DKV_KEYS + DKV_KEYS + a.window - 1) * a.qdiv);
  }
  c_lo = r_lo / DKV_CH;
  c_hi = max(c_lo, (r_hi + DKV_CH - 1) / DKV_CH);
}
__host__ __device__ inline int dkv_pieces(const FlashBwdArgs& a, int s) {
  int lo, hi;
  dkv_slab_chunks(a, s, lo, hi);
  const int n = hi - lo;
  return (a.dkv_target <= 0 || n <= a.dkv_target) ? 1 : (n + a.dkv_target - 1) / a.dkv_target;
}
__host__ __device__ inline int dkv_part_base(const FlashBwdArgs& a, int s) {
  int base = 0;
  for (int t = 0; t < s; ++t) {
    const int pt = dkv_pieces(a, t);
    if (pt > 1) base += pt;
  }
  return base;
}

int launch_attn_bwd(const FlashBwdArgs& a, int nz, hipStream_t st, FlashBwdArgs* defer = nullptr);
size_t attn_bwd_workspace_bytes(const FlashBwdArgs& a, int nz);

int launch_transpose(const bf16_t* in, long ld_in, long sin0, long sin1, int zin, bf16_t* out, long ld_out,
                     long sout0, long sout1, int nz, int rows, int cols, int rows_pad, hipStream_t st);
int launch_pack_kstep_tiles(const bf16_t* src, bf16_t* dst, int N, int K, hipStream_t st);
int launch_im2col(const bf16_t* px, bf16_t* out, int B, int C, int H, int W, int P, hipStream_t st);
int launch_cast_f32_bf16(const float* in, bf16_t* out, long n, hipStream_t st);
int launch_build_llm_inputs(const bf16_t* embed, const int64_t* ids, int B, int T, int Nv, int S, int Spad,
                            int H, float scale_bf16, int pad_id, float* x, int32_t* key_valid,
                            hipStream_t st);
int launch_ce_fwd_bwd(bf16_t* logits, long ld, int R, int V, const int64_t* targets, float* row_loss,
                      const float* gscale, hipStream_t st);
int launch_ce_stats_fwd_bwd(bf16_t* logits, long ld, int R, int V, const float* stats, long ld_stats,
                            const int64_t* targets, float* row_loss, const float* gscale, hipStream_t st);
int launch_count_valid(const int64_t* labels, int n, float loss_scale, float* gscale, float* count,
                       hipStream_t st);
int launch_loss_reduce(const float* row_loss, int R, const float* count, float* loss, hipStream_t st);
int launch_gather_dy(const float* dx, int B, int N, int Spad, int H, bf16_t* dy, hipStream_t st);
int launch_colsum_bf16(const bf16_t* x, int rows, int cols, float* out, float* partial, long part_floats,
                       hipStream_t st);
int launch_sumsq_partial(const float* x, long n, float* partial, int nparts, hipStream_t st);
int launch_clip_adamw(float* p, const float* g, float* m, float* v, long n, const float* partial,
                      int nparts, float grad_scale, float max_norm, float lr, float b1, float b2,
                      float eps, float wd, int step, float* norm_out, hipStream_t st);
int launch_sum_partials(const float* part, int nsplit, long n, float* out, hipStream_t st);
int launch_zero(void* p, size_t bytes, hipStream_t st);
int launch_geglu_bwd(const bf16_t* dh, const bf16_t* g, const bf16_t* u, bf16_t* dgu, long M, int I, hipStream_t st);
int launch_fill_normal_bf16(bf16_t* out, long n, uint64_t seed, float std, float mean, hipStream_t st);

int launch_gen_prompt(const float* src, long ld_b, int B, int P, int Pp, int H, float* x, int32_t* kv, hipStream_t st);
int launch_kv_append(const bf16_t* src, long src_z, bf16_t* dst, long dst_z, int Z, int p0, int n, int D,
                     hipStream_t st);
int launch_gen_sample(const bf16_t* logits, long ld, int B, int V, int do_sample, int top_k, float temperature,
                      float top_p, uint64_t seed, int step, long eos_id, long pad_id, int32_t* finished, int64_t* out,
                      long ld_out, int64_t* next, hipStream_t st);
bool skinny_supported(int M, int N, int K, long lda, long ldb, long ldc, int act);
size_t skinny_part_bytes(int M, int N, int K);
int launch_gemm_skinny(const bf16_t* A, long lda, const bf16_t* B, long ldb, bf16_t* C, long ldc, int M, int N,
                       int K, int act, float* part, size_t part_bytes, hipStream_t st);
int launch_dec_prompt(const float* src, long ld_b, const int32_t* mask, long mask_ld, int repeat, int rows, int P,
                      int Pp, int H, float* x, int32_t* kv, hipStream_t st);
int launch_dec_positions(const int32_t* kv, int rows, int P, int Pp, int Smax, int32_t* pos, int32_t* slot_ok,
                         int32_t* nvalid, hipStream_t st);
int launch_dec_step_prep(int32_t* slot_ok, const int32_t* nvalid, int rows, int Smax, int p0, int t, int k_lo, int nk,
                         int32_t* pos, int32_t* kmask, hipStream_t st);
int launch_dec_gather_rows(const void* in, void* out, const int32_t* src, int rows, long row_bytes, hipStream_t st);
int launch_dec_gather_i32(const int32_t* in, int32_t* out, const int32_t* src, int rows, hipStream_t st);
int launch_dec_repeat_index(int32_t* src, int rows, int repeat, hipStream_t st);
struct PenArgs {
  const int64_t* history;
  long ld_hist;
  int n_hist;
  float penalty;
  int32_t* status;
};
inline bool pen_active(const PenArgs& pa) { return pa.n_hist > 0 && pa.penalty != 1.f; }
int pen_validate(const char* who, const PenArgs& pa);
int gen_sample_validate(const char* who, int V, int do_sample, int top_k, float temperature, float top_p,
                        const PenArgs& pa);
int beam_candidates_validate(int batch, int K, int V, int do_sample, int top_k, float top_p, float temperature,
                             int min_keep, int n_cand, const void* ws, size_t ws_bytes, const PenArgs& pa);
int pen_status_check(const char* who, int32_t* status, hipStream_t st);
int launch_gen_sample_pen(const bf16_t* logits, long ld, int B, int V, int do_sample, int top_k, float temperature,
                          float top_p, uint64_t seed, int step, long eos_id, long pad_id, int32_t* finished,
// ... 45 lines not shown
```

projectiontrainer_amd/kernels.py:

```python
from __future__ import annotations

import os

import torch

from . import _lib as L
from ._lib import check, ptr


def _require_cuda(*ts):
    for t in ts:
        if t is not None and not t.is_cuda:
            raise L.PtkError("libptk ops need HIP device tensors (no CPU fallback)")


def _bits(t):
    return ptr(t)


def gemm(A, B, *, C=None, out_dtype=torch.bfloat16, act=L.ACT_NONE, alpha=1.0, bias=None, rowadd=None,
         resid=None, aux=None, aux2=None, aux_in=None, aux_in2=None, M=None, N=None, K=None,
         lda=None, ldb=None, ldc=None, batch=1, batch_inner=1, strides=(0, 0, 0, 0, 0, 0),
         amap=(0, 0, 0, 0), cmap=(0, 0, 0, 0), out_mode=None, resid16=None, bf16_linear=False, tail_ws=None,
         B_kt=None, A_kt=False, C_kt=False, aux_kt=False, aux_in_kt=False):
# ... 101 lines not shown
    check(L.lib().ptk_cross_entropy(ptr(logits), logits.stride(0), R, V, ptr(targets), ptr(row_loss), ptr(gscale),
                                    L.stream_ptr(logits.device)), "cross_entropy")
    return row_loss


def transpose_rows(x, rows, rows_pad, map_g=0, map_gs=0, map_off=0, ld_out=None):
    if x.dtype != torch.bfloat16 or x.dim() != 2 or x.stride(1) != 1:
        raise L.PtkError("transpose_rows: x must be a 2-D bf16 tensor with unit column stride")
    cols = x.shape[1]
    ld = rows_pad if ld_out is None else ld_out
    out = torch.empty((cols, ld), dtype=torch.bfloat16, device=x.device)
    check(L.lib().ptk_transpose_rows_bf16(ptr(x), x.stride(0), map_g, map_gs, map_off, rows, cols, ptr(out), ld,
                                          rows_pad, L.stream_ptr(x.device)), "transpose_rows")
    return out


def weight_grad(dy, x, grad, rows=None, ymap=(0, 0, 0), xmap=(0, 0, 0), part=None, mode=0):
    for t in (dy, x, grad):
        if t.dtype != torch.bfloat16 or t.dim() != 2 or t.stride(1) != 1:
            raise L.PtkError("weight_grad: dy, x, grad must be 2-D bf16 tensors with unit column stride")
    Ny, Nx = dy.shape[1], x.shape[1]
    if tuple(grad.shape) != (Ny, Nx) or grad.stride(0) != Nx:
        raise L.PtkError("weight_grad: grad must be a contiguous [Ny, Nx] tensor")
    rows = dy.shape[0] if rows is None else rows
    kp = (rows + 63) // 64 * 64
    ta = tb = None
    if mode != 2:
        ta = torch.empty((Ny, kp), dtype=torch.bfloat16, device=dy.device)
        tb = torch.empty((Nx, kp), dtype=torch.bfloat16, device=dy.device)
    pf = 0 if part is None else part.numel()
    check(L.lib().ptk_weight_grad_bf16(ptr(dy), dy.stride(0), ymap[0], ymap[1], ymap[2], Ny, ptr(x), x.stride(0),
                                       xmap[0], xmap[1], xmap[2], Nx, rows, ptr(grad), ptr(ta), ptr(tb), ptr(part),
                                       pf, mode, L.stream_ptr(dy.device)), "weight_grad")
    return grad


def transpose(x, rows_pad=None, out=None):
    squeeze = x.dim() == 2
    x3 = x.unsqueeze(0) if squeeze else x
    Z, rows, cols = x3.shape
    rp = rows if rows_pad is None else rows_pad
    if out is None:
        out = torch.empty((Z, cols, rp), dtype=x.dtype, device=x.device)
    else:
        if tuple(out.shape[-2:]) != (cols, rp) or out.numel() != Z * cols * rp or not out.is_contiguous():
            raise L.PtkError(f"transpose: out {tuple(out.shape)} does not hold [{Z}, {cols}, {rp}]")
        out = out.view(Z, cols, rp)
    check(L.lib().ptk_transpose_bf16(ptr(x3), x3.stride(1), ptr(out), rp, Z, x3.stride(0), cols * rp, rows, cols, rp,
                                     L.stream_ptr(x.device)), "transpose")
    return out[0] if squeeze else out


def pack_kstep_tiles(w):
    _require_cuda(w)
    if w.dim() != 2 or w.dtype != torch.bfloat16 or not w.is_contiguous():
        raise L.PtkError("pack_kstep_tiles: a contiguous bf16 [N, K] matrix")
    out = torch.empty_like(w)
    check(L.lib().ptk_pack_kstep_tiles_bf16(ptr(w), ptr(out), w.shape[0], w.shape[1], L.stream_ptr(w.device)),
          "pack_kstep_tiles")
    return out


def frozen_kstep_tiles(w):
    if os.environ.get("PTK_B_KTILED", "1") == "0" or w.shape[0] % 16 or w.shape[1] % 32:
        return None
    return pack_kstep_tiles(w)


def cast_bf16(x, out=None):
    out = torch.empty(x.shape, dtype=torch.bfloat16, device=x.device) if out is None else out
    check(L.lib().ptk_cast_f32_bf16(ptr(x), ptr(out), x.numel(), L.stream_ptr(x.device)), "cast")
    return out


def fill_normal_(t, seed, std=0.02, mean=0.0):
    assert t.dtype == torch.bfloat16 and t.is_contiguous()
    check(L.lib().ptk_fill_normal_bf16(ptr(t), t.numel(), seed & (2**64 - 1), std, mean, L.stream_ptr(t.device)),
          "fill_normal")
    return t


def flash_attn(Q, K, V, O, *, rows, nkeys, head_dim, ldq, ldk, ldo, batch, batch_inner=1, zdiv=1,
               strides=(0, 0, 0, 0, 0, 0), qmap=(0, 0, 0, 0), omap=(0, 0, 0, 0), qdiv=1, causal=False,
               window=0, key_valid=None, scale=1.0, lse=None):
    _require_cuda(Q, K, V, O)
    d = L.FlashDesc()
    d.Q, d.K, d.V, d.O, d.lse = ptr(Q), ptr(K), ptr(V), ptr(O), ptr(lse)
    d.rows, d.nkeys, d.head_dim = rows, nkeys, head_dim
    d.ldq, d.ldk, d.ldo = ldq, ldk, ldo
    d.batch, d.batch_inner, d.zdiv = batch, batch_inner, zdiv
    d.sQ0, d.sQ1, d.sK0, d.sK1, d.sO0, d.sO1 = strides
    d.qmap, d.omap = L.RowMap(*qmap), L.RowMap(*omap)
    d.qdiv, d.causal, d.window = qdiv, int(causal), window
    d.key_valid, d.scale = ptr(key_valid), scale
    check(L.lib().ptk_flash_attn_fwd(d, L.stream_ptr(Q.device)), "flash_attn_fwd")
    return O


def flash_attn_bwd(Q, K, V, O, dO, lse, *, rows, nkeys, head_dim, batch, batch_inner=1, zdiv=1, ldo=None,
                   sO=(0, 0), omap=(0, 0, 0, 0), qdiv=1, causal=False, window=0, key_valid=None, scale=1.0,
                   split=True):
    _require_cuda(Q, K, V, O, dO, lse)
    dQ, dK, dV = torch.empty_like(Q), torch.empty_like(K), torch.empty_like(V)
    delta = torch.empty(batch * rows, dtype=torch.float32, device=Q.device)
    d = L.FlashBwdDesc()
    d.Q, d.K, d.V, d.O, d.dO, d.lse, d.delta = ptr(Q), ptr(K), ptr(V), ptr(O), ptr(dO), ptr(lse), ptr(delta)
    d.dQ, d.dK, d.dV = ptr(dQ), ptr(dK), ptr(dV)
    d.rows, d.nkeys, d.head_dim = rows, nkeys, head_dim
    d.batch, d.batch_inner, d.zdiv = batch, batch_inner, zdiv
    d.ldo = head_dim if ldo is None else ldo
    d.sO0, d.sO1 = sO
    d.omap = L.RowMap(*omap)
    d.qdiv, d.causal, d.window = qdiv, int(causal), window
    d.key_valid, d.scale = ptr(key_valid), scale
    ws = None
    if split:
        nb = L.lib().ptk_flash_bwd_workspace_bytes(d)
        if nb:
            ws = torch.empty(nb, dtype=torch.uint8, device=Q.device)
            d.workspace, d.workspace_bytes = ptr(ws), nb
    check(L.lib().ptk_flash_attn_bwd(d, L.stream_ptr(Q.device)), "flash_attn_bwd")
    return dQ, dK, dV


def sample_next_token(logits, *, do_sample=False, top_k=0, temperature=1.0, top_p=1.0, seed=0, step=0,
                      eos_token_id=-1, pad_token_id=0, finished=None, history=None, repetition_penalty=1.0):
    _require_cuda(logits, finished, history)
    if logits.dim() != 2 or logits.dtype != torch.bfloat16 or logits.stride(1) != 1:
        raise L.PtkError("sample_next_token: logits must be bf16 [B, V] with contiguous rows")
    if finished is not None and (finished.dtype != torch.int32 or not finished.is_contiguous()):
        raise L.PtkError("sample_next_token: finished must be contiguous int32 [B]")
    B, V = logits.shape
    out = torch.empty(B, dtype=torch.int64, device=logits.device)
    n = L.lib().ptk_sample_next_token_workspace_bytes(B)
    ws = torch.empty(n, dtype=torch.uint8, device=logits.device)
    n_hist = 0 if history is None else int(history.shape[1])
    if history is not None and (history.dtype != torch.int64 or history.stride(1) != 1):
        raise L.PtkError("sample_next_token: history must be int64 with contiguous rows")
    check(L.lib().ptk_sample_next_token(ptr(logits), logits.stride(0), B, V, int(bool(do_sample)), int(top_k or 0),
                                        float(temperature), float(top_p), int(seed) & ((1 << 64) - 1), int(step),
                                        int(eos_token_id), int(pad_token_id), ptr(finished), ptr(history),
                                        history.stride(0) if history is not None else 0, n_hist,
                                        float(repetition_penalty), ptr(out), ptr(ws), n, L.stream_ptr(logits.device)),
          "ptk_sample_next_token")
    return out
```

Measured before the change: 321.9 images/sec.

## Trim Gemma last layer to loss rows only in frozen-LM fwd/bwd

When the language model is frozen, the final decoder layer now computes only the rows that feed the loss (the text positions after the vision tokens). It does this for attention queries (a row_lo offset), the output projection, the residual norms and the MLP, in both forward and backward. Vision-token rows in that layer cannot affect the loss, so their matmuls and attention blocks are wasted work. The change threads row maps through the norm kernels and adds a row_lo option to flash attention fwd/bwd, which zeroes dO rows that are not computed. It also lets the trimmed GEMM reuse the full-size split-K plan. The extra plumbing and per-slab chunk tables make the attention descriptors larger and add more validation paths.

```diff
diff --git a/include/ptk.h b/include/ptk.h
--- a/include/ptk.h
+++ b/include/ptk.h
@@ -62,6 +62,8 @@
 int ptk_gemm_ktiled_pair(const ptk_gemm_desc* producer, const ptk_gemm_desc* consumer, int ncu, int64_t part_floats,
                          int train);
 int ptk_a_ktiled_reload(void);
+int ptk_last_layer_rows_reload(void);
+int ptk_last_layer_rows_counts(int64_t* out2, int reset);
 int ptk_gemm(const ptk_gemm_desc* d, void* stream);
 int64_t ptk_kstep_tile_offset(int64_t row, int64_t k, int64_t K);
 int ptk_pack_kstep_tiles_bf16(const void* src, void* dst, int N, int K, void* stream);
@@ -119,6 +121,7 @@
   int qdiv, causal, window;
   const int32_t* key_valid;
   float scale;
+  int row_lo;
 } ptk_flash_desc;
 int ptk_flash_attn_fwd(const ptk_flash_desc* d, void* stream);
 
@@ -135,6 +138,7 @@
   float scale;
   void* workspace;
   int64_t workspace_bytes;
+  int row_lo;
 } ptk_flash_bwd_desc;
 size_t ptk_flash_bwd_workspace_bytes(const ptk_flash_bwd_desc* d);
 int ptk_flash_attn_bwd(const ptk_flash_bwd_desc* d, void* stream);
diff --git a/projectiontrainer_amd/_lib.py b/projectiontrainer_amd/_lib.py
--- a/projectiontrainer_amd/_lib.py
+++ b/projectiontrainer_amd/_lib.py
@@ -44,7 +44,7 @@
                 ("sQ0", c_int64), ("sQ1", c_int64), ("sK0", c_int64), ("sK1", c_int64),
                 ("sO0", c_int64), ("sO1", c_int64), ("qmap", RowMap), ("omap", RowMap),
                 ("qdiv", c_int), ("causal", c_int), ("window", c_int), ("key_valid", c_void_p),
-                ("scale", c_float)]
+                ("scale", c_float), ("row_lo", c_int)]
 
 
 class FlashBwdDesc(C.Structure):
@@ -54,7 +54,7 @@
                 ("batch", c_int), ("batch_inner", c_int), ("zdiv", c_int),
                 ("ldo", c_int64), ("sO0", c_int64), ("sO1", c_int64), ("omap", RowMap),
                 ("qdiv", c_int), ("causal", c_int), ("window", c_int), ("key_valid", c_void_p),
-                ("scale", c_float), ("workspace", c_void_p), ("workspace_bytes", c_int64)]
+                ("scale", c_float), ("workspace", c_void_p), ("workspace_bytes", c_int64), ("row_lo", c_int)]
 
 
 class SiglipConfigC(C.Structure):
@@ -171,6 +171,8 @@
     "ptk_gemm_ktiled_counts": (c_int, [c_void_p, c_int]),
     "ptk_gemm_ktiled_pair": (c_int, [C.POINTER(GemmDesc), C.POINTER(GemmDesc), c_int, c_int64, c_int]),
     "ptk_a_ktiled_reload": (c_int, []),
+    "ptk_last_layer_rows_reload": (c_int, []),
+    "ptk_last_layer_rows_counts": (c_int, [c_void_p, c_int]),
     "ptk_stage_timers_enable": (c_int, [c_int]),
     "ptk_stage_begin": (c_int, [C.c_char_p, c_void_p]),
     "ptk_stage_end": (c_int, [c_void_p]),
@@ -289,6 +291,12 @@
     return {(GEMM_PATHS[i // 8], i % 8): int(v) for i, v in enumerate(buf) if v}
 
 
+def last_layer_rows_counts(reset=False):
+    buf = (C.c_int64 * 2)()
+    check(lib().ptk_last_layer_rows_counts(buf, int(reset)), "last_layer_rows_counts")
+    return int(buf[0]), int(buf[1])
+
+
 def gemm_ktiled_counts(reset=False):
     buf = (C.c_int64 * 2)()
     check(lib().ptk_gemm_ktiled_counts(buf, int(reset)), "gemm_ktiled_counts")
diff --git a/projectiontrainer_amd/csrc/attn.hip b/projectiontrainer_amd/csrc/attn.hip
--- a/projectiontrainer_amd/csrc/attn.hip
+++ b/projectiontrainer_amd/csrc/attn.hip
@@ -151,6 +151,9 @@
         const float mul = which == 0 ? fb.scale : 1.f;
 #pragma unroll
         for (int e = 0; e < EPL; ++e) gy[i][e] = f2bf(acc[e] * mul);
+      } else if (h < sh.Hq && s * G < fb.row_lo) {
+#pragma unroll
+        for (int e = 0; e < EPL; ++e) gy[i][e] = 0;
       } else {
 #pragma unroll
         for (int e = 0; e < EPL; ++e) gy[i][e] = dy[e];
@@ -314,6 +317,8 @@
       return set_error("qknorm_rope_bwd: deferred dK/dV plan does not match the shape");
     fb = *dkv;
   }
+  fb.row_lo = dkv ? dkv->row_lo : 0;
+  if (fb.row_lo % (s.Hq / s.Hkv)) return set_error("qknorm_rope_bwd: row_lo %d splits a position's query heads", fb.row_lo);
   const long waves = (long)s.B * s.S;
   dim3 grid((unsigned)((waves + 3) / 4));
   QKR_DISPATCH(qknorm_rope_bwd_kernel, qkv, qw, kw, cos_t, sin_t, s, rstd_q, rstd_k, dQ, dK, dV, dqkv, fb)
diff --git a/projectiontrainer_amd/csrc/capi.cpp b/projectiontrainer_amd/csrc/capi.cpp
--- a/projectiontrainer_amd/csrc/capi.cpp
+++ b/projectiontrainer_amd/csrc/capi.cpp
@@ -202,6 +202,7 @@
   a.qmap = to_map(d->qmap); a.omap = to_map(d->omap);
   a.qdiv = d->qdiv > 0 ? d->qdiv : 1; a.causal = d->causal; a.window = d->window;
   a.key_valid = d->key_valid; a.scale = d->scale;
+  a.row_lo = d->row_lo;
   return launch_attn_fwd(a, d->batch > 0 ? d->batch : 1, ST);
 }
 
@@ -217,6 +218,7 @@
   a.key_valid = d->key_valid; a.scale = d->scale;
   a.dkv_part = (float*)d->workspace;
   a.dkv_part_bytes = d->workspace && d->workspace_bytes > 0 ? (size_t)d->workspace_bytes : 0;
+  a.row_lo = d->row_lo;
   return a;
 }
 
diff --git a/projectiontrainer_amd/csrc/flash.hip b/projectiontrainer_amd/csrc/flash.hip
--- a/projectiontrainer_amd/csrc/flash.hip
+++ b/projectiontrainer_amd/csrc/flash.hip
@@ -2133,9 +2133,15 @@
   return span;
 }
 
-static void dkv_plan(FlashBwdArgs& a, int nz, int& nslab, long& npieces, long& nsplit) {
+static void dkv_plan(FlashBwdArgs& a, int nz, int& nslab, long& npieces, long& nsplit, long max_ns = -1) {
   a.nz = nz;
   nslab = (a.nkeys + DKV_KEYS - 1) / DKV_KEYS;
+  for (int s = 0; s < nslab && s < 128; ++s) dkv_slab_range(a, s, a.dkv_slab_c[s][0], a.dkv_slab_c[s][1]);
+  if (nslab > 128) {
+    npieces = nslab;
+    nsplit = 0;
+    return;
+  }
   long total = 0;
   for (int s = 0; s < nslab; ++s) {
     int lo, hi;
@@ -2148,6 +2154,11 @@
     long items = 0;
     a.dkv_target = t;
     for (int s = 0; s < nslab; ++s) items += dkv_pieces(a, s);
+    if (max_ns >= 0) {
+      long slots = 0;
+      for (int s = 0; s < nslab; ++s) slots += dkv_pieces(a, s) > 1 ? dkv_pieces(a, s) : 0;
+      if (slots > max_ns) return 129L;
+    }
     return items;
   };
   int base = (int)std::max(4L, (total * nz + ncu - 1) / ncu);
@@ -2192,6 +2203,16 @@
   return (size_t)ns * nz * 2 * DKV_KEYS * 256 * sizeof(float);
 }
 
+bool attn_row_lo_ok(const FlashBwdArgs& a) {
+  return a.D == 256 && (a.nkeys + 31) / 32 <= FA_MAXT && a.row_lo >= 0 && a.row_lo < a.rows;
+}
+
+__global__ void __launch_bounds__(256) attn_zero_rows_kernel(bf16_t* p, long zstride, long off, long n16) {
+  const long i = (long)blockIdx.x * 256 + threadIdx.x;
+  if (i >= n16) return;
+  reinterpret_cast<uint4*>(p + blockIdx.y * zstride + off)[i] = make_uint4(0u, 0u, 0u, 0u);
+}
+
 int launch_attn_bwd(const FlashBwdArgs& a, int nz, hipStream_t st, FlashBwdArgs* defer) {
   if (defer) {
     *defer = a;
@@ -2201,6 +2222,8 @@
   if (a.rows % 64 || a.nkeys % 64) return set_error("attn_bwd: rows (%d) and keys (%d) must be multiples of 64",
                                                    a.rows, a.nkeys);
   if (a.ldo & 7) return set_error("attn_bwd: O stride must be a multiple of 8");
+  if (a.row_lo != 0 && (!attn_row_lo_ok(a) || (a.row_hi != 0 && a.row_hi <= a.row_lo)))
+    return set_error("attn_bwd: row_lo %d is not served at head_dim %d, %d rows, %d keys", a.row_lo, a.D, a.rows, a.nkeys);
   const dim3 gd((unsigned)(((long)nz * a.rows + 15) / 16)), gq((unsigned)((long)((a.rows + 127) / 128) * nz)),
       gk((unsigned)(a.nkeys / 64), (unsigned)nz);
   switch (a.D) {
@@ -2213,7 +2236,8 @@
       FlashBwdArgs b = a;
       int nslab;
       long np, ns;
-      dkv_plan(b, nz, nslab, np, ns);
+      const size_t slot_bytes = (size_t)nz * 2 * DKV_KEYS * 256 * sizeof(float);
+      dkv_plan(b, nz, nslab, np, ns, a.row_lo > 0 ? (long)(b.dkv_part ? b.dkv_part_bytes / slot_bytes : 0) : -1);
       if (ns > 0 && (!b.dkv_part || b.dkv_part_bytes < (size_t)ns * nz * 2 * DKV_KEYS * 256 * sizeof(float))) {
         b.dkv_target = 0;
         np = nslab;
@@ -2225,7 +2249,18 @@
       const bool dq_new = (a.nkeys + 31) / 32 <= FA_MAXT;
       if (dq_new) {
         const bool persist = PTK_AB("PTK_ATTN_PERSIST", 1) != 0;
-        const long nblk = (long)gq.x;
+        const int blk_lo = a.row_lo / 128;
+        const long nblk = (long)gq.x - (long)blk_lo * nz;
+        if (a.row_lo > blk_lo * 128) {
+          const long n16 = (long)(a.row_lo - blk_lo * 128) * 256 / 8;
+          hipLaunchKernelGGL(attn_zero_rows_kernel, dim3((unsigned)((n16 + 255) / 256), (unsigned)nz), dim3(256), 0, st,
+                             const_cast<bf16_t*>(a.dO), (long)a.rows * 256, (long)blk_lo * 128 * 256, n16);
+        }
+        if (a.row_lo > 0 && a.row_hi > 0 && a.row_hi < a.rows) {
+          const long n16 = (long)(a.rows - a.row_hi) * 256 / 8;
+          hipLaunchKernelGGL(attn_zero_rows_kernel, dim3((unsigned)((n16 + 255) / 256), (unsigned)nz), dim3(256), 0, st,
+                             const_cast<bf16_t*>(a.dO), (long)a.rows * 256, (long)a.row_hi * 256, n16);
+        }
         const long g = persist ? std::min<long>(nblk, device_cus()) : nblk;
         hipLaunchKernelGGL(attn_bwd_dq256w_kernel, dim3((unsigned)g), dim3(256), 0, st, b, nz, (int)nblk);
       }
@@ -2272,8 +2307,9 @@
         hipLaunchKernelGGL((attn_fwd_kernel<256, 1>), grid, dim3(512), 0, st, a);
       else {
         const bool persist = PTK_AB("PTK_ATTN_PERSIST", 1) != 0;
-        const long g = persist ? std::min<long>(nblk, device_cus()) : nblk;
-        hipLaunchKernelGGL(attn_fwd256w_kernel, dim3((unsigned)g), dim3(256), 0, st, a, nz, (int)nblk);
+        const long nrun = nblk - (long)(std::min(std::max(a.row_lo, 0), a.rows - 1) / 128) * nz;
+        const long g = persist ? std::min<long>(nrun, device_cus()) : nrun;
+        hipLaunchKernelGGL(attn_fwd256w_kernel, dim3((unsigned)g), dim3(256), 0, st, a, nz, (int)nrun);
       }
       break;
     }
diff --git a/projectiontrainer_amd/csrc/models.cpp b/projectiontrainer_amd/csrc/models.cpp
--- a/projectiontrainer_amd/csrc/models.cpp
+++ b/projectiontrainer_amd/csrc/models.cpp
@@ -102,6 +102,26 @@
 extern "C" int ptk_a_ktiled_reload(void) {
   g_a_ktiled = -1;
   return a_ktiled_mode();
+}
+namespace {
+int g_last_layer_rows = -1;
+int64_t g_ll_counts[2] = {0, 0};
+int last_layer_rows_mode() {
+  if (g_last_layer_rows < 0) {
+    const char* e = getenv("PTK_LAST_LAYER_ROWS");
+    g_last_layer_rows = e && e[0] == '0' ? 0 : 1;
+  }
+  return g_last_layer_rows;
+}
+}
+extern "C" int ptk_last_layer_rows_reload(void) {
+  g_last_layer_rows = -1;
+  return last_layer_rows_mode();
+}
+extern "C" int ptk_last_layer_rows_counts(int64_t* out2, int reset) {
+  if (out2) { out2[0] = g_ll_counts[0]; out2[1] = g_ll_counts[1]; }
+  if (reset) g_ll_counts[0] = g_ll_counts[1] = 0;
+  return 0;
 }
 namespace {
 
@@ -251,9 +271,16 @@
   return w;
 }
 
-int gemm_split(const GemmArgs& a, int out, float* part, long part_floats, hipStream_t st) {
+int gemm_split(const GemmArgs& a, int out, float* part, long part_floats, hipStream_t st,
+               const GemmArgs* like = nullptr) {
   const GemmPlanEnv env = gemm_plan_env();
-  const GemmSplitPlan sp = gemm_split_plan(a, out, part ? part_floats : 0, env);
+  GemmSplitPlan sp = gemm_split_plan(a, out, part ? part_floats : 0, env);
+  if (like) {
+    const GemmSplitPlan lp = gemm_split_plan(*like, out, part ? part_floats : 0, env);
+    if (lp.kc != 0 && a.K == like->K && (long)(lp.slices + (lp.rem ? 1 : 0)) * a.M * a.N <= part_floats) {
+      sp.kc = lp.kc; sp.slices = lp.slices; sp.rem = lp.rem;
+    }
+  }
   if (sp.kc != 0 && a.a_kt) return set_error("gemm_split: a K split cannot read a k-step-tiled A");
   if (sp.kc == 0) {
     GemmArgs b = a;
@@ -473,6 +500,15 @@
 
   const RowMap lossmap{Tl, 0, Sp, Nv - 1 + lo};
 
+  const int row_lo = (Nv - 1 + lo) * G;
+  bool trim = false;
+  if (!train && nl >= 1 && D == 256 && row_lo > 0 && last_layer_rows_mode()) {
+    FlashBwdArgs probe;
+    probe.rows = SG; probe.nkeys = Sp; probe.D = D; probe.row_lo = row_lo;
+    trim = attn_row_lo_ok(probe);
+  }
+  if (nl >= 1) ++g_ll_counts[trim ? 0 : 1];
+
   auto mlp_fwd = [&](int l, GemmArgs& g, GemmArgs& d) {
     const ptk_gemma3_layer& L = wt->layers[l];
     g = gemm(train ? w.L[l].xn_ff : w.xn, H, L.wgu, H, train ? w.L[l].h : w.h, I, M, 2 * I, H, L.wgu_kt);
@@ -511,6 +547,7 @@
     bf16_t* xin = train ? sv.xn_in : w.xn;
     bf16_t* xff = train ? sv.xn_ff : w.xn;
     bf16_t* hh = train ? sv.h : w.h;
+    const bool tl = trim && l == nl - 1;
     sq.next("gemma.fwd.attn");
     CK(gemm_split(gemm(xin, H, L.wqkv, H, sv.qkv, Dqkv, M, Dqkv, H, L.wqkv_kt), OUT_BF16, w.skpart, w.sk_floats, st));
     CK(launch_qknorm_rope_fwd(sv.qkv, L.q_norm, L.k_norm, cs, sn, ash, eps, sv.Q, sv.K, sv.V, sv.rstd_q, sv.rstd_k,
@@ -528,12 +565,22 @@
       fa.qdiv = G; fa.causal = 1; fa.window = sliding ? c->sliding_window : 0;
       fa.key_valid = w.key_valid;
       fa.scale = scale;
+      if (tl) fa.row_lo = row_lo;
       StageScope sf("gemma.fwd.flash", st);
       CK(launch_attn_fwd(fa, Z, st));
     }
-    CK(gemm_split(gemm(sv.O, Dq, L.wo, Dq, sv.ao, H, M, H, Dq, L.wo_kt), OUT_BF16, w.skpart, w.sk_floats, st));
-    CK(launch_residual_norm_fwd(sv.ao, w.x[l], L.ln_post_attn, L.ln_pre_ff, sv.x2, xff, sv.rstd_ao, sv.rstd_pre, M,
-                                H, eps, st));
+    if (tl) {
+      GemmArgs g = gemm(sv.O, Dq, L.wo, Dq, sv.ao, H, R, H, Dq, L.wo_kt);
+      g.amap = lossmap;
+      const GemmArgs full = gemm(sv.O, Dq, L.wo, Dq, sv.ao, H, M, H, Dq, L.wo_kt);
+      CK(gemm_split(g, OUT_BF16, w.skpart, w.sk_floats, st, &full));
+      CK(launch_residual_norm_fwd(sv.ao, w.x[l], L.ln_post_attn, L.ln_pre_ff, sv.x2, xff, sv.rstd_ao, sv.rstd_pre, R,
+                                  H, eps, st, lossmap));
+    } else {
+      CK(gemm_split(gemm(sv.O, Dq, L.wo, Dq, sv.ao, H, M, H, Dq, L.wo_kt), OUT_BF16, w.skpart, w.sk_floats, st));
+      CK(launch_residual_norm_fwd(sv.ao, w.x[l], L.ln_post_attn, L.ln_pre_ff, sv.x2, xff, sv.rstd_ao, sv.rstd_pre, M,
+                                  H, eps, st));
+    }
     sq.next("gemma.fwd.mlp");
     if (l + 1 < nl) {
       GemmArgs g, d;
@@ -544,23 +591,24 @@
       CK(gemm_split(d, OUT_BF16, w.skpart, w.sk_floats, st));
     } else {
       GemmArgs g = gemm(xff, H, L.wgu, H, hh, I, R, 2 * I, H, L.wgu_kt);
-      g.amap = lossmap;
+      if (!tl) g.amap = lossmap;
       g.aux = sv.glu_a; g.aux2 = sv.glu_b; g.ld_aux = I;
       CK(launch_gemm(g, ACT_GEGLU, OUT_BF16, 1, st));
-      CK(launch_zero(sv.dn, (size_t)M * H * sizeof(bf16_t), st));
+      if (!tl) CK(launch_zero(sv.dn, (size_t)M * H * sizeof(bf16_t), st));
       GemmArgs g2 = gemm(hh, I, L.wd, I, sv.dn, H, R, H, I, L.wd_kt);
-      g2.cmap = lossmap;
+      if (!tl) g2.cmap = lossmap;
       CK(launch_gemm(g2, ACT_NONE, OUT_BF16, 1, st));
     }
     const float* wnext = (l + 1 < nl) ? wt->layers[l + 1].ln_in : nullptr;
     float* rnext = (l + 1 < nl) ? w.L[l + 1].rstd_in : nullptr;
     bf16_t* xnext = (train && l + 1 < nl) ? w.L[l + 1].xn_in : w.xn;
-    CK(launch_residual_norm_fwd(sv.dn, sv.x2, L.ln_post_ff, wnext, w.x[l + 1], xnext, sv.rstd_dn, rnext, M, H, eps,
-                                st));
-  }
+    CK(launch_residual_norm_fwd(sv.dn, sv.x2, L.ln_post_ff, wnext, w.x[l + 1], xnext, sv.rstd_dn, rnext, tl ? R : M,
+                                H, eps, st));
+  }
+  const RowMap xlmap = trim ? ident : lossmap;
 
   sq.next("gemma.lm_head_ce");
-  CK(launch_rmsnorm_fwd(w.x[nl], H, lossmap, wt->final_norm, w.xf, w.rstd_f, R, H, eps, st));
+  CK(launch_rmsnorm_fwd(w.x[nl], H, xlmap, wt->final_norm, w.xf, w.rstd_f, R, H, eps, st));
   {
     GemmArgs g = gemm(w.xf, H, wt->embed, H, w.logits, V, R, V, H);
     if (w.ce_stats && !ce_two_pass()) {
@@ -598,7 +646,7 @@
   }
   float* dR = bt->dx;
   CK(launch_zero(dR, (size_t)M * H * 4, st));
-  CK(launch_rmsnorm_bwd_scatter(w.x[nl], lossmap, wt->final_norm, w.rstd_f, w.dxf, dR, R, H, st));
+  CK(launch_rmsnorm_bwd_scatter(w.x[nl], xlmap, wt->final_norm, w.rstd_f, w.dxf, dR, R, H, st, &lossmap));
   if (train)
     CK(launch_rms_wgrad(w.x[nl], H, lossmap, w.rstd_f, w.dxf, H, 1, R, H, (bf16_t*)gr->final_norm, w.wpart, st));
 
@@ -609,10 +657,11 @@
     const bool sliding = (l + 1) % c->sliding_pattern != 0;
     const float* cs = sliding ? wt->rope_cos_local : wt->rope_cos_global;
     const float* sn = sliding ? wt->rope_sin_local : wt->rope_sin_global;
-    const bool last = l == nl - 1;
+    const bool last = l == nl - 1, tl = trim && last;
     sq.next("gemma.bwd.mlp");
     if (last) {
-      CK(launch_post_norm_bwd(dR, sv.dn, L.ln_post_ff, sv.rstd_dn, w.dao, M, H, st));
+      if (tl) CK(launch_post_norm_bwd(dR, sv.dn, L.ln_post_ff, sv.rstd_dn, w.dao, R, H, st, lossmap));
+      else CK(launch_post_norm_bwd(dR, sv.dn, L.ln_post_ff, sv.rstd_dn, w.dao, M, H, st));
       if (train)
         CK(launch_rms_wgrad_bx(sv.dn, H, ident, sv.rstd_dn, dR, H, 1, M, H, (bf16_t*)GL->ln_post_ff, w.wpart, st));
     }
@@ -639,29 +688,34 @@
       }
     } else {
       GemmArgs g = gemm(w.dao, H, L.wd_t, H, w.h, I, R, I, H, L.wd_t_kt);
-      g.amap = lossmap;
+      if (!tl) g.amap = lossmap;
       CK(launch_gemm(g, ACT_NONE, OUT_BF16, 1, st));
       CK(launch_geglu_bwd(w.h, sv.glu_a, sv.glu_b, w.dgu, R, I, st));
       if (train) CK(weight_grad(w.dgu, 2 * I, ident, 2 * I, sv.xn_ff, H, lossmap, H, R, w.TA, w.TB, GL->wgu, w.skpart, w.sk_floats, st));
-      CK(launch_zero(w.dtmp, (size_t)M * H * sizeof(bf16_t), st));
+      if (!tl) CK(launch_zero(w.dtmp, (size_t)M * H * sizeof(bf16_t), st));
       GemmArgs g2 = gemm(w.dgu, 2 * I, L.wgu_t, 2 * I, w.dtmp, H, R, H, 2 * I, L.wgu_t_kt);
-      g2.cmap = lossmap;
+      if (!tl) g2.cmap = lossmap;
       CK(launch_gemm(g2, ACT_NONE, OUT_BF16, 1, st));
     }
     sq.next("gemma.bwd.attn");
-    CK(residual_norm_bwd_grads(sv.x2, L.ln_pre_ff, sv.rstd_pre, w.dtmp, dR, sv.ao, L.ln_post_attn, sv.rstd_ao, w.dao,
-                               M, H, train ? (bf16_t*)GL->ln_pre_ff : nullptr,
-                               train ? (bf16_t*)GL->ln_post_attn : nullptr, w.wpart, st));
+    if (tl)
+      CK(launch_residual_norm_bwd_bdn(sv.x2, L.ln_pre_ff, sv.rstd_pre, w.dtmp, dR, sv.ao, L.ln_post_attn, sv.rstd_ao,
+                                      w.dao, R, H, st, lossmap));
+    else
+      CK(residual_norm_bwd_grads(sv.x2, L.ln_pre_ff, sv.rstd_pre, w.dtmp, dR, sv.ao, L.ln_post_attn, sv.rstd_ao, w.dao,
+                                 M, H, train ? (bf16_t*)GL->ln_pre_ff : nullptr,
+                                 train ? (bf16_t*)GL->ln_post_attn : nullptr, w.wpart, st));
     if (train)
       CK(weight_grad(w.dao, H, ident, H, sv.O, Dq, ident, Dq, M, w.TA, w.TB, GL->wo, w.skpart, w.sk_floats, st));
     {
-      GemmArgs g = gemm(w.dao, H, L.wo_t, H, w.dO, (long)G * D, M, G * D, H, L.wo_t_kt);
+      GemmArgs g = gemm(w.dao, H, L.wo_t, H, w.dO, (long)G * D, tl ? R : M, G * D, H, L.wo_t_kt);
       g.sB0 = (long)G * D * H; g.sC0 = (long)Sp * G * D;
-      g.cmap = RowMap{Sp, 0, (long)Hkv * Sp, 0};
+      g.cmap = tl ? RowMap{Tl, 0, (long)Hkv * Sp, Nv - 1 + lo} : RowMap{Sp, 0, (long)Hkv * Sp, 0};
       CK(launch_gemm(g, ACT_NONE, OUT_BF16, Hkv, st));
     }
     FlashBwdArgs dkv_plan;
     dkv_plan.dkv_deferred = 0;
+    dkv_plan.row_lo = tl ? row_lo : 0;
     {
       FlashBwdArgs fb;
       fb.Q = sv.Q; fb.K = sv.K; fb.V = sv.V; fb.O = sv.O; fb.dO = w.dO; fb.lse = sv.lse; fb.delta = w.delta;
@@ -674,6 +728,8 @@
       fb.key_valid = w.key_valid;
       fb.scale = scale;
       fb.dkv_part = w.dkv_part; fb.dkv_part_bytes = w.dkv_part_bytes;
+      fb.row_lo = tl ? row_lo : 0;
+      fb.row_hi = tl ? (Nv - 1 + T) * G : 0;
       StageScope sf("gemma.bwd.flash", st);
       CK(launch_attn_bwd(fb, Z, st, (dkv_reduce_split() || train) ? nullptr : &dkv_plan));
     }
diff --git a/projectiontrainer_amd/csrc/norm.hip b/projectiontrainer_amd/csrc/norm.hip
--- a/projectiontrainer_amd/csrc/norm.hip
+++ b/projectiontrainer_amd/csrc/norm.hip
@@ -89,8 +89,9 @@
 __global__ void __launch_bounds__(256) residual_norm_fwd_kernel(
     const bf16_t* __restrict__ t, const float* __restrict__ xi, const float* __restrict__ w_post,
     const float* __restrict__ w_next, float* __restrict__ xo, bf16_t* __restrict__ n,
-    float* __restrict__ rstd_t, float* __restrict__ rstd_x, long rows, int cols, float eps) {
-  ROW_SETUP
+    float* __restrict__ rstd_t, float* __restrict__ rstd_x, long rows, int cols, float eps, RowMap ximap) {
+  ROW_SETUP
+  const float* xir = xi + map_row(ximap, row) * cols;
   float4 r[NV];
   float q = 0.f;
 #pragma unroll
@@ -101,7 +102,7 @@
 #pragma unroll
   FOR_V {
     float4 yv = bfr4(mul4(scl4(r[v], rs), onep(ld4(w_post + COL))));
-    float4 xv = add4(ld4(xi + row * cols + COL), yv);
+    float4 xv = add4(ld4(xir + COL), yv);
     st4(xo + row * cols + COL, xv);
     r[v] = xv;
     q2 += dot4(xv, xv);
@@ -153,17 +154,17 @@
 
 template <int NV>
 __global__ void __launch_bounds__(256) rmsnorm_bwd_scatter_kernel(const float* __restrict__ x, RowMap xmap,
-                                                                  const float* __restrict__ w,
+                                                                  RowMap dmap, const float* __restrict__ w,
                                                                   const float* __restrict__ rstd,
                                                                   const float* __restrict__ dn, float* dR,
                                                                   long rows, int cols) {
   ROW_SETUP
-  const long xr = map_row(xmap, row);
+  const long xr = map_row(xmap, row), dr = map_row(dmap, row);
   float4 xv[NV], dv[NV];
 #pragma unroll
   FOR_V { xv[v] = ld4(x + xr * cols + COL); dv[v] = ld4(dn + row * cols + COL); }
   const float rs = rstd[row];
-  RMS_BWD_BODY(xv, dv, rs, { st4(dR + xr * cols + COL, add4(ld4(dR + xr * cols + COL), dxv)); })
+  RMS_BWD_BODY(xv, dv, rs, { st4(dR + dr * cols + COL, add4(ld4(dR + dr * cols + COL), dxv)); })
 }
 
 template <int NV>
@@ -180,8 +181,9 @@
     const float* __restrict__ x2, const float* __restrict__ w_pre, const float* __restrict__ rstd_pre,
     const TD* __restrict__ dn, float* __restrict__ dR, const bf16_t* __restrict__ t,
     const float* __restrict__ w_post, const float* __restrict__ rstd_t, bf16_t* __restrict__ dt, long rows,
-    int cols) {
-  ROW_SETUP
+    int cols, RowMap rmap) {
+  ROW_SETUP
+  float* dRr = dR + map_row(rmap, row) * cols;
   float4 nd[NV];
   {
     const float* w = w_pre;
@@ -190,8 +192,8 @@
     FOR_V { xv[v] = ld4(x2 + row * cols + COL); dv[v] = ldx4(dn + row * cols + COL); }
     const float rs = rstd_pre[row];
     RMS_BWD_BODY(xv, dv, rs, {
-      nd[v] = add4(ld4(dR + row * cols + COL), dxv);
-      st4(dR + row * cols + COL, nd[v]);
+      nd[v] = add4(ld4(dRr + COL), dxv);
+      st4(dRr + COL, nd[v]);
     })
   }
   {
@@ -209,15 +211,16 @@
     const float* __restrict__ dn, float* __restrict__ dR, const bf16_t* __restrict__ t,
     const float* __restrict__ w_post, const float* __restrict__ rstd_t, bf16_t* __restrict__ dt, long rows,
     int cols) {
-  residual_norm_bwd_body<float, NV>(x2, w_pre, rstd_pre, dn, dR, t, w_post, rstd_t, dt, rows, cols);
+  residual_norm_bwd_body<float, NV>(x2, w_pre, rstd_pre, dn, dR, t, w_post, rstd_t, dt, rows, cols,
+                                    RowMap{0, 0, 0, 0});
 }
 template <int NV>
 __global__ void __launch_bounds__(256) residual_norm_bwd_bdn_kernel(
     const float* __restrict__ x2, const float* __restrict__ w_pre, const float* __restrict__ rstd_pre,
     const bf16_t* __restrict__ dn, float* __restrict__ dR, const bf16_t* __restrict__ t,
     const float* __restrict__ w_post, const float* __restrict__ rstd_t, bf16_t* __restrict__ dt, long rows,
-    int cols) {
-  residual_norm_bwd_body<bf16_t, NV>(x2, w_pre, rstd_pre, dn, dR, t, w_post, rstd_t, dt, rows, cols);
+    int cols, RowMap rmap) {
+  residual_norm_bwd_body<bf16_t, NV>(x2, w_pre, rstd_pre, dn, dR, t, w_post, rstd_t, dt, rows, cols, rmap);
 }
 
 #ifndef PTK_NWG_WAVES
@@ -283,9 +286,10 @@
 template <int NV>
 __global__ void __launch_bounds__(256) post_norm_bwd_kernel(const float* __restrict__ dR, const bf16_t* __restrict__ t,
                                                             const float* __restrict__ w, const float* __restrict__ rstd_t,
-                                                            bf16_t* __restrict__ dt, long rows, int cols) {
-  ROW_SETUP
-  post_norm_bwd_row<NV>(dR + row * cols, t + row * cols, w, rstd_t[row], dt + row * cols, lane, cols);
+                                                            bf16_t* __restrict__ dt, long rows, int cols,
+                                                            RowMap rmap) {
+  ROW_SETUP
+  post_norm_bwd_row<NV>(dR + map_row(rmap, row) * cols, t + row * cols, w, rstd_t[row], dt + row * cols, lane, cols);
 }
 
 #define NORM_DISPATCH(KERNEL, ...)                                                                  \
@@ -336,11 +340,11 @@
 }
 int launch_residual_norm_fwd(const bf16_t* t, const float* xi, const float* w_post, const float* w_next, float* xo,
                              bf16_t* n, float* rstd_t, float* rstd_x, int rows, int cols, float eps,
-                             hipStream_t st) {
+                             hipStream_t st, RowMap ximap) {
   if (check_cols(cols)) return -1;
   if (rows <= 0) return 0;
   NORM_DISPATCH(residual_norm_fwd_kernel, t, xi, w_post, w_next, xo, n, rstd_t, rstd_x,
-                     (long)rows, cols, eps);
+                     (long)rows, cols, eps, ximap);
   RET_LAUNCH("residual_norm_fwd");
 }
 int launch_rmsnorm_bwd_f32(const float* x, const float* w, const float* rstd, const float* dn, const float* dacc,
@@ -359,10 +363,11 @@
 }
 int launch_residual_norm_bwd_bdn(const float* x2, const float* w_pre, const float* rstd_pre, const bf16_t* dn,
                                  float* dR, const bf16_t* t, const float* w_post, const float* rstd_t, bf16_t* dt,
-                                 int rows, int cols, hipStream_t st) {
-  if (check_cols(cols)) return -1;
-  if (rows <= 0) return 0;
-  NORM_DISPATCH(residual_norm_bwd_bdn_kernel, x2, w_pre, rstd_pre, dn, dR, t, w_post, rstd_t, dt, (long)rows, cols);
+                                 int rows, int cols, hipStream_t st, RowMap rmap) {
+  if (check_cols(cols)) return -1;
+  if (rows <= 0) return 0;
+  NORM_DISPATCH(residual_norm_bwd_bdn_kernel, x2, w_pre, rstd_pre, dn, dR, t, w_post, rstd_t, dt, (long)rows, cols,
+                rmap);
   RET_LAUNCH("residual_norm_bwd_bdn");
 }
 int residual_norm_bwd_wg_blocks(int rows) { return (rows + NWG - 1) / NWG; }
@@ -380,10 +385,10 @@
   RET_LAUNCH("residual_norm_bwd_wg");
 }
 int launch_rmsnorm_bwd_scatter(const float* x, RowMap xmap, const float* w, const float* rstd, const float* dn,
-                               float* dR, int rows, int cols, hipStream_t st) {
-  if (check_cols(cols)) return -1;
-  if (rows <= 0) return 0;
-  NORM_DISPATCH(rmsnorm_bwd_scatter_kernel, x, xmap, w, rstd, dn, dR, (long)rows, cols);
+                               float* dR, int rows, int cols, hipStream_t st, const RowMap* dmap) {
+  if (check_cols(cols)) return -1;
+  if (rows <= 0) return 0;
+  NORM_DISPATCH(rmsnorm_bwd_scatter_kernel, x, xmap, dmap ? *dmap : xmap, w, rstd, dn, dR, (long)rows, cols);
   RET_LAUNCH("rmsnorm_bwd_scatter");
 }
 int launch_residual_norm_bwd(const float* x2, const float* w_pre, const float* rstd_pre, const float* dn, float* dR,
@@ -396,10 +401,10 @@
   RET_LAUNCH("residual_norm_bwd");
 }
 int launch_post_norm_bwd(const float* dR, const bf16_t* t, const float* w, const float* rstd_t, bf16_t* dt,
-                         int rows, int cols, hipStream_t st) {
-  if (check_cols(cols)) return -1;
-  if (rows <= 0) return 0;
-  NORM_DISPATCH(post_norm_bwd_kernel, dR, t, w, rstd_t, dt, (long)rows, cols);
+                         int rows, int cols, hipStream_t st, RowMap rmap) {
+  if (check_cols(cols)) return -1;
+  if (rows <= 0) return 0;
+  NORM_DISPATCH(post_norm_bwd_kernel, dR, t, w, rstd_t, dt, (long)rows, cols, rmap);
   RET_LAUNCH("post_norm_bwd");
 }
 
diff --git a/projectiontrainer_amd/csrc/ptk_internal.h b/projectiontrainer_amd/csrc/ptk_internal.h
--- a/projectiontrainer_amd/csrc/ptk_internal.h
+++ b/projectiontrainer_amd/csrc/ptk_internal.h
@@ -3,6 +3,7 @@
 #include <stddef.h>
 #include <stdint.h>
 
+#include <algorithm>
 #include <type_traits>
 
 #include "common.h"
@@ -191,25 +192,26 @@
                        int rows, int cols, float eps, hipStream_t st);
 int launch_residual_norm_fwd(const bf16_t* t, const float* xi, const float* w_post, const float* w_next,
                              float* xo, bf16_t* n, float* rstd_t, float* rstd_x, int rows, int cols,
-                             float eps, hipStream_t st);
+                             float eps, hipStream_t st, RowMap ximap = RowMap{0, 0, 0, 0});
 int launch_rmsnorm_bwd_f32(const float* x, const float* w, const float* rstd, const float* dn,
                            const float* dacc, float* dx, int rows, int cols, hipStream_t st);
 int launch_residual_norm_bwd(const float* x2, const float* w_pre, const float* rstd_pre, const float* dn,
                              float* dR, const bf16_t* t, const float* w_post, const float* rstd_t,
                              bf16_t* dt, int rows, int cols, hipStream_t st);
 int launch_post_norm_bwd(const float* dR, const bf16_t* t, const float* w, const float* rstd_t, bf16_t* dt,
-                         int rows, int cols, hipStream_t st);
+                         int rows, int cols, hipStream_t st, RowMap rmap = RowMap{0, 0, 0, 0});
 int launch_rmsnorm_bwd_bdn(const float* x, const float* w, const float* rstd, const bf16_t* dn, const float* dacc,
                            float* dx, int rows, int cols, hipStream_t st);
 int launch_residual_norm_bwd_bdn(const float* x2, const float* w_pre, const float* rstd_pre, const bf16_t* dn,
                                  float* dR, const bf16_t* t, const float* w_post, const float* rstd_t, bf16_t* dt,
-                                 int rows, int cols, hipStream_t st);
+                                 int rows, int cols, hipStream_t st, RowMap rmap = RowMap{0, 0, 0, 0});
 int residual_norm_bwd_wg_blocks(int rows);
 int launch_residual_norm_bwd_wg(const float* x2, const float* w_pre, const float* rstd_pre, const bf16_t* dn,
                                 float* dR, const bf16_t* t, const float* w_post, const float* rstd_t, bf16_t* dt,
                                 int rows, int cols, float* part_pre, float* part_post, hipStream_t st);
 int launch_rmsnorm_bwd_scatter(const float* x, RowMap xmap, const float* w, const float* rstd,
-                               const float* dn, float* dR, int rows, int cols, hipStream_t st);
+                               const float* dn, float* dR, int rows, int cols, hipStream_t st,
+                               const RowMap* dmap = nullptr);
 
 struct AttnShape {
   int B, S, Hq, Hkv, D;
@@ -251,6 +253,7 @@
   const int32_t* key_valid = nullptr;
   float scale = 1.f;
   int variant = 0;
+  int row_lo = 0;
 };
 int launch_attn_fwd(const FlashArgs& a, int nz, hipStream_t st);
 struct FlashBwdArgs {
@@ -277,15 +280,26 @@
   int dkv_items = 0;
   unsigned char dkv_item_slab[128], dkv_item_piece[128];
   int dkv_deferred = 0;
-};
+  int row_lo = 0;
+  int row_hi = 0;
+  int dkv_slab_c[128][2] = {};
+};
+bool attn_row_lo_ok(const FlashBwdArgs& a);
 
 constexpr int DKV_KEYS = 128, DKV_CH = 32;
 __host__ __device__ inline void dkv_slab_chunks(const FlashBwdArgs& a, int s, int& c_lo, int& c_hi) {
+  c_lo = a.dkv_slab_c[s][0];
+  c_hi = a.dkv_slab_c[s][1];
+}
+inline void dkv_slab_range(const FlashBwdArgs& a, int s, int& c_lo, int& c_hi) {
+  using std::max;
+  using std::min;
   int r_lo = 0, r_hi = a.rows;
   if (a.causal) {
     r_lo = min(a.rows, s * DKV_KEYS * a.qdiv);
     if (a.window > 0) r_hi = min(a.rows, (s * DKV_KEYS + DKV_KEYS + a.window - 1) * a.qdiv);
   }
+  r_lo = max(r_lo, a.row_lo);
   c_lo = r_lo / DKV_CH;
   c_hi = max(c_lo, (r_hi + DKV_CH - 1) / DKV_CH);
 }
diff --git a/projectiontrainer_amd/kernels.py b/projectiontrainer_amd/kernels.py
--- a/projectiontrainer_amd/kernels.py
+++ b/projectiontrainer_amd/kernels.py
@@ -207,7 +207,7 @@
 
 def flash_attn(Q, K, V, O, *, rows, nkeys, head_dim, ldq, ldk, ldo, batch, batch_inner=1, zdiv=1,
                strides=(0, 0, 0, 0, 0, 0), qmap=(0, 0, 0, 0), omap=(0, 0, 0, 0), qdiv=1, causal=False,
-               window=0, key_valid=None, scale=1.0, lse=None):
+               window=0, key_valid=None, scale=1.0, lse=None, row_lo=0):
     _require_cuda(Q, K, V, O)
     d = L.FlashDesc()
     d.Q, d.K, d.V, d.O, d.lse = ptr(Q), ptr(K), ptr(V), ptr(O), ptr(lse)
@@ -218,15 +218,16 @@
     d.qmap, d.omap = L.RowMap(*qmap), L.RowMap(*omap)
     d.qdiv, d.causal, d.window = qdiv, int(causal), window
     d.key_valid, d.scale = ptr(key_valid), scale
+    d.row_lo = row_lo
     check(L.lib().ptk_flash_attn_fwd(d, L.stream_ptr(Q.device)), "flash_attn_fwd")
     return O
 
 
 def flash_attn_bwd(Q, K, V, O, dO, lse, *, rows, nkeys, head_dim, batch, batch_inner=1, zdiv=1, ldo=None,
                    sO=(0, 0), omap=(0, 0, 0, 0), qdiv=1, causal=False, window=0, key_valid=None, scale=1.0,
-                   split=True):
+                   split=True, row_lo=0, out=None):
     _require_cuda(Q, K, V, O, dO, lse)
-    dQ, dK, dV = torch.empty_like(Q), torch.empty_like(K), torch.empty_like(V)
+    dQ, dK, dV = out if out is not None else (torch.empty_like(Q), torch.empty_like(K), torch.empty_like(V))
     delta = torch.empty(batch * rows, dtype=torch.float32, device=Q.device)
     d = L.FlashBwdDesc()
     d.Q, d.K, d.V, d.O, d.dO, d.lse, d.delta = ptr(Q), ptr(K), ptr(V), ptr(O), ptr(dO), ptr(lse), ptr(delta)
@@ -238,6 +239,7 @@
     d.omap = L.RowMap(*omap)
     d.qdiv, d.causal, d.window = qdiv, int(causal), window
     d.key_valid, d.scale = ptr(key_valid), scale
+    d.row_lo = row_lo
     ws = None
     if split:
         nb = L.lib().ptk_flash_bwd_workspace_bytes(d)
```

Result: no change. 323.7 images/sec, median of 6 (+0.6%).
